# noamzilo/sed-crnn

Measured on AMD Instinct MI355X. Metric: mel-frames/sec training throughput (seq=256, mel=40), higher is better.
Workload: dtype f32; 1 GPU; BASELINE config 2: mono (B=128,256,40,1) per GPU, 3xConv3x3(128)+BN+ReLU+pool(1,2)+dropout0.5, BiGRU 2x128, Linear(256,1), BCEWithLogits, Adam lr 1e-3; full fit step (fwd+loss+bwd+allreduce+Adam); global_batch=128, seq_len=256, n_mels=40, parallelism=single

## Files before the change

### include/sedcrnn.h

```cpp
#ifndef SEDCRNN_H
#define SEDCRNN_H

#include <stddef.h>
#include <stdint.h>

#ifdef __cplusplus
extern "C" {
#endif

#define SED_MAX_CONV 4
#define SED_MAX_GRU 4
#define SED_MAX_DENSE 4

int sed_version(void);
const char* sed_last_error_string(void);

int sed_conv3x3_pack_weights(const float* w_oihw, float* wp_fwd, float* wp_dgrad,
                             int Cout, int Cin, void* stream);

int sed_conv3x3_stat_rows(int B, int Cin, int F, int T, int Cout, int x_is_nchw);

int sed_conv3x3_plan(int B, int Cin, int F, int T, int Cout, int x_is_nchw, int which, int* out);

int sed_conv3x3_fwd(const float* x, int x_is_nchw, const float* wp, const float* bias,
                    float* y, float* stat_partials,
                    int B, int Cin, int F, int T, int Cout, void* stream);

int sed_conv3x3_pack_weights_ex(const float* w_oihw, float* wp_fwd, float* wp_dgrad, int Cout, int Cin, int mode, void* stream);
int sed_conv3x3_fwd_ex(const float* x, int x_is_nchw, const float* wp, const float* bias, float* y, float* stat_partials,
                       int B, int Cin, int F, int T, int Cout, int mode, void* stream);

size_t sed_conv3x3_wgrad_workspace_bytes(int B, int Cin, int F, int T, int Cout);
int sed_conv3x3_wgrad(const float* x, int x_is_nchw, const float* dy, float* dw_oihw,
                      void* workspace, int B, int Cin, int F, int T, int Cout, void* stream);

#define SED_WGRAD_ZERO_ROW_CLEAN 0x100
#define SED_WGRAD_DIRECT 0x200
size_t sed_conv3x3_wgrad_zero_row_bytes(int B, int Cin, int F, int T, int Cout);
int sed_conv3x3_wgrad_ex(const float* x, int x_is_nchw, const float* dy, float* dw_oihw,
                         void* workspace, int B, int Cin, int F, int T, int Cout, int mode, void* stream);

int sed_conv3x3_bn_relu_pool_eval_supported(int B, int Cin, int F, int T, int Cout);
int sed_conv3x3_pack_weights_bn_folded(const float* w, const float* bias, const float* gamma, const float* beta,
                                       const float* running_mean, const float* running_var, float eps,
                                       float* wf, float* bias_folded, int Cout, int Cin, void* stream);
int sed_conv3x3_bn_relu_pool_eval(const float* x, const float* wp_folded, const float* bias_folded, float* pooled,
                                  int B, int Cin, int F, int T, int Cout, void* stream);
int sed_conv3x3_bf16_eval_supported(int B, int Cin, int F, int T, int Cout);
int sed_conv3x3_bf16_pack_weights_bn_folded(const float* w, const float* bias, const float* gamma, const float* beta,
                                            const float* running_mean, const float* running_var, float eps,
                                            void* wf_bf16, float* bias_folded, int Cout, int Cin, void* stream);
int sed_conv3x3_bf16_bn_relu_pool_eval(const void* x, int x_is_bf16, const void* wf_bf16, const float* bias_folded,
                                       void* pooled_bf16, int B, int Cin, int F, int T, int Cout, void* stream);
int sed_conv3x3_dgrad_bnred_rows(int B, int C, int F, int T, int Cin);
int sed_conv3x3_dgrad_bnred(const float* dy, const float* wp_dgrad, float* dx, float* partials, const float* pooled,
                            const float* gamma, const float* beta, const float* conv_out_below, const float* mean,
                            const float* rstd, float drop_p, int pool_f, int pool_t, int Fy, int Ty,
                            int B, int C, int F, int T, int Cin, void* stream);
int sed_conv3x3_wino_rows(int B, int Cin, int F, int T, int Cout);
int sed_conv3x3_wino_phase_ticks(unsigned long long* buf);
size_t sed_conv3x3_wino_packed_floats(int Cout, int Cin);
int sed_conv3x3_wino_pack_weights(const float* w_oihw, float* uf, float* ud, int Cout, int Cin, void* stream);
int sed_conv3x3_wino_fwd(const float* x, const float* uf, const float* bias, float* y, float* stat_partials,
                         int B, int Cin, int F, int T, int Cout, void* stream);
int sed_conv3x3_wino_dgrad_bnred(const float* dy, const float* ud, float* dx, float* partials, const float* pooled,
                                 const float* gamma, const float* beta, const float* conv_out_below, const float* mean,
                                 const float* rstd, float drop_p, int pool_f, int pool_t, int Fy, int Ty,
                                 int B, int C, int F, int T, int Cin, void* stream);
int sed_conv3x3_wino_pack_weights_bn_folded(const float* w_oihw, const float* bias, const float* gamma, const float* beta,
                                            const float* running_mean, const float* running_var, float eps,
                                            float* uf, float* bias_folded, int Cout, int Cin, void* stream);
int sed_conv3x3_wino_bn_relu_pool_eval(const float* x, const float* uf_folded, const float* bias_folded, float* pooled,
                                       int B, int Cin, int F, int T, int Cout, void* stream);
int sed_conv3x3_wino_rg_rows(int B, int C, int F, int T, int Cin, int Cin1);
int sed_conv3x3_wino_dgrad_bnred_rg(const float* dy, const float* ud, float* dx, float* partials, const float* pooled,
                                    const float* gamma, const float* beta, const float* mean, const float* rstd, float drop_p,
                                    const float* x1, int Cin1, const unsigned char* argmax_bits, float* rg_partials,
                                    int B, int C, int F, int T, int Cin, void* stream);
int sed_conv3x3_dgrad_bnred_rg_rows(int B, int C, int F, int T, int Cin, int Cin1);
int sed_conv3x3_dgrad_bnred_rg(const float* dy, const float* wp_dgrad, float* dx, float* partials, const float* pooled,
                               const float* gamma, const float* beta, const float* mean, const float* rstd, float drop_p,
                               const float* x1, int Cin1, const unsigned char* argmax_bits, float* rg_partials,
                               int B, int C, int F, int T, int Cin, void* stream);

int sed_bn_finalize_train(const float* stat_partials, int rows, int C, double count,
                          const float* gamma, const float* beta,
                          float* running_mean, float* running_var, float momentum, float eps,
                          float* mean, float* rstd, float* scale, float* shift, void* stream);
int sed_bn_stat_sums(const float* stat_partials, int rows, int C, float* sums, void* stream);
int sed_bn_finalize_from_sums(const float* sums, int C, double count, const float* gamma, const float* beta,
                              float* running_mean, float* running_var, float momentum, float eps,
                              float* mean, float* rstd, float* scale, float* shift, void* stream);
int sed_bn_finalize_eval(const float* gamma, const float* beta, const float* running_mean,
                         const float* running_var, float eps, int C,
                         float* scale, float* shift, void* stream);

int sed_bn_relu_pool_drop_fwd(const float* y, const float* scale, const float* shift, float* out,
                              int B, int T, int F, int C, int pool_f, int pool_t, int out_tcf,
                              float drop_p, uint64_t seed, const uint64_t* seed_dev, void* stream);

int sed_bn_relu_pool_route(const float* y, const float* scale, const float* shift, unsigned char* route,
                           int B, int T, int F, int C, int pool_f, int pool_t, void* stream);
int sed_bn_bwd_rows(int B, int T, int pool_t);
int sed_bn_relu_pool_drop_bwd_reduce(const float* y, const float* dout, const float* scale,
                                     const float* shift, const float* mean, const float* rstd,
                                     float* partials, int B, int T, int F, int C, int pool_f,
                                     int pool_t, int out_tcf, float drop_p, uint64_t seed, const uint64_t* seed_dev, void* stream);
int sed_bn_bwd_finalize(const float* partials, int rows, int C, float* sum_g, float* sum_gx,
                        float* dgamma, float* dbeta, void* stream);
int sed_bn_bwd_finalize_small_gamma(const float* partials, int rows, int C, float* sum_g, float* sum_gx,
                                    float* dgamma, float* dbeta, const float* dpooled, const float* pooled,
                                    const float* y, const float* gamma, const float* beta, const float* mean,
                                    const float* rstd, const float* scale, const float* shift,
                                    int B, int T, int F, int pool_f, int pool_t, float drop_p, void* stream);
int sed_bn_bwd_reduce_pooled_supported(int F, int C, int pool_f, int pool_t, int out_tcf);
int sed_bn_bwd_reduce_pooled(const float* pooled, const float* dout, const float* gamma, const float* beta,
                             const float* y, const float* mean, const float* rstd, const float* scale, const float* shift,
                             float* partials, int B, int T, int F, int C, int pool_f, int pool_t, int out_tcf, float drop_p, void* stream);
int sed_bn_relu_pool_drop_bwd_apply(const float* y, const float* dout, const float* scale,
                                    const float* shift, const float* mean, const float* rstd,
                                    const float* sum_g, const float* sum_gx, float* dy,
                                    float* dbias_partials, int B, int T, int F, int C, int pool_f,
                                    int pool_t, int out_tcf, float drop_p, uint64_t seed, const uint64_t* seed_dev, void* stream);
int sed_reduce_rows(const float* partials, int rows, int C, int row_stride, float* out, void* stream);

int sed_conv1_fused_supported(int Cin, int F, int T, int C, int pool_f, int pool_t);
int sed_conv1_fused_rows(int B, int T);
size_t sed_conv1_stats_workspace_bytes(int B, int Cin, int T);
size_t sed_conv1_moments_doubles(int Cin);
int sed_conv1_stats(const float* x, const float* wp, const float* bias, float* stat_partials, void* workspace,
                    int B, int Cin, int F, int T, int C, double* moments, void* stream);
int sed_conv1_bn_relu_pool_drop_fwd(const float* x, const float* wp, const float* bias, const float* scale,
                                    const float* shift, float* out, int B, int Cin, int F, int T, int C,
                                    int pool_f, int pool_t, float drop_p, uint64_t seed, const uint64_t* seed_dev,
                                    unsigned char* argmax_bits, void* stream);
int sed_conv1_route(const float* x, const float* wp, const float* bias, const float* scale, const float* shift,
                    unsigned char* route, int B, int Cin, int F, int T, int C, int pool_f, int pool_t, void* stream);
int sed_conv1_bwd_reduce(const float* x, const float* wp, const float* bias, const float* dout,
                         const float* scale, const float* shift, const float* mean, const float* rstd,
                         float* partials, int B, int Cin, int F, int T, int C, int pool_f, int pool_t,
                         float drop_p, uint64_t seed, const uint64_t* seed_dev, void* stream);
size_t sed_conv1_bwd_apply_workspace_bytes(int B, int Cin, int T, int C);
int sed_conv1_bwd_apply_wgrad(const float* x, const float* wp, const float* bias, const float* dout,
                              const float* scale, const float* shift, const float* mean, const float* rstd,
                              const float* sum_g, const float* sum_gx, float* dw_oihw, float* dbias,
                              void* workspace, int B, int Cin, int F, int T, int C, int pool_f, int pool_t,
                              float drop_p, uint64_t seed, const uint64_t* seed_dev,
                              const float* gamma, const float* beta, float* dgamma, void* stream);

int sed_conv1_rgrad_supported(int Cin, int F, int T, int C, int pool_f, int pool_t);
size_t sed_conv1_bwd_wgrad_workspace_bytes(int B, int Cin, int T, int C);
int sed_conv1_bwd_wgrad(const float* x, const float* dout, const float* pooled, const unsigned char* argmax_bits,
                        const double* moments, const float* wp, const float* bias, const float* mean, const float* rstd,
                        const float* scale, const float* sum_g, const float* sum_gx, float* dw_oihw, float* dbias,
                        void* workspace, int B, int Cin, int F, int T, int C, float drop_p,
                        const float* gamma, const float* beta, float* dgamma, void* stream);
int sed_conv1_bwd_wgrad_assemble(const float* partials, int rows, const double* moments, const float* wp, const float* bias,
                                 const float* mean, const float* rstd, const float* scale, const float* sum_g,
                                 const float* sum_gx, float* dw_oihw, float* dbias, int B, int Cin, int F, int T, int C,
                                 const float* gamma, const float* beta, float* dgamma, void* stream);

int sed_gemm_f32(const float* A, long a_si, long a_sk, const float* B, long b_sk, long b_sj,
                 float* C, long ldc, const float* bias, float beta, int M, int N, int K, void* stream);
size_t sed_gemm_f32_workspace_bytes(int M, int N, int K);
int sed_gemm_f32_ws(const float* A, long a_si, long a_sk, const float* B, long b_sk, long b_sj,
                    float* C, long ldc, const float* bias, int M, int N, int K, void* workspace, void* stream);

int sed_gemm_bf16_nt(const void* A, const void* B, const float* bias, float* C, long ldc, int M, int N, int K, void* stream);

int sed_gemm_f32_wgrad(const float* A, long a_si, long a_sk, const float* B, long b_sk, long b_sj,
                       float* C, long ldc, int M, int N, int K, void* workspace, void* stream);
int sed_gemm_f32_plan(int M, int N, int K, int policy, int* bm, int* bn, int* splits, int* k_len);

int sed_linear_fwd(const float* x, const float* W, const float* b, float* y,
                   int M, int K, int N, int relu, void* stream);
size_t sed_linear_bwd_workspace_bytes(int M, int K, int N);
int sed_linear_bwd(const float* x, const float* W, const float* y, float* dy, float* dx,
                   float* dW, float* db, void* workspace, int M, int K, int N, int relu, void* stream);

size_t sed_gru_seq_workspace_bytes(int H);
int sed_gru_seq_fwd(const float* gi, const float* const* whh, const float* const* bhh,
                    float* out, float* saved, void* workspace, int B, int T, int H, void* stream);
size_t sed_gru_seq_bwd_workspace_bytes(int B, int H);
int sed_gru_seq_bwd(const float* dout, const float* saved, const float* const* whh,
                    float* dgi, float* dgh, float* const* dbih, float* const* dbhh, void* workspace,
                    int B, int T, int H, void* stream);
int sed_gru_seq_variant(int B, int H, int* bt, int* hreg, int* hlds);

int sed_loss_fwd_bwd(const float* logits, const float* targets, int n, int kind, float alpha,
                     float gamma, int reduction_mean, float* loss, float* dlogits, float* probs,
                     void* stream);
int sed_sigmoid(const float* x, float* y, int n, void* stream);
int sed_scale(float* x, long n, float alpha, void* stream);

size_t sed_sqnorm_workspace_bytes(long n);
int sed_grad_norm_clip_coef(const float* g, long n, float max_norm, float* norm_out,
                            void* workspace, void* stream);
int sed_adam_step(float* p, const float* g, float* m, float* v, long n, float lr, float beta1,
                  float beta2, float eps, float weight_decay, int step, const float* grad_scale,
                  const uint64_t* step_state, void* stream);
int sed_step_advance(uint64_t* step_state, void* stream);

size_t sed_logmel_tables_bytes(const float* melfb_host, int n_fft, int n_mels);
int sed_logmel_build_tables(const float* window_host, const float* melfb_host, int n_fft, int n_mels,
                            void* tables_host, size_t tables_bytes);
int sed_logmel(const float* pcm, long n_samples, const void* tables, size_t tables_bytes,
               const float* mu, const float* inv_sigma, float* out,
               int n_fft, int hop, int n_mels, int pad_mode, void* stream);
size_t sed_logmel_batch_workspace_bytes(int R);
int sed_logmel_batch(const float* pcm, long pcm_len, const long* clips_host, int R, const void* tables, size_t tables_bytes,
                     const float* mu, const float* inv_sigma, float* out, long out_rows, int n_fft, int hop, int n_mels,
                     int pad_mode, void* workspace, size_t workspace_bytes, void* stream);
size_t sed_logmel_multi_workspace_bytes(int R, int channels);
int sed_logmel_multi(const float* pcm, long pcm_len, const long* clips_host, int R, int channels, const void* tables,
                     size_t tables_bytes, const float* mu, const float* inv_sigma, float* out, long out_rows, int n_fft, int hop,
                     int n_mels, int pad_mode, void* workspace, size_t workspace_bytes, void* stream);
size_t sed_logmel_gcc_workspace_bytes(int R, int channels);
int sed_logmel_gcc(const float* pcm, long pcm_len, const long* clips_host, int R, int channels, const void* tables,
                   size_t tables_bytes, const float* mu, const float* inv_sigma, float* out, long out_rows, int n_fft, int hop,
                   int n_mels, int n_lags, int pad_mode, void* workspace, size_t workspace_bytes, void* stream);
size_t sed_event_tdoa_workspace_bytes(int R, int channels, long E, long max_n_samples, int hop, int max_frames);
int sed_event_tdoa(const float* pcm, long pcm_len, const long* clips_host, int R, int channels, const void* tables,
                   size_t tables_bytes, const int* ev_rec, const int* ev_onset, const int* ev_offset, const int* ev_peak_frame,
                   long E, int time_factor, int hop, int pad_mode, int max_lag, int max_frames, float* lag_out, float* strength_out,
                   int* frames_out, float* acc_out, void* workspace, size_t workspace_bytes, void* stream);
size_t sed_stream_ring_write_workspace_bytes(int lanes);
int sed_stream_ring_write(float* ring, long ring_len, int lanes, long cap, const float* src, long src_len, const long* table_host,
                          void* workspace, size_t workspace_bytes, void* stream);
size_t sed_event_tdoa_ring_workspace_bytes(int R, int channels, long E, long cap, int hop, int max_frames);
int sed_event_tdoa_ring(const float* ring, long ring_len, long cap, const long* n_host, int R, int channels, const void* tables,
                        size_t tables_bytes, const int* ev_rec, const int* ev_onset, const int* ev_offset, const int* ev_peak_frame,
                        long E, int time_factor, int hop, int max_lag, int max_frames, int lat_frames, int history_frames,
                        float* lag_out, float* strength_out, int* frames_out, float* acc_out, void* workspace,
                        size_t workspace_bytes, void* stream);
size_t sed_event_doa_workspace_bytes(int R, int channels, long E, long max_n_samples, int hop, int max_frames);
int sed_event_doa(const float* pcm, long pcm_len, const long* clips_host, int R, int channels, const void* tables,
                  size_t tables_bytes, const int* ev_rec, const int* ev_onset, const int* ev_offset, const int* ev_peak_frame,
                  long E, int time_factor, int hop, int pad_mode, int max_lag, int max_frames, float* lag_out, float* strength_out,
                  int* frames_out, float* acc_out, const int* steer_lags, int D, int Q, const float* trig, int* dir_out,
                  float* power_out, float* srp_out, void* workspace, size_t workspace_bytes, void* stream);
size_t sed_event_doa_ring_workspace_bytes(int R, int channels, long E, long cap, int hop, int max_frames);
int sed_event_doa_ring(const float* ring, long ring_len, long cap, const long* n_host, int R, int channels, const void* tables,
                       size_t tables_bytes, const int* ev_rec, const int* ev_onset, const int* ev_offset, const int* ev_peak_frame,
                       long E, int time_factor, int hop, int max_lag, int max_frames, int lat_frames, int history_frames,
                       float* lag_out, float* strength_out, int* frames_out, float* acc_out, const int* steer_lags, int D, int Q,
                       const float* trig, int* dir_out, float* power_out, float* srp_out, void* workspace, size_t workspace_bytes,
                       void* stream);
size_t sed_event_doa_track_workspace_bytes(int R, int channels, long E, long max_n_samples, int hop, int max_frames, int D,
                                           int block_chunks, int smooth);
int sed_event_doa_track(const float* pcm, long pcm_len, const long* clips_host, int R, int channels, const void* tables,
                        size_t tables_bytes, const int* ev_rec, const int* ev_onset, const int* ev_offset, const int* ev_peak_frame,
                        long E, int time_factor, int hop, int pad_mode, int max_lag, int max_frames, float* lag_out,
// ... 50 lines not shown
                         const int* ev_loc_frames, long E, int time_factor, int hop, int max_frames, const double* tau, int D,
                         double loading, int noise_blocks, int noise_guard, const void* tables, size_t tables_bytes,
                         const int* audio_len, const long* audio_start, float* audio, long audio_total, int* noise_frames_out,
                         void* workspace, size_t workspace_bytes, void* stream);
size_t sed_event_mvdr_noise_ring_workspace_bytes(int R, int channels, int max_frames, int hop, int noise_blocks);
int sed_event_mvdr_noise_ring(const float* ring, long ring_len, long cap, const long* n_host, int R, int channels, const int* ev_rec,
                              const int* ev_onset, const int* ev_offset, const int* ev_peak_frame, const int* ev_dir,
                              const int* ev_loc_frames, long E, int time_factor, int hop, int max_frames, const double* tau, int D,
                              double loading, int noise_blocks, int noise_guard, const void* tables, size_t tables_bytes,
                              const int* audio_len, const long* audio_start, float* audio, long audio_total, int* noise_frames_out,
                              void* workspace, size_t workspace_bytes, void* stream);

size_t sed_event_quiet_frames_workspace_bytes(int R, int channels, long mask_frames, int noise_blocks);
int sed_event_quiet_frames(long pcm_len, const long* clips_host, int R, int channels, const int* ev_rec, const int* ev_cls,
                           const int* ev_onset, const int* ev_offset, const int* ev_peak_frame, const int* ev_dir,
                           const int* ev_loc_frames, long E, int time_factor, int hop, int max_frames, int D, int n_classes,
                           int noise_blocks, int noise_guard, int noise_search, int noise_min, int exclude_any, int* noise_frames_out,
                           int* noise_sel_out, void* workspace, size_t workspace_bytes, void* stream);
size_t sed_event_mvdr_quiet_workspace_bytes(int R, int channels, int max_frames, int hop, int noise_blocks, long mask_frames);
int sed_event_mvdr_quiet(const float* pcm, long pcm_len, const long* clips_host, int R, int channels, const int* ev_rec,
                         const int* ev_cls, const int* ev_onset, const int* ev_offset, const int* ev_peak_frame, const int* ev_dir,
                         const int* ev_loc_frames, long E, int time_factor, int hop, int max_frames, const double* tau, int D,
                         double loading, int noise_blocks, int noise_guard, int n_classes, int noise_search, int noise_min,
                         int exclude_any, const void* tables, size_t tables_bytes, const int* audio_len, const long* audio_start,
                         float* audio, long audio_total, int* noise_frames_out, int* noise_sel_out, void* workspace,
                         size_t workspace_bytes, void* stream);

size_t sed_event_mvdr_track_workspace_bytes(int R, int channels, int max_frames, int hop, int noise_blocks, int track_slots);
int sed_event_mvdr_track(const float* pcm, long pcm_len, const long* clips_host, int R, int channels, const int* ev_rec,
                         const int* ev_onset, const int* ev_offset, const int* ev_peak_frame, const int* ev_dir,
                         const int* ev_loc_frames, long E, int time_factor, int hop, int max_frames, const double* tau, int D,
                         double loading, int noise_blocks, int noise_guard, const void* tables, size_t tables_bytes,
                         const int* audio_len, const long* audio_start, float* audio, long audio_total, int* noise_frames_out,
                         int block_chunks, int track_slots, const int* trk_len, const int* trk_dir, void* workspace,
                         size_t workspace_bytes, void* stream);
size_t sed_event_mvdr_track_ring_workspace_bytes(int R, int channels, int max_frames, int hop, int noise_blocks, int track_slots);
int sed_event_mvdr_track_ring(const float* ring, long ring_len, long cap, const long* n_host, int R, int channels, const int* ev_rec,
                              const int* ev_onset, const int* ev_offset, const int* ev_peak_frame, const int* ev_dir,
                              const int* ev_loc_frames, long E, int time_factor, int hop, int max_frames, const double* tau, int D,
                              double loading, int noise_blocks, int noise_guard, const void* tables, size_t tables_bytes,
                              const int* audio_len, const long* audio_start, float* audio, long audio_total, int* noise_frames_out,
                              int block_chunks, int track_slots, const int* trk_len, const int* trk_dir, void* workspace,
                              size_t workspace_bytes, void* stream);
size_t sed_event_mvdr_quiet_track_workspace_bytes(int R, int channels, int max_frames, int hop, int noise_blocks, long mask_frames,
                                                  int track_slots);
int sed_event_mvdr_quiet_track(const float* pcm, long pcm_len, const long* clips_host, int R, int channels, const int* ev_rec,
                               const int* ev_cls, const int* ev_onset, const int* ev_offset, const int* ev_peak_frame,
                               const int* ev_dir, const int* ev_loc_frames, long E, int time_factor, int hop, int max_frames,
                               const double* tau, int D, double loading, int noise_blocks, int noise_guard, int n_classes,
                               int noise_search, int noise_min, int exclude_any, const void* tables, size_t tables_bytes,
                               const int* audio_len, const long* audio_start, float* audio, long audio_total, int* noise_frames_out,
                               int* noise_sel_out, int block_chunks, int track_slots, const int* trk_len, const int* trk_dir,
                               void* workspace, size_t workspace_bytes, void* stream);

size_t sed_pcen_workspace_bytes(long rows, int R, int W);
int sed_pcen(float* x, long rows, int stride, int col0, int W, const long* recs_host, int R, float* state, double smooth_b,
             float gain, float bias, float power, float eps, float scale, const float* mu, const float* inv_sigma,
             void* workspace, size_t workspace_bytes, void* stream);

size_t sed_resample_workspace_bytes(int R);
int sed_resample_check_table(const long* rows_host, int R, long x_frames, long hist_len, long out_len, int L, int M, int half);
int sed_resample(const void* x, long x_frames, int format, int channels, float* hist, long hist_len, const float* taps,
                 long taps_len, int L, int M, int half, const long* rows_host, int R, float* out, long out_len, void* workspace,
                 size_t workspace_bytes, void* stream);
size_t sed_resample_select_workspace_bytes(int R);
int sed_resample_select_check_table(const long* rows_host, int R, int channels, long x_frames, long hist_len, long out_len, int L,
                                    int M, int half);
int sed_resample_select(const void* x, long x_frames, int format, int channels, float* hist, long hist_len, const float* taps,
                        long taps_len, int L, int M, int half, const long* rows_host, int R, float* out, long out_len,
                        void* workspace, size_t workspace_bytes, void* stream);

int sed_window_batch(const float* mel, const float* lab, long N, int C, int F, int K, const int* starts,
                     const int* tmask, const int* fmask, int n_masks, int time_w, int freq_w,
                     float* x, float* y, int B, int L, int pool, void* stream);
int sed_pack_sequences(const float* feat, long N, int C, int F, int S, int time_last, float* out, void* stream);
size_t sed_col_mean_std_workspace_bytes(int F);
int sed_col_mean_std(const float* x, long N, int F, double* mean, double* stdv, void* workspace, void* stream);
int sed_col_standardize(const float* x, long N, int F, const double* mean, const double* stdv, float* out, void* stream);

#define SED_SEGMENT_COUNTS 17
int sed_segment_counts(const float* pred, const float* lab, long rows, int K, int block, float threshold,
                       unsigned long long* counts17, void* stream);

int sed_detect_stitch(const float* logits, long n_win, int win_out, int K, int hop_out, long last_start_out, long n_out,
                      int combine, int trim, float* probs, void* stream);
size_t sed_detect_workspace_bytes(long n_out, int K, int max_events);
int sed_detect_events(const float* probs, long n_out, int K, int median, float lo, float hi, int min_gap, int min_len,
                      int max_events, void* workspace, size_t workspace_bytes, int* cls, int* onset, int* offset,
                      float* peak, int* peak_frame, int* count, void* stream);
size_t sed_detect_batch_workspace_bytes(long n_total, int K, int R, int max_events);
int sed_detect_stitch_batch(const float* logits, long logits_len, const long* recs_host, int R, int K, int combine, int trim,
                            float* probs, long n_total, void* workspace, size_t workspace_bytes, void* stream);
int sed_detect_events_batch(const float* probs, const long* n_out_host, int R, int K, int median, float lo, float hi, int min_gap,
                            int min_len, int max_events, void* workspace, size_t workspace_bytes, int* rec, int* cls, int* onset,
                            int* offset, float* peak, int* peak_frame, int* event_off, void* stream);

typedef struct sed_tune_setting { int median; float lo, hi; int min_gap, min_len; } sed_tune_setting;
size_t sed_tune_workspace_bytes(long n_total, int K, int R, int n_tracks, int G);
int sed_tune_sweep(const float* probs, const long* n_out_host, int R, int K, const sed_tune_setting* settings_host, int G,
                   const int* ref_off, const int* ref_onset, const int* ref_offset, const int* ref_tol, int collar, int block,
                   void* workspace, size_t workspace_bytes, long* counts, void* stream);

size_t sed_psds_workspace_bytes(long n_total, int K, int R, int n_tracks, int G);
int sed_psds_sweep(const float* probs, const long* n_out_host, int R, int K, const sed_tune_setting* settings_host, int G,
                   const int* ref_off, const int* ref_onset, const int* ref_offset, int dtc_milli, int gtc_milli, int cttc_milli,
                   void* workspace, size_t workspace_bytes, long* counts, long* ct, void* stream);

size_t sed_stream_state_bytes(int S, int K, int win_out, int hop_out, int median, int max_new_windows);
int sed_stream_init(void* state, size_t state_bytes, int S, int K, int win_out, int hop_out, int median, int max_new_windows,
                    void* stream);
int sed_stream_reset(void* state, size_t state_bytes, int S, int K, int win_out, int hop_out, int median, int max_new_windows,
                     const int* streams_host, int n_streams, void* stream);
size_t sed_stream_step_workspace_bytes(int S, int K, int max_new_decided);
int sed_stream_step(void* state, size_t state_bytes, int S, int K, int win_out, int hop_out, int median, int max_new_windows,
                    int combine, int trim, float lo, float hi, int min_gap, int min_len, const float* logits, long logits_len,
                    const long* table_host, int max_new_decided, float* probs, long probs_rows, int max_events, int* ev_stream,
                    int* cls, int* onset, int* offset, float* peak, int* peak_frame, int* event_off, void* workspace,
                    size_t workspace_bytes, void* stream);
size_t sed_stream_append_workspace_bytes(int S);
int sed_stream_append(float* buf, long buf_len, long stride, const float* fresh, long fresh_len, float* work, long work_len,
                      const long* table_host, int S, void* workspace, size_t workspace_bytes, void* stream);

typedef sed_tune_setting sed_decoder_setting;
int sed_detect_events_classwise(const float* probs, long n_out, int K, const sed_decoder_setting* classes_host, int max_events,
                                void* workspace, size_t workspace_bytes, int* cls, int* onset, int* offset, float* peak,
                                int* peak_frame, int* count, void* stream);
int sed_detect_events_batch_classwise(const float* probs, const long* n_out_host, int R, int K,
                                      const sed_decoder_setting* classes_host, int max_events, void* workspace, size_t workspace_bytes,
                                      int* rec, int* cls, int* onset, int* offset, float* peak, int* peak_frame, int* event_off,
                                      void* stream);
int sed_stream_step_classwise(void* state, size_t state_bytes, int S, int K, int win_out, int hop_out, int median, int max_new_windows,
                              int combine, int trim, const sed_decoder_setting* classes_host, const float* logits, long logits_len,
                              const long* table_host, int max_new_decided, float* probs, long probs_rows, int max_events,
                              int* ev_stream, int* cls, int* onset, int* offset, float* peak, int* peak_frame, int* event_off,
                              void* workspace, size_t workspace_bytes, void* stream);

typedef struct sed_net_cfg {
    int B, Cin, F, T;
    int n_conv;
    int C[SED_MAX_CONV];
    int pool_f[SED_MAX_CONV], pool_t[SED_MAX_CONV];
    float drop_p[SED_MAX_CONV];
    int n_gru;
    int H[SED_MAX_GRU];
    int n_dense;
    int D[SED_MAX_DENSE];
    float bn_eps, bn_momentum;
    int conv_mode;
    int flags;
} sed_net_cfg;
#define SED_NET_AUX_FIRST 0x1
#define SED_NET_NO_GATE 0x2
#define SED_NET_DIRECT_CONV 0x4

typedef struct sed_net_params {
    float* conv_w[SED_MAX_CONV];
    float* conv_b[SED_MAX_CONV];
    float* bn_g[SED_MAX_CONV];
    float* bn_b[SED_MAX_CONV];
    float* bn_rm[SED_MAX_CONV];
    float* bn_rv[SED_MAX_CONV];
    float* gru_wih[SED_MAX_GRU][2];
    float* gru_whh[SED_MAX_GRU][2];
    float* gru_bih[SED_MAX_GRU][2];
    float* gru_bhh[SED_MAX_GRU][2];
    float* dense_w[SED_MAX_DENSE];
    float* dense_b[SED_MAX_DENSE];
} sed_net_params;

int sed_net_out_shape(const sed_net_cfg* cfg, int* Tp, int* Fp);
size_t sed_net_workspace_bytes(const sed_net_cfg* cfg, int training);
int sed_net_forward(const sed_net_cfg* cfg, const sed_net_params* p, const float* x, float* logits,
                    void* workspace, int training, uint64_t seed, const uint64_t* seed_dev, void* stream);
int sed_net_backward(const sed_net_cfg* cfg, const sed_net_params* p, const sed_net_params* g,
                     const float* x, const float* dlogits, void* workspace, uint64_t seed, const uint64_t* seed_dev,
                     int stage_begin, int stage_end, void* stream, void* aux_stream);
int sed_net_backward_ready_stage(const sed_net_cfg* cfg, int block);

int sed_net_sync_region(const sed_net_cfg* cfg, int backward, int block, size_t* offset_bytes, size_t* n_floats);
int sed_net_forward_phases(const sed_net_cfg* cfg, const sed_net_params* p, const float* x, float* logits,
                           void* workspace, int training, uint64_t seed, int phase_begin, int phase_end,
                           float count_scale, void* stream);
int sed_net_backward_phases(const sed_net_cfg* cfg, const sed_net_params* p, const sed_net_params* g,
                            const float* x, const float* dlogits, void* workspace, uint64_t seed,
                            int phase_begin, int phase_end, float count_scale, void* stream);

int sed_net_workspace_region(const sed_net_cfg* cfg, int training, const char* name, int index,
                             size_t* offset_bytes, size_t* n_floats);

int sed_net_inference_plan(const sed_net_cfg* cfg, int* conv_bf16, int* proj_bf16);

int sed_net_routing(const sed_net_cfg* cfg, const sed_net_params* p, const float* x, const void* workspace, int block,
                    unsigned char* route, void* stream);

enum sed_kernel_tag {
    SED_K_CONV_MFMA_FWD = 0,
    SED_K_CONV_SMALL_FWD,
    SED_K_CONV_MFMA_WGRAD,
    SED_K_CONV_SMALL_WGRAD,
    SED_K_BN_FWD,
    SED_K_BN_BWD_REDUCE,
    SED_K_BN_BWD_APPLY,
    SED_K_GEMM,
    SED_K_GRU_FWD,
    SED_K_GRU_BWD,
    SED_K_ADAM,
    SED_K_LOGMEL,
    SED_K_CONV_MFMA_DGRAD,
    SED_K_COUNT
};
int sed_prof_enable(unsigned tag_mask);
int sed_prof_read(int tag, double* total_ms, long* launches, double* total_units);
const char* sed_prof_tag_name(int tag);
int sed_prof_tag_count(void);

#ifdef __cplusplus
}
#endif
#endif
```

### sed_crnn_amd/_lib.py

```python
import ctypes as C
import os

HERE = os.path.dirname(os.path.abspath(__file__))
LIB_PATH = os.environ.get("SED_CRNN_LIB") or os.path.join(HERE, "libsedcrnn.so")

SED_MAX_CONV = 4
SED_MAX_GRU = 4
SED_MAX_DENSE = 4

_fp = C.c_void_p
_stream = C.c_void_p


class NetCfg(C.Structure):
    _fields_ = [
        ("B", C.c_int), ("Cin", C.c_int), ("F", C.c_int), ("T", C.c_int),
        ("n_conv", C.c_int),
        ("C", C.c_int * SED_MAX_CONV),
        ("pool_f", C.c_int * SED_MAX_CONV), ("pool_t", C.c_int * SED_MAX_CONV),
        ("drop_p", C.c_float * SED_MAX_CONV),
        ("n_gru", C.c_int), ("H", C.c_int * SED_MAX_GRU),
        ("n_dense", C.c_int), ("D", C.c_int * SED_MAX_DENSE),
        ("bn_eps", C.c_float), ("bn_momentum", C.c_float),
        ("conv_mode", C.c_int),
        ("flags", C.c_int),
    ]


class NetParams(C.Structure):
    _fields_ = [
        ("conv_w", _fp * SED_MAX_CONV), ("conv_b", _fp * SED_MAX_CONV),
        ("bn_g", _fp * SED_MAX_CONV), ("bn_b", _fp * SED_MAX_CONV),
        ("bn_rm", _fp * SED_MAX_CONV), ("bn_rv", _fp * SED_MAX_CONV),
        ("gru_wih", (_fp * 2) * SED_MAX_GRU), ("gru_whh", (_fp * 2) * SED_MAX_GRU),
        ("gru_bih", (_fp * 2) * SED_MAX_GRU), ("gru_bhh", (_fp * 2) * SED_MAX_GRU),
        ("dense_w", _fp * SED_MAX_DENSE), ("dense_b", _fp * SED_MAX_DENSE),
    ]


class TuneSetting(C.Structure):
    _fields_ = [("median", C.c_int), ("lo", C.c_float), ("hi", C.c_float), ("min_gap", C.c_int), ("min_len", C.c_int)]


_i, _l, _f, _d, _u64, _sz = C.c_int, C.c_long, C.c_float, C.c_double, C.c_uint64, C.c_size_t
_pp = C.POINTER(_fp)

SIGNATURES = {
    "sed_version": (_i, []),
    "sed_last_error_string": (C.c_char_p, []),
    "sed_conv3x3_pack_weights": (_i, [_fp, _fp, _fp, _i, _i, _stream]),
    "sed_conv3x3_stat_rows": (_i, [_i, _i, _i, _i, _i, _i]),
    "sed_conv3x3_plan": (_i, [_i, _i, _i, _i, _i, _i, _i, C.POINTER(_i)]),
    "sed_conv3x3_fwd": (_i, [_fp, _i, _fp, _fp, _fp, _fp, _i, _i, _i, _i, _i, _stream]),
    "sed_conv3x3_pack_weights_ex": (_i, [_fp, _fp, _fp, _i, _i, _i, _stream]),
    "sed_conv3x3_fwd_ex": (_i, [_fp, _i, _fp, _fp, _fp, _fp, _i, _i, _i, _i, _i, _i, _stream]),
    "sed_conv3x3_wgrad_workspace_bytes": (_sz, [_i, _i, _i, _i, _i]),
    "sed_conv3x3_wgrad_zero_row_bytes": (_sz, [_i, _i, _i, _i, _i]),
    "sed_conv3x3_wgrad": (_i, [_fp, _i, _fp, _fp, _fp, _i, _i, _i, _i, _i, _stream]),
    "sed_conv3x3_wgrad_ex": (_i, [_fp, _i, _fp, _fp, _fp, _i, _i, _i, _i, _i, _i, _stream]),
    "sed_conv3x3_bn_relu_pool_eval_supported": (_i, [_i, _i, _i, _i, _i]),
    "sed_conv3x3_pack_weights_bn_folded": (_i, [_fp, _fp, _fp, _fp, _fp, _fp, _f, _fp, _fp, _i, _i, _stream]),
    "sed_conv3x3_bn_relu_pool_eval": (_i, [_fp, _fp, _fp, _fp, _i, _i, _i, _i, _i, _stream]),
    "sed_conv3x3_bf16_eval_supported": (_i, [_i, _i, _i, _i, _i]),
    "sed_conv3x3_bf16_pack_weights_bn_folded": (_i, [_fp, _fp, _fp, _fp, _fp, _fp, _f, _fp, _fp, _i, _i, _stream]),
    "sed_conv3x3_bf16_bn_relu_pool_eval": (_i, [_fp, _i, _fp, _fp, _fp, _i, _i, _i, _i, _i, _stream]),
    "sed_conv3x3_dgrad_bnred_rows": (_i, [_i, _i, _i, _i, _i]),
    "sed_conv3x3_dgrad_bnred": (_i, [_fp, _fp, _fp, _fp, _fp, _fp, _fp, _fp, _fp, _fp, _f, _i, _i, _i, _i, _i, _i, _i, _i, _i, _stream]),
    "sed_conv3x3_wino_rows": (_i, [_i, _i, _i, _i, _i]),
    "sed_conv3x3_wino_phase_ticks": (_i, [_fp]),
    "sed_conv3x3_wino_packed_floats": (_sz, [_i, _i]),
    "sed_conv3x3_wino_pack_weights": (_i, [_fp, _fp, _fp, _i, _i, _stream]),
    "sed_conv3x3_wino_fwd": (_i, [_fp, _fp, _fp, _fp, _fp, _i, _i, _i, _i, _i, _stream]),
    "sed_conv3x3_wino_dgrad_bnred": (_i, [_fp, _fp, _fp, _fp, _fp, _fp, _fp, _fp, _fp, _fp, _f, _i, _i, _i, _i, _i, _i, _i, _i, _i, _stream]),
    "sed_conv3x3_wino_pack_weights_bn_folded": (_i, [_fp, _fp, _fp, _fp, _fp, _fp, _f, _fp, _fp, _i, _i, _stream]),
    "sed_conv3x3_wino_bn_relu_pool_eval": (_i, [_fp, _fp, _fp, _fp, _i, _i, _i, _i, _i, _stream]),
    "sed_conv3x3_wino_rg_rows": (_i, [_i, _i, _i, _i, _i, _i]),
    "sed_conv3x3_wino_dgrad_bnred_rg": (_i, [_fp, _fp, _fp, _fp, _fp, _fp, _fp, _fp, _fp, _f, _fp, _i, _fp, _fp, _i, _i, _i, _i, _i, _stream]),
    "sed_conv3x3_dgrad_bnred_rg_rows": (_i, [_i, _i, _i, _i, _i, _i]),
    "sed_conv3x3_dgrad_bnred_rg": (_i, [_fp, _fp, _fp, _fp, _fp, _fp, _fp, _fp, _fp, _f, _fp, _i, _fp, _fp, _i, _i, _i, _i, _i, _stream]),
    "sed_conv1_fused_supported": (_i, [_i, _i, _i, _i, _i, _i]),
    "sed_conv1_fused_rows": (_i, [_i, _i]),
    "sed_conv1_stats_workspace_bytes": (_sz, [_i, _i, _i]),
    "sed_conv1_moments_doubles": (_sz, [_i]),
    "sed_conv1_stats": (_i, [_fp, _fp, _fp, _fp, _fp, _i, _i, _i, _i, _i, _fp, _stream]),
    "sed_conv1_bn_relu_pool_drop_fwd": (_i, [_fp, _fp, _fp, _fp, _fp, _fp, _i, _i, _i, _i, _i, _i, _i, _f, _u64, _fp, _fp, _stream]),
    "sed_conv1_rgrad_supported": (_i, [_i, _i, _i, _i, _i, _i]),
    "sed_conv1_bwd_wgrad_workspace_bytes": (_sz, [_i, _i, _i, _i]),
    "sed_conv1_bwd_wgrad": (_i, [_fp, _fp, _fp, _fp, _fp, _fp, _fp, _fp, _fp, _fp, _fp, _fp, _fp, _fp, _fp, _i, _i, _i, _i, _i, _f, _fp, _fp, _fp, _stream]),
    "sed_conv1_bwd_wgrad_assemble": (_i, [_fp, _i, _fp, _fp, _fp, _fp, _fp, _fp, _fp, _fp, _fp, _fp, _i, _i, _i, _i, _i, _fp, _fp, _fp, _stream]),
    "sed_conv1_route": (_i, [_fp, _fp, _fp, _fp, _fp, _fp, _i, _i, _i, _i, _i, _i, _i, _stream]),
    "sed_conv1_bwd_reduce": (_i, [_fp, _fp, _fp, _fp, _fp, _fp, _fp, _fp, _fp, _i, _i, _i, _i, _i, _i, _i, _f, _u64, _fp, _stream]),
    "sed_conv1_bwd_apply_workspace_bytes": (_sz, [_i, _i, _i, _i]),
    "sed_conv1_bwd_apply_wgrad": (_i, [_fp, _fp, _fp, _fp, _fp, _fp, _fp, _fp, _fp, _fp, _fp, _fp, _fp, _i, _i, _i, _i, _i, _i, _i, _f, _u64, _fp, _fp, _fp, _fp, _stream]),
    "sed_bn_finalize_train": (_i, [_fp, _i, _i, _d, _fp, _fp, _fp, _fp, _f, _f, _fp, _fp, _fp, _fp, _stream]),
    "sed_bn_stat_sums": (_i, [_fp, _i, _i, _fp, _stream]),
    "sed_bn_finalize_from_sums": (_i, [_fp, _i, _d, _fp, _fp, _fp, _fp, _f, _f, _fp, _fp, _fp, _fp, _stream]),
    "sed_bn_finalize_eval": (_i, [_fp, _fp, _fp, _fp, _f, _i, _fp, _fp, _stream]),
    "sed_bn_relu_pool_drop_fwd": (_i, [_fp, _fp, _fp, _fp, _i, _i, _i, _i, _i, _i, _i, _f, _u64, _fp, _stream]),
    "sed_bn_relu_pool_route": (_i, [_fp, _fp, _fp, _fp, _i, _i, _i, _i, _i, _i, _stream]),
    "sed_bn_bwd_rows": (_i, [_i, _i, _i]),
    "sed_bn_relu_pool_drop_bwd_reduce": (_i, [_fp, _fp, _fp, _fp, _fp, _fp, _fp, _i, _i, _i, _i, _i, _i, _i, _f, _u64, _fp, _stream]),
    "sed_bn_bwd_finalize": (_i, [_fp, _i, _i, _fp, _fp, _fp, _fp, _stream]),
    "sed_bn_bwd_finalize_small_gamma": (_i, [_fp, _i, _i, _fp, _fp, _fp, _fp, _fp, _fp, _fp, _fp, _fp, _fp, _fp, _fp, _fp, _i, _i, _i, _i, _i, _f, _stream]),
    "sed_bn_bwd_reduce_pooled_supported": (_i, [_i, _i, _i, _i, _i]),
    "sed_bn_bwd_reduce_pooled": (_i, [_fp, _fp, _fp, _fp, _fp, _fp, _fp, _fp, _fp, _fp, _i, _i, _i, _i, _i, _i, _i, _f, _stream]),
    "sed_bn_relu_pool_drop_bwd_apply": (_i, [_fp, _fp, _fp, _fp, _fp, _fp, _fp, _fp, _fp, _fp, _i, _i, _i, _i, _i, _i, _i, _f, _u64, _fp, _stream]),
    "sed_reduce_rows": (_i, [_fp, _i, _i, _i, _fp, _stream]),
    "sed_gemm_f32": (_i, [_fp, _l, _l, _fp, _l, _l, _fp, _l, _fp, _f, _i, _i, _i, _stream]),
    "sed_gemm_f32_workspace_bytes": (_sz, [_i, _i, _i]),
    "sed_gemm_f32_ws": (_i, [_fp, _l, _l, _fp, _l, _l, _fp, _l, _fp, _i, _i, _i, _fp, _stream]),
    "sed_gemm_bf16_nt": (_i, [_fp, _fp, _fp, _fp, _l, _i, _i, _i, _stream]),
    "sed_gemm_f32_wgrad": (_i, [_fp, _l, _l, _fp, _l, _l, _fp, _l, _i, _i, _i, _fp, _stream]),
    "sed_gemm_f32_plan": (_i, [_i, _i, _i, _i, C.POINTER(_i), C.POINTER(_i), C.POINTER(_i), C.POINTER(_i)]),
    "sed_linear_fwd": (_i, [_fp, _fp, _fp, _fp, _i, _i, _i, _i, _stream]),
    "sed_linear_bwd_workspace_bytes": (_sz, [_i, _i, _i]),
    "sed_linear_bwd": (_i, [_fp, _fp, _fp, _fp, _fp, _fp, _fp, _fp, _i, _i, _i, _i, _stream]),
    "sed_gru_seq_workspace_bytes": (_sz, [_i]),
    "sed_gru_seq_fwd": (_i, [_fp, _pp, _pp, _fp, _fp, _fp, _i, _i, _i, _stream]),
    "sed_gru_seq_bwd_workspace_bytes": (_sz, [_i, _i]),
    "sed_gru_seq_bwd": (_i, [_fp, _fp, _pp, _fp, _fp, _pp, _pp, _fp, _i, _i, _i, _stream]),
    "sed_gru_seq_variant": (_i, [_i, _i, C.POINTER(_i), C.POINTER(_i), C.POINTER(_i)]),
    "sed_loss_fwd_bwd": (_i, [_fp, _fp, _i, _i, _f, _f, _i, _fp, _fp, _fp, _stream]),
    "sed_sigmoid": (_i, [_fp, _fp, _i, _stream]),
    "sed_scale": (_i, [_fp, _l, _f, _stream]),
    "sed_sqnorm_workspace_bytes": (_sz, [_l]),
    "sed_grad_norm_clip_coef": (_i, [_fp, _l, _f, _fp, _fp, _stream]),
    "sed_adam_step": (_i, [_fp, _fp, _fp, _fp, _l, _f, _f, _f, _f, _f, _i, _fp, _fp, _stream]),
    "sed_step_advance": (_i, [_fp, _stream]),
    "sed_logmel_tables_bytes": (_sz, [_fp, _i, _i]),
    "sed_logmel_build_tables": (_i, [_fp, _fp, _i, _i, _fp, _sz]),
    "sed_logmel": (_i, [_fp, _l, _fp, _sz, _fp, _fp, _fp, _i, _i, _i, _i, _stream]),
    "sed_logmel_batch_workspace_bytes": (_sz, [_i]),
    "sed_logmel_batch": (_i, [_fp, _l, _fp, _i, _fp, _sz, _fp, _fp, _fp, _l, _i, _i, _i, _i, _fp, _sz, _stream]),
    "sed_logmel_multi_workspace_bytes": (_sz, [_i, _i]),
    "sed_logmel_multi": (_i, [_fp, _l, _fp, _i, _i, _fp, _sz, _fp, _fp, _fp, _l, _i, _i, _i, _i, _fp, _sz, _stream]),
    "sed_logmel_gcc_workspace_bytes": (_sz, [_i, _i]),
    "sed_logmel_gcc": (_i, [_fp, _l, _fp, _i, _i, _fp, _sz, _fp, _fp, _fp, _l, _i, _i, _i, _i, _i, _fp, _sz, _stream]),
    "sed_event_tdoa_workspace_bytes": (_sz, [_i, _i, _l, _l, _i, _i]),
    "sed_event_tdoa": (_i, [_fp, _l, _fp, _i, _i, _fp, _sz, _fp, _fp, _fp, _fp, _l, _i, _i, _i, _i, _i, _fp, _fp, _fp, _fp, _fp, _sz,
                            _stream]),
    "sed_stream_ring_write_workspace_bytes": (_sz, [_i]),
    "sed_stream_ring_write": (_i, [_fp, _l, _i, _l, _fp, _l, _fp, _fp, _sz, _stream]),
    "sed_event_tdoa_ring_workspace_bytes": (_sz, [_i, _i, _l, _l, _i, _i]),
    "sed_event_tdoa_ring": (_i, [_fp, _l, _l, _fp, _i, _i, _fp, _sz, _fp, _fp, _fp, _fp, _l, _i, _i, _i, _i, _i, _i, _fp, _fp, _fp, _fp,
                                 _fp, _sz, _stream]),
    "sed_event_doa_workspace_bytes": (_sz, [_i, _i, _l, _l, _i, _i]),
    "sed_event_doa": (_i, [_fp, _l, _fp, _i, _i, _fp, _sz, _fp, _fp, _fp, _fp, _l, _i, _i, _i, _i, _i, _fp, _fp, _fp, _fp, _fp, _i, _i,
                           _fp, _fp, _fp, _fp, _fp, _sz, _stream]),
    "sed_event_doa_ring_workspace_bytes": (_sz, [_i, _i, _l, _l, _i, _i]),
    "sed_event_doa_ring": (_i, [_fp, _l, _l, _fp, _i, _i, _fp, _sz, _fp, _fp, _fp, _fp, _l, _i, _i, _i, _i, _i, _i, _fp, _fp, _fp, _fp,
                                _fp, _i, _i, _fp, _fp, _fp, _fp, _fp, _sz, _stream]),
    "sed_event_doa_track_workspace_bytes": (_sz, [_i, _i, _l, _l, _i, _i, _i, _i, _i]),
    "sed_event_doa_track": (_i, [_fp, _l, _fp, _i, _i, _fp, _sz, _fp, _fp, _fp, _fp, _l, _i, _i, _i, _i, _i, _fp, _fp, _fp, _fp, _fp, _i,
                                 _i, _fp, _fp, _fp, _fp, _i, _fp, _fp, _fp, _fp, _fp, _fp, _fp, _fp, _sz, _stream]),
    "sed_event_doa_track_ring_workspace_bytes": (_sz, [_i, _i, _l, _l, _i, _i, _i, _i, _i]),
    "sed_event_doa_track_ring": (_i, [_fp, _l, _l, _fp, _i, _i, _fp, _sz, _fp, _fp, _fp, _fp, _l, _i, _i, _i, _i, _i, _i, _fp, _fp, _fp,
                                      _fp, _fp, _i, _i, _fp, _fp, _fp, _fp, _i, _fp, _fp, _fp, _fp, _fp, _fp, _fp, _fp, _sz, _stream]),
    "sed_event_beam_workspace_bytes": (_sz, [_i, _i]),
    "sed_event_beam_ring_workspace_bytes": (_sz, [_i]),
    "sed_event_beam_spans": (_i, [_l, _fp, _i, _i, _fp, _fp, _fp, _fp, _fp, _fp, _l, _i, _i, _i, _i, _fp, _fp, _fp, _fp, _sz, _stream]),
    "sed_event_beam_spans_ring": (_i, [_fp, _i, _i, _fp, _fp, _fp, _fp, _fp, _fp, _l, _i, _i, _i, _i, _fp, _fp, _fp, _fp, _sz, _stream]),
    "sed_event_beamform": (_i, [_fp, _l, _fp, _i, _i, _fp, _fp, _fp, _fp, _fp, _fp, _l, _i, _i, _i, _fp, _i, _i, _i, _fp, _fp, _fp, _fp,
                                _l, _fp, _sz, _stream]),
    "sed_event_beamform_ring": (_i, [_fp, _l, _l, _fp, _i, _i, _fp, _fp, _fp, _fp, _fp, _fp, _l, _i, _i, _i, _fp, _i, _i, _i, _fp, _fp,
                                     _fp, _fp, _l, _fp, _sz, _stream]),
    "sed_event_mvdr_workspace_bytes": (_sz, [_i, _i, _i, _i]),
    "sed_event_mvdr": (_i, [_fp, _l, _fp, _i, _i, _fp, _fp, _fp, _fp, _fp, _fp, _l, _i, _i, _i, _fp, _i, _d, _fp, _sz, _fp, _fp, _fp, _l,
                            _fp, _sz, _stream]),
    "sed_event_mvdr_ring_workspace_bytes": (_sz, [_i, _i, _i, _i]),
    "sed_event_mvdr_ring": (_i, [_fp, _l, _l, _fp, _i, _i, _fp, _fp, _fp, _fp, _fp, _fp, _l, _i, _i, _i, _fp, _i, _d, _fp, _sz, _fp, _fp,
                                 _fp, _l, _fp, _sz, _stream]),
    "sed_event_mvdr_noise_workspace_bytes": (_sz, [_i, _i, _i, _i, _i]),
    "sed_event_mvdr_noise": (_i, [_fp, _l, _fp, _i, _i, _fp, _fp, _fp, _fp, _fp, _fp, _l, _i, _i, _i, _fp, _i, _d, _i, _i, _fp, _sz, _fp,
                                  _fp, _fp, _l, _fp, _fp, _sz, _stream]),
    "sed_event_mvdr_noise_ring_workspace_bytes": (_sz, [_i, _i, _i, _i, _i]),
    "sed_event_mvdr_noise_ring": (_i, [_fp, _l, _l, _fp, _i, _i, _fp, _fp, _fp, _fp, _fp, _fp, _l, _i, _i, _i, _fp, _i, _d, _i, _i, _fp,
                                       _sz, _fp, _fp, _fp, _l, _fp, _fp, _sz, _stream]),
    "sed_event_quiet_frames_workspace_bytes": (_sz, [_i, _i, _l, _i]),
    "sed_event_quiet_frames": (_i, [_l, _fp, _i, _i, _fp, _fp, _fp, _fp, _fp, _fp, _fp, _l, _i, _i, _i, _i, _i, _i, _i, _i, _i, _i, _fp, _fp,
                                    _fp, _sz, _stream]),
    "sed_event_mvdr_quiet_workspace_bytes": (_sz, [_i, _i, _i, _i, _i, _l]),
    "sed_event_mvdr_quiet": (_i, [_fp, _l, _fp, _i, _i, _fp, _fp, _fp, _fp, _fp, _fp, _fp, _l, _i, _i, _i, _fp, _i, _d, _i, _i, _i, _i, _i,
                                  _i, _fp, _sz, _fp, _fp, _fp, _l, _fp, _fp, _fp, _sz, _stream]),
    "sed_event_mvdr_track_workspace_bytes": (_sz, [_i, _i, _i, _i, _i, _i]),
    "sed_event_mvdr_track": (_i, [_fp, _l, _fp, _i, _i, _fp, _fp, _fp, _fp, _fp, _fp, _l, _i, _i, _i, _fp, _i, _d, _i, _i, _fp, _sz, _fp,
                                  _fp, _fp, _l, _fp, _i, _i, _fp, _fp, _fp, _sz, _stream]),
    "sed_event_mvdr_track_ring_workspace_bytes": (_sz, [_i, _i, _i, _i, _i, _i]),
    "sed_event_mvdr_track_ring": (_i, [_fp, _l, _l, _fp, _i, _i, _fp, _fp, _fp, _fp, _fp, _fp, _l, _i, _i, _i, _fp, _i, _d, _i, _i, _fp,
                                       _sz, _fp, _fp, _fp, _l, _fp, _i, _i, _fp, _fp, _fp, _sz, _stream]),
    "sed_event_mvdr_quiet_track_workspace_bytes": (_sz, [_i, _i, _i, _i, _i, _l, _i]),
    "sed_event_mvdr_quiet_track": (_i, [_fp, _l, _fp, _i, _i, _fp, _fp, _fp, _fp, _fp, _fp, _fp, _l, _i, _i, _i, _fp, _i, _d, _i, _i, _i, _i,
                                        _i, _i, _fp, _sz, _fp, _fp, _fp, _l, _fp, _fp, _i, _i, _fp, _fp, _fp, _sz, _stream]),
    "sed_pcen_workspace_bytes": (_sz, [_l, _i, _i]),
    "sed_pcen": (_i, [_fp, _l, _i, _i, _i, _fp, _i, _fp, _d, _f, _f, _f, _f, _f, _fp, _fp, _fp, _sz, _stream]),
    "sed_resample_workspace_bytes": (_sz, [_i]),
    "sed_resample_check_table": (_i, [_fp, _i, _l, _l, _l, _i, _i, _i]),
    "sed_resample": (_i, [_fp, _l, _i, _i, _fp, _l, _fp, _l, _i, _i, _i, _fp, _i, _fp, _l, _fp, _sz, _stream]),
    "sed_resample_select_workspace_bytes": (_sz, [_i]),
    "sed_resample_select_check_table": (_i, [_fp, _i, _i, _l, _l, _l, _i, _i, _i]),
    "sed_resample_select": (_i, [_fp, _l, _i, _i, _fp, _l, _fp, _l, _i, _i, _i, _fp, _i, _fp, _l, _fp, _sz, _stream]),
    "sed_window_batch": (_i, [_fp, _fp, _l, _i, _i, _i, _fp, _fp, _fp, _i, _i, _i, _fp, _fp, _i, _i, _i, _stream]),
    "sed_pack_sequences": (_i, [_fp, _l, _i, _i, _i, _i, _fp, _stream]),
    "sed_col_mean_std_workspace_bytes": (_sz, [_i]),
    "sed_col_mean_std": (_i, [_fp, _l, _i, _fp, _fp, _fp, _stream]),
    "sed_col_standardize": (_i, [_fp, _l, _i, _fp, _fp, _fp, _stream]),
    "sed_segment_counts": (_i, [_fp, _fp, _l, _i, _i, _f, _fp, _stream]),
    "sed_detect_stitch": (_i, [_fp, _l, _i, _i, _i, _l, _l, _i, _i, _fp, _stream]),
    "sed_detect_workspace_bytes": (_sz, [_l, _i, _i]),
    "sed_detect_events": (_i, [_fp, _l, _i, _i, _f, _f, _i, _i, _i, _fp, _sz, _fp, _fp, _fp, _fp, _fp, _fp, _stream]),
    "sed_detect_batch_workspace_bytes": (_sz, [_l, _i, _i, _i]),
    "sed_detect_stitch_batch": (_i, [_fp, _l, _fp, _i, _i, _i, _i, _fp, _l, _fp, _sz, _stream]),
    "sed_detect_events_batch": (_i, [_fp, _fp, _i, _i, _i, _f, _f, _i, _i, _i, _fp, _sz, _fp, _fp, _fp, _fp, _fp, _fp, _fp, _stream]),
    "sed_tune_workspace_bytes": (_sz, [_l, _i, _i, _i, _i]),
    "sed_tune_sweep": (_i, [_fp, _fp, _i, _i, _fp, _i, _fp, _fp, _fp, _fp, _i, _i, _fp, _sz, _fp, _stream]),
    "sed_psds_workspace_bytes": (_sz, [_l, _i, _i, _i, _i]),
    "sed_psds_sweep": (_i, [_fp, _fp, _i, _i, _fp, _i, _fp, _fp, _fp, _i, _i, _i, _fp, _sz, _fp, _fp, _stream]),
    "sed_stream_state_bytes": (_sz, [_i, _i, _i, _i, _i, _i]),
    "sed_stream_init": (_i, [_fp, _sz, _i, _i, _i, _i, _i, _i, _stream]),
    "sed_stream_reset": (_i, [_fp, _sz, _i, _i, _i, _i, _i, _i, _fp, _i, _stream]),
    "sed_stream_step_workspace_bytes": (_sz, [_i, _i, _i]),
    "sed_stream_step": (_i, [_fp, _sz, _i, _i, _i, _i, _i, _i, _i, _i, _f, _f, _i, _i, _fp, _l, _fp, _i, _fp, _l, _i, _fp, _fp, _fp,
                             _fp, _fp, _fp, _fp, _fp, _sz, _stream]),
    "sed_stream_append_workspace_bytes": (_sz, [_i]),
    "sed_stream_append": (_i, [_fp, _l, _l, _fp, _l, _fp, _l, _fp, _i, _fp, _sz, _stream]),
    "sed_detect_events_classwise": (_i, [_fp, _l, _i, _fp, _i, _fp, _sz, _fp, _fp, _fp, _fp, _fp, _fp, _stream]),
    "sed_detect_events_batch_classwise": (_i, [_fp, _fp, _i, _i, _fp, _i, _fp, _sz, _fp, _fp, _fp, _fp, _fp, _fp, _fp, _stream]),
    "sed_stream_step_classwise": (_i, [_fp, _sz, _i, _i, _i, _i, _i, _i, _i, _i, _fp, _fp, _l, _fp, _i, _fp, _l, _i, _fp, _fp, _fp,
                                       _fp, _fp, _fp, _fp, _fp, _sz, _stream]),
    "sed_prof_enable": (_i, [C.c_uint]),
    "sed_prof_read": (_i, [_i, C.POINTER(_d), C.POINTER(_l), C.POINTER(_d)]),
    "sed_prof_tag_name": (C.c_char_p, [_i]),
    "sed_prof_tag_count": (_i, []),
    "sed_net_out_shape": (_i, [C.POINTER(NetCfg), C.POINTER(_i), C.POINTER(_i)]),
    "sed_net_workspace_bytes": (_sz, [C.POINTER(NetCfg), _i]),
    "sed_net_forward": (_i, [C.POINTER(NetCfg), C.POINTER(NetParams), _fp, _fp, _fp, _i, _u64, _fp, _stream]),
    "sed_net_sync_region": (_i, [C.POINTER(NetCfg), _i, _i, C.POINTER(_sz), C.POINTER(_sz)]),
    "sed_net_workspace_region": (_i, [C.POINTER(NetCfg), _i, C.c_char_p, _i, C.POINTER(_sz), C.POINTER(_sz)]),
    "sed_net_routing": (_i, [C.POINTER(NetCfg), C.POINTER(NetParams), _fp, _fp, _i, _fp, _stream]),
    "sed_net_inference_plan": (_i, [C.POINTER(NetCfg), C.POINTER(C.c_int), C.POINTER(C.c_int)]),
    "sed_net_forward_phases": (_i, [C.POINTER(NetCfg), C.POINTER(NetParams), _fp, _fp, _fp, _i, _u64, _i, _i, _f, _stream]),
    "sed_net_backward_phases": (_i, [C.POINTER(NetCfg), C.POINTER(NetParams), C.POINTER(NetParams), _fp, _fp, _fp, _u64, _i, _i, _f, _stream]),
    "sed_net_backward": (_i, [C.POINTER(NetCfg), C.POINTER(NetParams), C.POINTER(NetParams), _fp, _fp, _fp, _u64, _fp, _i, _i, _stream, _stream]),
    "sed_net_backward_ready_stage": (_i, [C.POINTER(NetCfg), _i]),
}

_lib = None


class SedHipError(RuntimeError):
    pass

# ... 33 lines not shown
```

### sed_crnn_amd/csrc/bnpool.hip

```cpp
#include "common.h"

#define BN_MAX_BLOCKS 1024

__device__ __forceinline__ void bn_two_channel_sums(const float* __restrict__ part, int rows, int C, int c, bool live,
                                                    double (*sred)[2][2], double* A_out, double* Q_out) {
    const int sl = threadIdx.x >> 1, lane = threadIdx.x & 63, wv = threadIdx.x >> 6;
    double a = 0.0, q = 0.0;
    if (live) {
#pragma unroll 8
        for (int r = sl; r < rows; r += 512) {
            const float* p0 = part + (size_t)r * 2 * C + c;
            a += (double)p0[0];
            q += (double)p0[C];
        }
    }
#pragma unroll
    for (int o = 2; o < 64; o <<= 1) { a += __shfl_xor(a, o, 64); q += __shfl_xor(q, o, 64); }
    if (lane < 2) { sred[wv][lane][0] = a; sred[wv][lane][1] = q; }
    __syncthreads();
    double A = 0.0, Q = 0.0;
    if (threadIdx.x < 2) {
        for (int w = 0; w < 16; ++w) { A += sred[w][threadIdx.x][0]; Q += sred[w][threadIdx.x][1]; }
    }
    *A_out = A; *Q_out = Q;
// ... 88 lines not shown
    int c = blockIdx.x * blockDim.x + threadIdx.x;
    if (c >= C) return;
    float sc = g[c] / sqrtf(rv[c] + eps);
    scale[c] = sc;
    shift[c] = b[c] - rm[c] * sc;
}

extern "C" int sed_bn_finalize_eval(const float* gamma, const float* beta, const float* rm, const float* rv,
                                    float eps, int C, float* scale, float* shift, void* stream) {
    SED_REQUIRE(gamma && beta && rm && rv && scale && shift && C > 0, "bn_finalize_eval: bad arguments");
    bn_finalize_eval_k<<<cdiv(C, 256), 256, 0, as_stream(stream)>>>(gamma, beta, rm, rv, eps, C, scale, shift);
    SED_LAUNCH_CHECK("bn_finalize_eval");
    return 0;
}

__global__ __launch_bounds__(256) void reduce_rows_k(const float* __restrict__ part, int rows, int C,
                                                     int row_stride, float* __restrict__ out) {
    __shared__ double s1[32][9];
    const int cl = threadIdx.x & 7, sl = threadIdx.x >> 3;
    const int c = blockIdx.x * 8 + cl;
    double a = 0.0;
    if (c < C) {
        double a1 = 0.0, a2 = 0.0, a3 = 0.0;
        int r = sl;
        for (; r + 96 < rows; r += 128) {
            const float* p0 = part + (size_t)r * row_stride + c;
            a += (double)p0[0];
            a1 += (double)p0[(size_t)32 * row_stride];
            a2 += (double)p0[(size_t)64 * row_stride];
            a3 += (double)p0[(size_t)96 * row_stride];
        }
        for (; r < rows; r += 32) a += (double)part[(size_t)r * row_stride + c];
        a += a1 + a2 + a3;
    }
    s1[sl][cl] = a;
    __syncthreads();
    if (sl == 0 && c < C) {
        double A = 0.0;
        for (int s = 0; s < 32; ++s) A += s1[s][cl];
        out[c] = (float)A;
    }
}

extern "C" int sed_reduce_rows(const float* part, int rows, int C, int row_stride, float* out, void* stream) {
    SED_REQUIRE(part && out && rows > 0 && C > 0 && row_stride >= C, "reduce_rows: bad arguments");
    reduce_rows_k<<<cdiv(C, 8), 256, 0, as_stream(stream)>>>(part, rows, C, row_stride, out);
    SED_LAUNCH_CHECK("reduce_rows");
    return 0;
}

__global__ __launch_bounds__(256) void bn_relu_pool_drop_fwd_k(
    const float* __restrict__ y, const float* __restrict__ scale, const float* __restrict__ shift,
    float* __restrict__ out, int B, int T, int F, int C, int pf, int pt, float drop_p, uint64_t seed,
    const uint64_t* __restrict__ seed_dev) {
    if (seed_dev) seed += seed_dev[0] * 0x9E3779B97F4A7C15ull;
    const int Tp = T / pt, Fp = F / pf, C4 = C >> 2;
    const size_t n = (size_t)B * Tp * Fp * C4;
    const float inv_keep = drop_p > 0.f ? 1.f / (1.f - drop_p) : 1.f;
    for (size_t i = (size_t)blockIdx.x * 256 + threadIdx.x; i < n; i += (size_t)gridDim.x * 256) {
        int c4 = (int)(i % C4);
        size_t pos = i / C4;
        int fp = (int)(pos % Fp);
        size_t bt = pos / Fp;
        int tp = (int)(bt % Tp);
        size_t b = bt / Tp;
        f32x4 sc = *(const f32x4*)(scale + c4 * 4), sh = *(const f32x4*)(shift + c4 * 4);
        f32x4 m = {0, 0, 0, 0};
        for (int dt = 0; dt < pt; ++dt)
            for (int df = 0; df < pf; ++df) {
                f32x4 v = *(const f32x4*)(y + (((b * T + tp * pt + dt) * F + fp * pf + df) * (size_t)C) + c4 * 4);
                v = v * sc + sh;
#pragma unroll
                for (int k = 0; k < 4; ++k) m[k] = fmaxf(m[k], v[k]);
            }
        if (drop_p > 0.f) {
#pragma unroll
            for (int k = 0; k < 4; ++k) m[k] *= sed_drop_mult(seed, i * 4 + k, drop_p, inv_keep);
        }
        *(f32x4*)(out + i * 4) = m;
    }
}

__global__ __launch_bounds__(256) void bn_relu_pool_drop_fwd_tcf_k(
    const float* __restrict__ y, const float* __restrict__ scale, const float* __restrict__ shift,
    float* __restrict__ out, int B, int T, int F, int C, int pf, int pt, float drop_p, uint64_t seed,
    const uint64_t* __restrict__ seed_dev) {
    if (seed_dev) seed += seed_dev[0] * 0x9E3779B97F4A7C15ull;
    extern __shared__ __attribute__((aligned(16))) float tile[];
    const int Tp = T / pt, Fp = F / pf, C4 = C >> 2, LD = C + 1;
    const float inv_keep = drop_p > 0.f ? 1.f / (1.f - drop_p) : 1.f;
    for (int bt = blockIdx.x; bt < B * Tp; bt += gridDim.x) {
        int tp = bt % Tp;
        size_t b = bt / Tp;
        __syncthreads();
        for (int i = threadIdx.x; i < Fp * C4; i += 256) {
            int c4 = i % C4, fp = i / C4;
            f32x4 sc = *(const f32x4*)(scale + c4 * 4), sh = *(const f32x4*)(shift + c4 * 4);
            f32x4 m = {0, 0, 0, 0};
            for (int dt = 0; dt < pt; ++dt)
                for (int df = 0; df < pf; ++df) {
                    f32x4 v = *(const f32x4*)(y + (((b * T + tp * pt + dt) * F + fp * pf + df) * (size_t)C) + c4 * 4);
                    v = v * sc + sh;
#pragma unroll
                    for (int k = 0; k < 4; ++k) m[k] = fmaxf(m[k], v[k]);
                }
            if (drop_p > 0.f) {
                size_t oi = (((size_t)bt * Fp + fp) * C4 + c4) * 4;
#pragma unroll
                for (int k = 0; k < 4; ++k) m[k] *= sed_drop_mult(seed, oi + k, drop_p, inv_keep);
            }
#pragma unroll
            for (int k = 0; k < 4; ++k) tile[fp * LD + c4 * 4 + k] = m[k];
        }
        __syncthreads();
        float* o = out + (size_t)bt * C * Fp;
        for (int i = threadIdx.x; i < C * Fp; i += 256) {
            int c = i / Fp, fp = i - c * Fp;
            o[i] = tile[fp * LD + c];
        }
    }
}

static int check_pool(const char* who, int B, int T, int F, int C, int pf, int pt) {
    SED_REQUIRE(B > 0 && T > 0 && F > 0 && C > 0 && pf > 0 && pt > 0, "%s: bad shape", who);
    SED_REQUIRE(C % 4 == 0, "%s: C must be a multiple of 4 (got %d)", who, C);
    SED_REQUIRE(T / pt >= 1 && F / pf >= 1, "%s: T=%d / F=%d smaller than the pool (%d,%d)", who, T, F, pt, pf);
    return 0;
}

extern "C" int sed_bn_relu_pool_drop_fwd(const float* y, const float* scale, const float* shift, float* out, int B,
                                         int T, int F, int C, int pf, int pt, int out_tcf, float drop_p,
                                         uint64_t seed, const uint64_t* seed_dev, void* stream) {
    SED_REQUIRE(y && scale && shift && out, "bn_relu_pool_drop_fwd: null pointer");
    SED_TRY(check_pool("bn_relu_pool_drop_fwd", B, T, F, C, pf, pt));
    SED_REQUIRE(drop_p >= 0.f && drop_p < 1.f, "bn_relu_pool_drop_fwd: drop_p=%f out of [0,1)", drop_p);
    hipStream_t s = as_stream(stream);
    const int Tp = T / pt, Fp = F / pf;
    SedProfScope prof(SED_K_BN_FWD, s, 4.0 * B * C * ((double)T * F + (double)Tp * Fp));
    if (!out_tcf) {
        size_t n = (size_t)B * Tp * Fp * (C / 4);
        int grid = (int)((n + 255) / 256 < 8192 ? (n + 255) / 256 : 8192);
        bn_relu_pool_drop_fwd_k<<<grid, 256, 0, s>>>(y, scale, shift, out, B, T, F, C, pf, pt, drop_p, seed, seed_dev);
    } else {
        size_t lds = (size_t)Fp * (C + 1) * sizeof(float);
        SED_REQUIRE(lds <= 150 * 1024, "bn_relu_pool_drop_fwd: F'*C tile too large for LDS");
        if (lds > 48 * 1024) (void)hipFuncSetAttribute((const void*)bn_relu_pool_drop_fwd_tcf_k, hipFuncAttributeMaxDynamicSharedMemorySize, (int)lds);
        int grid = B * Tp < 4096 ? B * Tp : 4096;
        bn_relu_pool_drop_fwd_tcf_k<<<grid, 256, lds, s>>>(y, scale, shift, out, B, T, F, C, pf, pt, drop_p, seed, seed_dev);
    }
    SED_LAUNCH_CHECK("bn_relu_pool_drop_fwd");
    return 0;
}

__global__ __launch_bounds__(256) void bn_relu_pool_route_k(
    const float* __restrict__ y, const float* __restrict__ scale, const float* __restrict__ shift,
    unsigned char* __restrict__ route, int B, int T, int F, int C, int pf, int pt) {
    const int Tp = T / pt, Fp = F / pf, C4 = C >> 2;
    const size_t n = (size_t)B * Tp * Fp * C4;
    for (size_t i = (size_t)blockIdx.x * 256 + threadIdx.x; i < n; i += (size_t)gridDim.x * 256) {
        int c4 = (int)(i % C4);
        size_t pos = i / C4;
        int fp = (int)(pos % Fp);
        size_t bt = pos / Fp;
        int tp = (int)(bt % Tp);
        size_t b = bt / Tp;
        f32x4 sc = *(const f32x4*)(scale + c4 * 4), sh = *(const f32x4*)(shift + c4 * 4);
        f32x4 best = {-INFINITY, -INFINITY, -INFINITY, -INFINITY};
        int bidx[4] = {0, 0, 0, 0};
        int widx = 0;
        for (int df = 0; df < pf; ++df)
            for (int dt = 0; dt < pt; ++dt, ++widx) {
                f32x4 v = *(const f32x4*)(y + (((b * T + tp * pt + dt) * F + fp * pf + df) * (size_t)C) + c4 * 4);
                f32x4 z = v * sc + sh;
#pragma unroll
                for (int k = 0; k < 4; ++k)
                    if (z[k] > best[k]) { best[k] = z[k]; bidx[k] = widx; }
            }
        uchar4 code;
        code.x = best[0] > 0.f ? (unsigned char)(1 + bidx[0]) : 0;
        code.y = best[1] > 0.f ? (unsigned char)(1 + bidx[1]) : 0;
        code.z = best[2] > 0.f ? (unsigned char)(1 + bidx[2]) : 0;
        code.w = best[3] > 0.f ? (unsigned char)(1 + bidx[3]) : 0;
        *(uchar4*)(route + i * 4) = code;
    }
}

extern "C" int sed_bn_relu_pool_route(const float* y, const float* scale, const float* shift, unsigned char* route,
                                      int B, int T, int F, int C, int pf, int pt, void* stream) {
    SED_REQUIRE(y && scale && shift && route, "bn_relu_pool_route: null pointer");
    SED_TRY(check_pool("bn_relu_pool_route", B, T, F, C, pf, pt));
    SED_REQUIRE(pf * pt <= 254, "bn_relu_pool_route: a %dx%d window does not fit the one-byte code", pf, pt);
    size_t n = (size_t)B * (T / pt) * (F / pf) * (C / 4);
    int grid = (int)((n + 255) / 256 < 8192 ? (n + 255) / 256 : 8192);
    bn_relu_pool_route_k<<<grid, 256, 0, as_stream(stream)>>>(y, scale, shift, route, B, T, F, C, pf, pt);
    SED_LAUNCH_CHECK("bn_relu_pool_route");
    return 0;
}

extern "C" int sed_bn_bwd_rows(int B, int T, int pool_t) {
    long r = (long)B * (T / (pool_t > 0 ? pool_t : 1));
    return (int)(r < BN_MAX_BLOCKS ? r : BN_MAX_BLOCKS);
}

template <int MODE, bool P12>
__global__ __launch_bounds__(256) void bn_relu_pool_drop_bwd_k(
    const float* __restrict__ y, const float* __restrict__ dout, const float* __restrict__ scale,
    const float* __restrict__ shift, const float* __restrict__ mean, const float* __restrict__ rstd,
    const float* __restrict__ sum_g, const float* __restrict__ sum_gx, float* __restrict__ dy,
    float* __restrict__ partials, int B, int T, int F, int C, int pf, int pt, int out_tcf, float drop_p,
    uint64_t seed, const uint64_t* __restrict__ seed_dev) {
    if (seed_dev) seed += seed_dev[0] * 0x9E3779B97F4A7C15ull;
    extern __shared__ __attribute__((aligned(16))) float smem[];
    const int Tp = T / pt, Fp = F / pf, C4 = C >> 2, LD = C + 1;
    float* tile = smem;
    const int tid = threadIdx.x;
    const int nslots = 256 / C4 > 0 ? 256 / C4 : 1;
    const int c4 = tid % C4, slot = tid / C4;
    const bool active = slot < nslots;
    const float inv_keep = drop_p > 0.f ? 1.f / (1.f - drop_p) : 1.f;
    const float invN = 1.f / ((float)B * (float)T * (float)F);

    f32x4 sc = {0, 0, 0, 0}, sh = sc, mu = sc, rs = sc, sg = sc, sgx = sc;
    if (active) {
        sc = *(const f32x4*)(scale + c4 * 4);
        sh = *(const f32x4*)(shift + c4 * 4);
        mu = *(const f32x4*)(mean + c4 * 4);
        rs = *(const f32x4*)(rstd + c4 * 4);
        if (MODE == 1) {
            sg = *(const f32x4*)(sum_g + c4 * 4) * invN;
            sgx = *(const f32x4*)(sum_gx + c4 * 4) * invN;
        }
    }
    f32x4 a1 = {0, 0, 0, 0}, a2 = {0, 0, 0, 0};

    for (int bt = blockIdx.x; bt < B * Tp; bt += gridDim.x) {
        int tp = bt % Tp;
        size_t b = bt / Tp;
        if (out_tcf) {
            __syncthreads();
            const float* d = dout + (size_t)bt * C * Fp;
            for (int i = tid; i < C * Fp; i += 256) {
                int c = i / Fp, fp = i - c * Fp;
                tile[fp * LD + c] = d[i];
            }
            __syncthreads();
        }
        if (!active) continue;
        for (int fp = slot; fp < Fp; fp += nslots) {
            f32x4 g;
            if (out_tcf) {
#pragma unroll
                for (int k = 0; k < 4; ++k) g[k] = tile[fp * LD + c4 * 4 + k];
            } else {
                g = *(const f32x4*)(dout + (((size_t)bt * Fp + fp) * C4 + c4) * 4);
            }
            if (drop_p > 0.f) {
                size_t oi = (((size_t)bt * Fp + fp) * C4 + c4) * 4;
#pragma unroll
                for (int k = 0; k < 4; ++k) g[k] *= sed_drop_mult(seed, oi + k, drop_p, inv_keep);
            }
            f32x4 best = {-INFINITY, -INFINITY, -INFINITY, -INFINITY};
            f32x4 bx = {0, 0, 0, 0};
            int bidx[4] = {0, 0, 0, 0};
            int widx = 0;
            f32x4 vw[2];
            if (P12) {
                const float* yp = y + (((b * T + tp * 2) * F + fp) * (size_t)C) + c4 * 4;
                vw[0] = *(const f32x4*)yp;
                vw[1] = *(const f32x4*)(yp + (size_t)F * C);
            }
#pragma unroll
            for (int df = 0; df < (P12 ? 1 : pf); ++df)
#pragma unroll
                for (int dt = 0; dt < (P12 ? 2 : pt); ++dt, ++widx) {
                    f32x4 v = P12 ? vw[dt] : *(const f32x4*)(y + (((b * T + tp * pt + dt) * F + fp * pf + df) * (size_t)C) + c4 * 4);
                    f32x4 z = v * sc + sh;
#pragma unroll
                    for (int k = 0; k < 4; ++k)
                        if (z[k] > best[k]) { best[k] = z[k]; bx[k] = (v[k] - mu[k]) * rs[k]; bidx[k] = widx; }
                }
#pragma unroll
            for (int k = 0; k < 4; ++k)
                if (!(best[k] > 0.f)) g[k] = 0.f;
            if (MODE == 0) {
                a1 += g;
                a2 += g * bx;
            } else {
                widx = 0;
#pragma unroll
                for (int df = 0; df < (P12 ? 1 : pf); ++df)
#pragma unroll
                    for (int dt = 0; dt < (P12 ? 2 : pt); ++dt, ++widx) {
                        size_t off = (((b * T + tp * pt + dt) * F + fp * pf + df) * (size_t)C) + c4 * 4;
                        f32x4 v = P12 ? vw[dt] : *(const f32x4*)(y + off);
                        f32x4 o;
#pragma unroll
                        for (int k = 0; k < 4; ++k) {
                            float xh = (v[k] - mu[k]) * rs[k];
                            float gk = (bidx[k] == widx) ? g[k] : 0.f;
                            o[k] = sc[k] * (gk - sg[k] - xh * sgx[k]);
                        }
                        *(f32x4*)(dy + off) = o;
                        a1 += o;
                    }
            }
        }
// ... 307 lines not shown
```

### sed_crnn_amd/csrc/conv_shared.h

```cpp
#pragma once
#include "common.h"

struct ConvBnRed {
    const float* pooled;
    const float* gamma;
    const float* beta;
    const float* ybelow;
    const float* mean;
    const float* rstd;
    float keep, inv_keep;
    int pf, pt, Fy, Ty;
    const float* x1;
    const unsigned char* bits;
    float* rgp;
    float invXT;
};

#ifdef __HIPCC__
__host__ __device__ inline size_t wino_frag_index(int comp, int k, int n, int K, int N) {
    const int cc = k >> 5, g = (k & 31) >> 3, h = (k & 7) >> 2, j = k & 3, coh = n >> 6, nt = (n >> 5) & 1, r = n & 31;
    (void)N;
    return (((((((size_t)coh * 16 + comp) * (K >> 5) + cc) * 4 + g) * 2 + nt) * 64) + r + 32 * h) * 4 + j;
}
__host__ __device__ inline size_t bf16_eval_frag_index(int tap, int co, int ci, int Cout, int Cin) {
    return (((((size_t)tap * (Cin >> 4) + (ci >> 4)) * (Cout >> 5) + (co >> 5)) * 64) + (co & 31) + 32 * ((ci & 15) >> 3)) * 8 + (ci & 7);
}
#define WN_ZTAIL 256
__device__ __forceinline__ void wino_pack_one(const float* __restrict__ w, float* __restrict__ uf, float* __restrict__ ud, int Cout, int Cin, int i,
                                              const float* __restrict__ gamma = nullptr, const float* __restrict__ rv = nullptr, float eps = 0.f) {
    if (i < WN_ZTAIL) {
        if (uf) uf[(size_t)16 * Cout * Cin + i] = 0.f;
        if (ud) ud[(size_t)16 * Cout * Cin + i] = 0.f;
    }
    if (i >= Cout * Cin) return;
    const int ci = i % Cin, co = i / Cin;
    float g[3][3];
#pragma unroll
    for (int kh = 0; kh < 3; ++kh)
#pragma unroll
        for (int kw = 0; kw < 3; ++kw) g[kw][kh] = w[(size_t)i * 9 + kh * 3 + kw];
    if (gamma) {
        const float sc = gamma[co] / sqrtf(rv[co] + eps);
#pragma unroll
        for (int k = 0; k < 9; ++k) g[k / 3][k % 3] *= sc;
    }
#pragma unroll
    for (int pass = 0; pass < 2; ++pass) {
        float* dst = pass ? ud : uf;
        if (!dst) continue;
        float t[4][3];
#pragma unroll
        for (int c = 0; c < 3; ++c) {
            const float g0 = pass ? g[2][2 - c] : g[0][c], g1 = pass ? g[1][2 - c] : g[1][c], g2 = pass ? g[0][2 - c] : g[2][c];
            t[0][c] = g0;
            t[1][c] = 0.5f * (g0 + g1 + g2);
            t[2][c] = 0.5f * (g0 - g1 + g2);
            t[3][c] = g2;
        }
#pragma unroll
        for (int xi = 0; xi < 4; ++xi) {
            const float u0 = t[xi][0], u1 = 0.5f * (t[xi][0] + t[xi][1] + t[xi][2]), u2 = 0.5f * (t[xi][0] - t[xi][1] + t[xi][2]), u3 = t[xi][2];
            const float uu[4] = {u0, u1, u2, u3};
#pragma unroll
            for (int nu = 0; nu < 4; ++nu)
                dst[pass ? wino_frag_index(xi * 4 + nu, co, ci, Cout, Cin) : wino_frag_index(xi * 4 + nu, ci, co, Cin, Cout)] = uu[nu];
        }
    }
}
#endif

int sed_internal_wino_rows(int B, int Cin, int F, int T, int Cout);
int sed_internal_wino_launch(const float* x, const float* uq, const float* bias, float* y, float* stat, const ConvBnRed* br,
                             int rgc, int B, int Cin, int F, int T, int Cout, hipStream_t s);
```

### sed_crnn_amd/csrc/net.hip

```cpp
#include <string.h>
#include "common.h"

namespace {

struct ConvL { int Cin, C, T, F, Tp, Fp, pf, pt, rows, bn_rows, nchw, fused; float drop;
               int red_rows;
               int rg_rows;
               int rgrad;
               int wino, wino_d;
               int ev;
               int bf; };

struct GruL { int in, H; };

struct Layout {
    int n_conv, n_gru, n_dense, M, Tp, Fp, feat;
    int proj_bf;
    ConvL cv[SED_MAX_CONV];
    GruL gr[SED_MAX_GRU];
    int dK[SED_MAX_DENSE], dN[SED_MAX_DENSE];
    size_t wp_f[SED_MAX_CONV], wp_d[SED_MAX_CONV], conv_out[SED_MAX_CONV], stat[SED_MAX_CONV];
    size_t mean[SED_MAX_CONV], rstd[SED_MAX_CONV], scale[SED_MAX_CONV], shift[SED_MAX_CONV];
    size_t pooled[SED_MAX_CONV], bn_sums[SED_MAX_CONV], c1_stat_ws, c1_bits, c1_mom;
    size_t bias_f[SED_MAX_CONV];
    size_t wih_perm;
    size_t gi[SED_MAX_GRU], gout[SED_MAX_GRU], saved[SED_MAX_GRU];
    size_t gru_ws[SED_MAX_GRU];
    size_t act[SED_MAX_DENSE];
    size_t wgrad_zrow;
    size_t wg_arrive;
    size_t bn_part, sum_g, sum_gx, dbias_part, dconv[SED_MAX_CONV], gradA, wgrad_ws, wgrad_ws_aux, c1_ws, dgi[SED_MAX_GRU], dgh[SED_MAX_GRU], dgout[SED_MAX_GRU];
    size_t gru_bws[SED_MAX_GRU];
    size_t dact[SED_MAX_DENSE], lin_ws, gemm_ws, gemm_ws_aux;
    size_t total;
};

struct Carver {
    size_t off = 0;
    size_t take(size_t n) { size_t o = off; off += (n + 63) & ~(size_t)63; return o; }
};

int build_layout(const sed_net_cfg* c, int training, Layout* L) {
    SED_REQUIRE(c, "net: null config");
    SED_REQUIRE(c->B > 0 && c->Cin > 0 && c->F > 0 && c->T > 0, "net: bad input shape B=%d Cin=%d F=%d T=%d", c->B, c->Cin, c->F, c->T);
    SED_REQUIRE(c->n_conv >= 1 && c->n_conv <= SED_MAX_CONV, "net: n_conv=%d out of range", c->n_conv);
    SED_REQUIRE(c->n_gru >= 1 && c->n_gru <= SED_MAX_GRU, "net: n_gru=%d out of range", c->n_gru);
    SED_REQUIRE(c->n_dense >= 1 && c->n_dense <= SED_MAX_DENSE, "net: n_dense=%d out of range", c->n_dense);
    SED_REQUIRE(c->conv_mode >= 0 && c->conv_mode <= 2, "net: conv_mode=%d (0 = exact fp32, 1 = bf16x3 experiment, 2 = bf16 inference)", c->conv_mode);
    SED_REQUIRE(c->conv_mode != 2 || !training, "net: conv_mode 2 (bf16 inference) is an eval-only plan; training runs with conv_mode 0 or 1");
    SED_REQUIRE((c->flags & ~(SED_NET_AUX_FIRST | SED_NET_NO_GATE | SED_NET_DIRECT_CONV)) == 0, "net: unknown flags 0x%x", c->flags);
    memset(L, 0, sizeof(*L));
    L->n_conv = c->n_conv; L->n_gru = c->n_gru; L->n_dense = c->n_dense;
    const int fm = c->conv_mode == 2 ? 0 : c->conv_mode;
    int bfl[SED_MAX_CONV] = {0};
    if (c->conv_mode == 2) {
        int Ci = c->Cin, Ti = c->T, Fi = c->F;
        int ok[SED_MAX_CONV] = {0};
        for (int l = 0; l < c->n_conv; ++l) {
            const int pf = c->pool_f[l], pt = c->pool_t[l];
            ok[l] = l > 0 && pf == 1 && pt == 2 && c->C[l] > 0 && Ti >= 2 && sed_conv3x3_bf16_eval_supported(c->B, Ci, Fi, Ti, c->C[l]);
            if (l == c->n_conv - 1 && (size_t)c->C[l] * Fi * sizeof(float) > 64 * 1024) ok[l] = 0;
            Ci = c->C[l]; Ti = pt > 0 ? Ti / pt : Ti; Fi = pf > 0 ? Fi / pf : Fi;
        }
        for (int l = c->n_conv - 1; l >= 0 && ok[l]; --l) bfl[l] = 1;
    }
    Carver cv;
    int Cin = c->Cin, T = c->T, F = c->F;
    size_t max_pool = 0, max_wgrad = 0, c1_ws = 64, c1_stat_ws = 64;
    int max_bn_rows = 0, maxC = 0;
    for (int l = 0; l < c->n_conv; ++l) {
        ConvL& q = L->cv[l];
        q.Cin = Cin; q.C = c->C[l]; q.T = T; q.F = F; q.pf = c->pool_f[l]; q.pt = c->pool_t[l];
        q.drop = c->drop_p[l]; q.nchw = (l == 0);
        SED_REQUIRE(q.C > 0 && q.C % 4 == 0, "net: conv channels C[%d]=%d must be a positive multiple of 4", l, q.C);
        SED_REQUIRE(q.pf >= 1 && q.pt >= 1 && T / q.pt >= 1 && F / q.pf >= 1,
                    "net: block %d: T=%d/F=%d smaller than the pool (%d,%d)", l, T, F, q.pt, q.pf);
        SED_REQUIRE(q.drop >= 0.f && q.drop < 1.f, "net: drop_p[%d]=%f out of [0,1)", l, q.drop);
        q.Tp = T / q.pt; q.Fp = F / q.pf;
        q.fused = (l == 0 && c->n_conv > 1 && sed_conv1_fused_supported(q.Cin, q.F, q.T, q.C, q.pf, q.pt)) ? 1 : 0;
        q.bf = bfl[l];
        if (l == 0 && !q.fused && c->n_conv > 1 && q.Cin <= 4 && fm == 0 &&
            sed_conv1_rgrad_supported(q.Cin, q.F, q.T, q.C, q.pf, q.pt) &&
            sed_conv3x3_dgrad_bnred_rows(c->B, c->C[1], q.F / q.pf, q.T / q.pt, q.C) > 0)
            q.fused = 1;
        const bool wino_ok = l > 0 && fm == 0 && !q.bf && !(c->flags & SED_NET_DIRECT_CONV);
        q.wino = (wino_ok && sed_conv3x3_wino_rows(c->B, q.Cin, q.F, q.T, q.C) > 0) ? 1 : 0;
        q.wino_d = (wino_ok && training && sed_conv3x3_wino_rows(c->B, q.C, q.F, q.T, q.Cin) > 0) ? 1 : 0;
        if (q.fused) {
            q.rows = 1;
            q.bn_rows = sed_conv1_fused_rows(c->B, q.T);
        } else {
            q.rows = q.wino ? sed_conv3x3_wino_rows(c->B, q.Cin, q.F, q.T, q.C) : sed_conv3x3_stat_rows(c->B, q.Cin, q.F, q.T, q.C, q.nchw);
            SED_REQUIRE(q.rows > 0, "net: conv block %d (Cin=%d C=%d F=%d) is not supported by any conv kernel", l, q.Cin, q.C, q.F);
            q.bn_rows = sed_bn_bwd_rows(c->B, q.T, q.pt);
        }
        q.ev = (!training && l > 0 && fm == 0 && !q.bf && q.pf == 1 && q.pt == 2 &&
                (q.wino || sed_conv3x3_bn_relu_pool_eval_supported(c->B, q.Cin, q.F, q.T, q.C))) ? 1 : 0;
        size_t nout = (q.fused || q.ev || q.bf) ? 64 : (size_t)c->B * q.T * q.F * q.C, npool = (size_t)c->B * q.Tp * q.Fp * q.C;
        L->wp_f[l] = cv.take(q.wino ? sed_conv3x3_wino_packed_floats(q.C, q.Cin) : q.bf ? (size_t)9 * q.C * q.Cin / 2 : (size_t)9 * q.C * q.Cin);
        L->wp_d[l] = cv.take(q.wino_d ? sed_conv3x3_wino_packed_floats(q.C, q.Cin) : (size_t)9 * q.C * q.Cin);
        L->conv_out[l] = cv.take(nout);
        L->stat[l] = cv.take((size_t)q.rows * 2 * q.C);
        L->mean[l] = cv.take(q.C); L->rstd[l] = cv.take(q.C); L->scale[l] = cv.take(q.C); L->shift[l] = cv.take(q.C);
        L->pooled[l] = cv.take(q.bf ? (npool + 1) / 2 : npool);
        L->bn_sums[l] = cv.take((size_t)2 * q.C);
        L->bias_f[l] = cv.take(q.C);
        if (npool > max_pool) max_pool = npool;
        if (q.fused) {
            q.rgrad = training && sed_conv1_rgrad_supported(q.Cin, q.F, q.T, q.C, q.pf, q.pt) ? 1 : 0;
            c1_ws = sed_conv1_bwd_apply_workspace_bytes(c->B, q.Cin, q.T, q.C) / sizeof(float);
            const size_t w2 = sed_conv1_bwd_wgrad_workspace_bytes(c->B, q.Cin, q.T, q.C) / sizeof(float);
            if (w2 > c1_ws) c1_ws = w2;
            const size_t sws = sed_conv1_stats_workspace_bytes(c->B, q.Cin, q.T) / sizeof(float);
            if (sws > c1_stat_ws) c1_stat_ws = sws;
        } else {
            size_t wg = sed_conv3x3_wgrad_workspace_bytes(c->B, q.Cin, q.F, q.T, q.C) / sizeof(float);
            if (l > 0) {
                const size_t zr = fm == 0 ? sed_conv3x3_wgrad_zero_row_bytes(c->B, q.Cin, q.F, q.T, q.C) / sizeof(float) : 0;
                if (l == 1) L->wgrad_zrow = zr;
                else if (zr != L->wgrad_zrow) L->wgrad_zrow = 0;
            }
            if (l == 0 && c->n_conv > 1) c1_ws = wg + 64;
            else if (wg > max_wgrad) max_wgrad = wg;
        }
        if (q.bn_rows > max_bn_rows) max_bn_rows = q.bn_rows;
        if (q.C > maxC) maxC = q.C;
        Cin = q.C; T = q.Tp; F = q.Fp;
    }
    for (int l = 1; l < c->n_conv; ++l) {
        const ConvL& q = L->cv[l];
        const int rr = (fm != 0) ? 0 : q.wino_d ? sed_conv3x3_wino_rows(c->B, q.C, q.F, q.T, q.Cin)
                                                           : sed_conv3x3_dgrad_bnred_rows(c->B, q.C, q.F, q.T, q.Cin);
        L->cv[l - 1].red_rows = rr;
        if (rr > max_bn_rows) max_bn_rows = rr;
        if (l == 1 && rr > 0 && L->cv[0].fused && L->cv[0].rgrad && L->cv[0].Cin <= 2) {
            const int gr = q.wino_d ? sed_conv3x3_wino_rg_rows(c->B, q.C, q.F, q.T, q.Cin, L->cv[0].Cin)
                                    : sed_conv3x3_dgrad_bnred_rg_rows(c->B, q.C, q.F, q.T, q.Cin, L->cv[0].Cin);
            L->cv[0].rg_rows = gr;
            const size_t need = (size_t)gr * q.Cin * (1 + 9 * L->cv[0].Cin);
            if (need > c1_ws) c1_ws = need;
        }
    }
    L->c1_stat_ws = cv.take(c1_stat_ws);
    L->c1_bits = L->cv[0].rgrad ? cv.take(((size_t)c->B * L->cv[0].Tp * L->cv[0].Fp * (L->cv[0].C / 4) + 3) / 4) : 0;
    L->c1_mom = L->cv[0].rgrad ? cv.take(2 * sed_conv1_moments_doubles(L->cv[0].Cin)) : 0;
    L->Tp = T; L->Fp = F; L->feat = Cin * F; L->M = c->B * T;
    const size_t M = (size_t)L->M;
    if (L->cv[c->n_conv - 1].ev && (size_t)L->feat * sizeof(float) > 64 * 1024) {
        ConvL& q = L->cv[c->n_conv - 1];
        q.ev = 0;
        L->conv_out[c->n_conv - 1] = cv.take((size_t)c->B * q.T * q.F * q.C);
    }
    L->proj_bf = L->cv[c->n_conv - 1].bf;
    L->wih_perm = ((L->cv[c->n_conv - 1].ev || L->proj_bf) && c->H[0] > 0) ? cv.take((size_t)6 * c->H[0] * L->feat / (L->proj_bf ? 2 : 1)) : 0;
    int in = L->feat, max2H = 0;
    for (int i = 0; i < c->n_gru; ++i) {
        int H = c->H[i];
        SED_REQUIRE(H > 0 && H % 4 == 0 && 3 * H <= 1024, "net: GRU hidden H[%d]=%d must be a multiple of 4 and <= 341", i, H);
        L->gr[i].in = in; L->gr[i].H = H;
        L->gi[i] = cv.take(M * 6 * H);
        L->gout[i] = cv.take(M * 2 * H);
        L->saved[i] = training ? cv.take(M * 10 * H) : 0;
        in = 2 * H;
        if (in > max2H) max2H = in;
    }
    for (int i = 0; i < c->n_gru; ++i) L->gru_ws[i] = cv.take((size_t)6 * c->H[i] * c->H[i]);
    size_t max_lin_ws = 0;
    for (int j = 0; j < c->n_dense; ++j) {
        SED_REQUIRE(c->D[j] > 0, "net: dense size D[%d]=%d", j, c->D[j]);
        L->dK[j] = in; L->dN[j] = c->D[j];
        L->act[j] = (j < c->n_dense - 1) ? cv.take(M * c->D[j]) : 0;
        size_t w = sed_linear_bwd_workspace_bytes(L->M, in, c->D[j]) / sizeof(float);
        if (w > max_lin_ws) max_lin_ws = w;
        in = c->D[j];
    }
    if (training) {
        L->bn_part = cv.take((size_t)max_bn_rows * 2 * maxC);
        L->sum_g = cv.take((size_t)2 * maxC); L->sum_gx = 0;
        L->dbias_part = cv.take((size_t)max_bn_rows * maxC);
        for (int l = 0; l < c->n_conv; ++l)
            L->dconv[l] = L->cv[l].fused ? 0 : cv.take((size_t)c->B * L->cv[l].T * L->cv[l].F * L->cv[l].C);
        size_t ga = max_pool > M * (size_t)L->feat ? max_pool : M * (size_t)L->feat;
        L->gradA = cv.take(ga);
        L->wg_arrive = cv.take(64);
        L->wgrad_ws = cv.take(max_wgrad + 64);
        L->wgrad_ws_aux = cv.take(max_wgrad + 64);
        L->c1_ws = cv.take(c1_ws);
        for (int i = 0; i < c->n_gru; ++i) {
            L->dgi[i] = cv.take(M * 6 * c->H[i]);
            L->dgh[i] = cv.take(M * 6 * c->H[i]);
        }
        for (int i = 0; i < c->n_gru; ++i) L->gru_bws[i] = cv.take(sed_gru_seq_bwd_workspace_bytes(c->B, c->H[i]) / sizeof(float));
        for (int i = 0; i < c->n_gru; ++i) L->dgout[i] = cv.take(M * 2 * c->H[i]);
        for (int j = 0; j < c->n_dense - 1; ++j) L->dact[j] = cv.take(M * c->D[j]);
        L->lin_ws = cv.take(max_lin_ws);
    }
    {
        size_t gw = 0;
        for (int i = 0; i < c->n_gru; ++i) {
            size_t f = sed_gemm_f32_workspace_bytes(L->M, 6 * c->H[i], L->gr[i].in) / sizeof(float);
            if (f > gw) gw = f;
            if (training) {
                size_t a = sed_gemm_f32_workspace_bytes(3 * c->H[i], c->H[i], L->M) / sizeof(float);
                size_t b = sed_gemm_f32_workspace_bytes(6 * c->H[i], L->gr[i].in, L->M) / sizeof(float);
                if (a > gw) gw = a;
                if (b > gw) gw = b;
            }
        }
        L->gemm_ws = cv.take(gw + 64);
        L->gemm_ws_aux = training ? cv.take(gw + 64) : 0;
    }
    L->total = cv.off;
    return 0;
}

inline uint64_t layer_seed(uint64_t seed, int l) { return seed + 0x9E3779B97F4A7C15ull * (uint64_t)(l + 1); }

}

extern "C" int sed_net_out_shape(const sed_net_cfg* cfg, int* Tp, int* Fp) {
    Layout L;
    SED_TRY(build_layout(cfg, 0, &L));
    if (Tp) *Tp = L.Tp;
    if (Fp) *Fp = L.Fp;
    return 0;
}

extern "C" size_t sed_net_workspace_bytes(const sed_net_cfg* cfg, int training) {
    Layout L;
    if (build_layout(cfg, training, &L) != 0) return 0;
    return L.total * sizeof(float);
}

static int forward_impl(const sed_net_cfg* c, const sed_net_params* p, const float* x, float* logits, void* workspace,
                        int training, uint64_t seed, const uint64_t* seed_dev, int pb, int pe, float count_scale, void* stream) {
    SED_REQUIRE(p && x && logits && workspace, "net_forward: null pointer");
    Layout L;
    SED_TRY(build_layout(c, training, &L));
    SED_REQUIRE(pb >= 0 && pe <= 2 * L.n_conv + 1 && pb < pe, "net_forward: bad phase range [%d,%d)", pb, pe);
    float* ws = (float*)workspace;
    const int B = c->B;
    SED_REQUIRE(c->conv_mode != 2 || (pb == 0 && pe == 2 * L.n_conv + 1), "net_forward: the bf16 inference plan (conv_mode 2) runs whole, not in phases");
    const bool eval_plan = !training && (c->conv_mode == 0 || c->conv_mode == 2) && pb == 0 && pe == 2 * L.n_conv + 1;
    if (!eval_plan)
        for (int l = 0; l < L.n_conv; ++l)
            SED_REQUIRE(!(L.cv[l].ev || L.cv[l].bf),
                        "net_forward: phases [%d,%d) of an inference layout whose conv block %d keeps no conv output (pooled in the conv epilogue); "
                        "run inference whole: sed_net_forward, or phases [0,%d)", pb, pe, l, 2 * L.n_conv + 1);
    const ConvL& qtop = L.cv[L.n_conv - 1];
    const bool wih_permuted = eval_plan && (qtop.ev || L.proj_bf) && L.wih_perm != 0;
    if (eval_plan) {
        const float* w[SED_MAX_CONV]; const float* bs[SED_MAX_CONV]; const float* gm[SED_MAX_CONV]; const float* bt[SED_MAX_CONV];
        const float* rm[SED_MAX_CONV]; const float* rv[SED_MAX_CONV];
        float* wf[SED_MAX_CONV]; float* sc[SED_MAX_CONV]; float* sh[SED_MAX_CONV]; float* bf[SED_MAX_CONV];
        int fold[SED_MAX_CONV], co[SED_MAX_CONV], ci[SED_MAX_CONV], wn[SED_MAX_CONV];
        void* wb[SED_MAX_CONV];
        for (int l = 0; l < L.n_conv; ++l) {
            SED_REQUIRE(p->conv_w[l] && p->conv_b[l] && p->bn_g[l] && p->bn_b[l] && p->bn_rm[l] && p->bn_rv[l],
                        "net_forward: missing parameters of conv block %d", l);
            w[l] = p->conv_w[l]; bs[l] = p->conv_b[l]; gm[l] = p->bn_g[l]; bt[l] = p->bn_b[l]; rm[l] = p->bn_rm[l]; rv[l] = p->bn_rv[l];
            wf[l] = ws + L.wp_f[l]; sc[l] = ws + L.scale[l]; sh[l] = ws + L.shift[l]; bf[l] = ws + L.bias_f[l];
            fold[l] = L.cv[l].ev || L.cv[l].bf; co[l] = L.cv[l].C; ci[l] = L.cv[l].Cin; wn[l] = L.cv[l].ev && L.cv[l].wino;
            wb[l] = L.cv[l].bf ? (void*)wf[l] : nullptr;
            if (L.cv[l].bf) wf[l] = nullptr;
        }
        if (wih_permuted) SED_REQUIRE(p->gru_wih[0][0] && p->gru_wih[0][1], "net_forward: missing parameters of GRU layer 0");
        SED_TRY(sed_internal_conv_pack_eval(L.n_conv, w, bs, gm, bt, rm, rv, c->bn_eps, wf, sc, sh, bf, fold, wn, co, ci,
                                            wih_permuted ? p->gru_wih[0][0] : nullptr, wih_permuted ? p->gru_wih[0][1] : nullptr,
                                            ws + L.wih_perm, 3 * L.gr[0].H, qtop.C, qtop.Fp, wb, L.proj_bf, stream));
        for (int l = 0; l < L.n_conv; ++l) {
            const ConvL& q = L.cv[l];
            const float* in = (l == 0) ? x : ws + L.pooled[l - 1];
            const int last = (l == L.n_conv - 1);
            if (q.bf) {
                SED_TRY(sed_conv3x3_bf16_bn_relu_pool_eval(in, l > 0 && L.cv[l - 1].bf, ws + L.wp_f[l], ws + L.bias_f[l], ws + L.pooled[l],
                                                           B, q.Cin, q.F, q.T, q.C, stream));
            } else if (q.fused) {
                SED_TRY(sed_conv1_bn_relu_pool_drop_fwd(in, ws + L.wp_f[l], p->conv_b[l], ws + L.scale[l], ws + L.shift[l], ws + L.pooled[l],
                                                        B, q.Cin, q.F, q.T, q.C, q.pf, q.pt, 0.f, 0, nullptr, nullptr, stream));
            } else if (q.ev && q.wino) {
                SED_TRY(sed_conv3x3_wino_bn_relu_pool_eval(in, ws + L.wp_f[l], ws + L.bias_f[l], ws + L.pooled[l], B, q.Cin, q.F, q.T, q.C, stream));
            } else if (q.ev) {
                SED_TRY(sed_conv3x3_bn_relu_pool_eval(in, ws + L.wp_f[l], ws + L.bias_f[l], ws + L.pooled[l], B, q.Cin, q.F, q.T, q.C, stream));
            } else {
                SED_TRY(sed_conv3x3_fwd_ex(in, q.nchw, ws + L.wp_f[l], p->conv_b[l], ws + L.conv_out[l], nullptr, B, q.Cin, q.F, q.T, q.C, 0, stream));
                SED_TRY(sed_bn_relu_pool_drop_fwd(ws + L.conv_out[l], ws + L.scale[l], ws + L.shift[l], ws + L.pooled[l], B,
                                                  q.T, q.F, q.C, q.pf, q.pt, last, 0.f, 0, nullptr, stream));
            }
        }
    }
    const bool packed_up_front = !eval_plan && pb == 0 && c->conv_mode == 0 && L.n_conv > 1;
    const bool gru_packed_up_front = packed_up_front && pe > 2 * L.n_conv;
    if (packed_up_front) {
        const float* w[SED_MAX_CONV]; float* wf[SED_MAX_CONV]; float* wd[SED_MAX_CONV]; int co[SED_MAX_CONV], ci[SED_MAX_CONV];
        int wnf[SED_MAX_CONV], wnd[SED_MAX_CONV];
        for (int l = 0; l < L.n_conv; ++l) {
            SED_REQUIRE(p->conv_w[l], "net_forward: missing parameters of conv block %d", l);
            w[l] = p->conv_w[l]; wf[l] = ws + L.wp_f[l]; wd[l] = (training && l > 0) ? ws + L.wp_d[l] : nullptr;
            co[l] = L.cv[l].C; ci[l] = L.cv[l].Cin; wnf[l] = L.cv[l].wino; wnd[l] = L.cv[l].wino_d;
        }
        const float* whh[2 * SED_MAX_GRU]; float* whh_t[SED_MAX_GRU]; int gh[SED_MAX_GRU];
        for (int i = 0; i < L.n_gru && gru_packed_up_front; ++i) {
            SED_REQUIRE(p->gru_whh[i][0] && p->gru_whh[i][1], "net_forward: missing parameters of GRU layer %d", i);
            whh[2 * i] = p->gru_whh[i][0]; whh[2 * i + 1] = p->gru_whh[i][1]; whh_t[i] = ws + L.gru_ws[i]; gh[i] = L.gr[i].H;
        }
        SED_TRY(sed_internal_conv_pack_multi_gru(L.n_conv, w, wf, wd, co, ci, wnf, wnd, gru_packed_up_front ? L.n_gru : 0, whh, whh_t, gh, stream));
    }
    for (int l = 0; l < L.n_conv && !eval_plan; ++l) {
        const ConvL& q = L.cv[l];
        const float* in = (l == 0) ? x : ws + L.pooled[l - 1];
        const bool do_a = pb <= 2 * l && 2 * l < pe, do_b = pb <= 2 * l + 1 && 2 * l + 1 < pe;
        if (!do_a && !do_b) continue;
        const bool one_shot = do_a && do_b && count_scale == 1.f;
        const bool stats_with_bn = training && one_shot && q.fused && q.Cin <= 2;
        SED_REQUIRE(p->conv_w[l] && p->conv_b[l] && p->bn_g[l] && p->bn_b[l] && p->bn_rm[l] && p->bn_rv[l],
                    "net_forward: missing parameters of conv block %d", l);
        if (do_a) {
            if (!packed_up_front) {
                float* const wdp = (training && l > 0) ? ws + L.wp_d[l] : nullptr;
                if (q.wino || (q.wino_d && wdp))
                    SED_TRY(sed_conv3x3_wino_pack_weights(p->conv_w[l], q.wino ? ws + L.wp_f[l] : nullptr, q.wino_d ? wdp : nullptr, q.C, q.Cin, stream));
                if (!q.wino || (wdp && !q.wino_d))
                    SED_TRY(sed_conv3x3_pack_weights_ex(p->conv_w[l], q.wino ? nullptr : ws + L.wp_f[l], q.wino_d ? nullptr : wdp,
                                                        q.C, q.Cin, (l > 0) ? c->conv_mode : 0, stream));
            }
            if (q.fused) {
                if (training && stats_with_bn)
                    SED_TRY(sed_internal_conv1_stats_bn(in, ws + L.wp_f[l], p->conv_b[l], ws + L.stat[l], ws + L.c1_stat_ws, B, q.Cin, q.F, q.T, q.C,
                                                        q.rgrad ? (double*)(ws + L.c1_mom) : nullptr, p->bn_g[l], p->bn_b[l], p->bn_rm[l], p->bn_rv[l],
                                                        c->bn_momentum, c->bn_eps, ws + L.mean[l], ws + L.rstd[l], ws + L.scale[l], ws + L.shift[l], stream));
                else if (training)
                    SED_TRY(sed_conv1_stats(in, ws + L.wp_f[l], p->conv_b[l], ws + L.stat[l], ws + L.c1_stat_ws, B, q.Cin, q.F, q.T, q.C,
                                            q.rgrad ? (double*)(ws + L.c1_mom) : nullptr, stream));
            } else if (q.wino) {
                SED_TRY(sed_conv3x3_wino_fwd(in, ws + L.wp_f[l], p->conv_b[l], ws + L.conv_out[l], training ? ws + L.stat[l] : nullptr,
                                             B, q.Cin, q.F, q.T, q.C, stream));
            } else {
                SED_TRY(sed_conv3x3_fwd_ex(in, q.nchw, ws + L.wp_f[l], p->conv_b[l], ws + L.conv_out[l],
                                           training ? ws + L.stat[l] : nullptr, B, q.Cin, q.F, q.T, q.C, (l > 0) ? c->conv_mode : 0, stream));
            }
            if (training && !one_shot) SED_TRY(sed_bn_stat_sums(ws + L.stat[l], q.rows, q.C, ws + L.bn_sums[l], stream));
        }
        if (!do_b) continue;
        const double count = (double)B * q.T * q.F;
        if (stats_with_bn) {
        } else if (training && one_shot)
            SED_TRY(sed_bn_finalize_train(ws + L.stat[l], q.rows, q.C, count, p->bn_g[l], p->bn_b[l],
                                          p->bn_rm[l], p->bn_rv[l], c->bn_momentum, c->bn_eps, ws + L.mean[l],
                                          ws + L.rstd[l], ws + L.scale[l], ws + L.shift[l], stream));
        else if (training)
            SED_TRY(sed_bn_finalize_from_sums(ws + L.bn_sums[l], q.C, count * (double)count_scale, p->bn_g[l], p->bn_b[l],
                                              p->bn_rm[l], p->bn_rv[l], c->bn_momentum, c->bn_eps, ws + L.mean[l],
                                              ws + L.rstd[l], ws + L.scale[l], ws + L.shift[l], stream));
        else
            SED_TRY(sed_bn_finalize_eval(p->bn_g[l], p->bn_b[l], p->bn_rm[l], p->bn_rv[l], c->bn_eps, q.C,
                                         ws + L.scale[l], ws + L.shift[l], stream));
        const int last = (l == L.n_conv - 1);
        if (q.fused)
            SED_TRY(sed_conv1_bn_relu_pool_drop_fwd(in, ws + L.wp_f[l], p->conv_b[l], ws + L.scale[l], ws + L.shift[l],
                                                    ws + L.pooled[l], B, q.Cin, q.F, q.T, q.C, q.pf, q.pt,
                                                    training ? q.drop : 0.f, layer_seed(seed, l), seed_dev,
                                                    (training && q.rgrad) ? (unsigned char*)(ws + L.c1_bits) : nullptr, stream));
        else
            SED_TRY(sed_bn_relu_pool_drop_fwd(ws + L.conv_out[l], ws + L.scale[l], ws + L.shift[l], ws + L.pooled[l], B,
                                              q.T, q.F, q.C, q.pf, q.pt, last, training ? q.drop : 0.f,
                                              layer_seed(seed, l), seed_dev, stream));
    }
    if (pe <= 2 * L.n_conv) return 0;
    const int M = L.M;
    const float* gin = ws + L.pooled[L.n_conv - 1];
    for (int i = 0; i < L.n_gru; ++i) {
        const int H = L.gr[i].H, K = L.gr[i].in;
        for (int d = 0; d < 2; ++d)
            SED_REQUIRE(p->gru_wih[i][d] && p->gru_whh[i][d] && p->gru_bih[i][d] && p->gru_bhh[i][d],
                        "net_forward: missing parameters of GRU layer %d dir %d", i, d);
        const float* wih[2] = {p->gru_wih[i][0], p->gru_wih[i][1]};
        if (i == 0 && wih_permuted) { wih[0] = ws + L.wih_perm; wih[1] = wih[0] + (size_t)3 * H * K; }
        const bool fused = wih[1] == wih[0] + (size_t)3 * H * K && p->gru_bih[i][1] == p->gru_bih[i][0] + 3 * H;
        if (i == 0 && eval_plan && L.proj_bf) {
            const void* wb16 = (const void*)(ws + L.wih_perm);
            if (p->gru_bih[i][1] == p->gru_bih[i][0] + 3 * H) {
                SED_TRY(sed_gemm_bf16_nt(gin, wb16, p->gru_bih[i][0], ws + L.gi[i], 6 * H, M, 6 * H, K, stream));
            } else {
                for (int d = 0; d < 2; ++d)
                    SED_TRY(sed_gemm_bf16_nt(gin, (const void*)((const uint16_t*)wb16 + (size_t)d * 3 * H * K), p->gru_bih[i][d],
                                             ws + L.gi[i] + d * 3 * H, 6 * H, M, 3 * H, K, stream));
            }
        } else if (fused) {
            SED_TRY(sed_gemm_f32_ws(gin, K, 1, wih[0], 1, K, ws + L.gi[i], 6 * H, p->gru_bih[i][0], M, 6 * H, K, ws + L.gemm_ws, stream));
        } else {
            for (int d = 0; d < 2; ++d)
                SED_TRY(sed_gemm_f32(gin, K, 1, wih[d], 1, K, ws + L.gi[i] + d * 3 * H, 6 * H,
                                     p->gru_bih[i][d], 0.f, M, 3 * H, K, stream));
        }
        const float* whh[2] = {p->gru_whh[i][0], p->gru_whh[i][1]};
        const float* bhh[2] = {p->gru_bhh[i][0], p->gru_bhh[i][1]};
        if (gru_packed_up_front)
            SED_TRY(sed_internal_gru_seq_fwd_packed(ws + L.gi[i], ws + L.gru_ws[i], bhh, ws + L.gout[i], training ? ws + L.saved[i] : nullptr,
                                                    B, L.Tp, H, stream));
        else
            SED_TRY(sed_gru_seq_fwd(ws + L.gi[i], whh, bhh, ws + L.gout[i], training ? ws + L.saved[i] : nullptr,
                                    ws + L.gru_ws[i], B, L.Tp, H, stream));
        gin = ws + L.gout[i];
    }
    const float* din = gin;
    for (int j = 0; j < L.n_dense; ++j) {
        SED_REQUIRE(p->dense_w[j] && p->dense_b[j], "net_forward: missing parameters of dense layer %d", j);
        const int last = (j == L.n_dense - 1);
        float* y = last ? logits : ws + L.act[j];
        SED_TRY(sed_linear_fwd(din, p->dense_w[j], p->dense_b[j], y, M, L.dK[j], L.dN[j], !last, stream));
        din = y;
    }
    return 0;
}

extern "C" int sed_net_forward(const sed_net_cfg* c, const sed_net_params* p, const float* x, float* logits,
                               void* workspace, int training, uint64_t seed, const uint64_t* seed_dev, void* stream) {
    return forward_impl(c, p, x, logits, workspace, training, seed, seed_dev, 0, 2 * (c ? c->n_conv : 0) + 1, 1.f, stream);
}

extern "C" int sed_net_forward_phases(const sed_net_cfg* c, const sed_net_params* p, const float* x, float* logits,
                                      void* workspace, int training, uint64_t seed, int phase_begin, int phase_end,
                                      float count_scale, void* stream) {
    SED_REQUIRE(count_scale >= 1.f, "net_forward_phases: count_scale must be >= 1");
    SED_REQUIRE(!c || c->conv_mode != 2, "net_forward_phases: conv_mode 2 (bf16 inference) has no phases; run it with sed_net_forward, training = 0");
    return forward_impl(c, p, x, logits, workspace, training, seed, nullptr, phase_begin, phase_end, count_scale, stream);
}

extern "C" int sed_net_sync_region(const sed_net_cfg* c, int backward, int block, size_t* offset_bytes, size_t* n_floats) {
    Layout L;
    SED_TRY(build_layout(c, 1, &L));
    SED_REQUIRE(block >= 0 && block < L.n_conv && offset_bytes && n_floats, "net_sync_region: bad arguments");
    *offset_bytes = (backward ? L.sum_g : L.bn_sums[block]) * sizeof(float);
    *n_floats = (size_t)2 * L.cv[block].C;
    return 0;
}

extern "C" int sed_net_workspace_region(const sed_net_cfg* c, int training, const char* name, int index,
                                        size_t* offset_bytes, size_t* n_floats) {
    Layout L;
    SED_TRY(build_layout(c, training, &L));
    SED_REQUIRE(name && offset_bytes && n_floats, "net_workspace_region: null pointer");
    const bool conv_idx = index >= 0 && index < L.n_conv, gru_idx = index >= 0 && index < L.n_gru;
    size_t off = 0, n = 0;
    bool ok = false;
    auto is = [&](const char* q) { return strcmp(name, q) == 0; };
    if (conv_idx) {
        const ConvL& q = L.cv[index];
        const size_t nout = (size_t)c->B * q.T * q.F * q.C, npool = (size_t)c->B * q.Tp * q.Fp * q.C;
        if (is("conv_out") && !q.fused && !q.ev && !q.bf) { off = L.conv_out[index]; n = nout; ok = true; }
        else if (is("pooled")) { off = L.pooled[index]; n = npool; ok = true; }
        else if (is("mean")) { off = L.mean[index]; n = q.C; ok = true; }
        else if (is("rstd")) { off = L.rstd[index]; n = q.C; ok = true; }
        else if (is("scale")) { off = L.scale[index]; n = q.C; ok = true; }
        else if (is("shift")) { off = L.shift[index]; n = q.C; ok = true; }
        else if (is("dconv") && training && !q.fused) { off = L.dconv[index]; n = nout; ok = true; }
    }
    if (!ok && gru_idx) {
        const size_t M = (size_t)L.M, H = L.gr[index].H;
        if (is("gi")) { off = L.gi[index]; n = M * 6 * H; ok = true; }
        else if (is("gru_out")) { off = L.gout[index]; n = M * 2 * H; ok = true; }
        else if (is("dgru_out") && training) { off = L.dgout[index]; n = M * 2 * H; ok = true; }
        else if (is("gru_whh_t")) { off = L.gru_ws[index]; n = 6 * H * H; ok = true; }
        else if (is("gru_bias_part") && training) { off = L.gru_bws[index]; n = sed_gru_seq_bwd_workspace_bytes(c->B, (int)H) / sizeof(float); ok = true; }
    }
    if (!ok && training && index == 0) {
        if (is("grad_act")) {
            off = L.gradA;
            size_t mp = 0;
            for (int l = 0; l < L.n_conv; ++l) {
                const size_t np = (size_t)c->B * L.cv[l].Tp * L.cv[l].Fp * L.cv[l].C;
                if (np > mp) mp = np;
            }
            n = mp > (size_t)L.M * L.feat ? mp : (size_t)L.M * L.feat;
            ok = true;
        } else if (is("bn_sums_bwd")) { off = L.sum_g; n = 2 * (size_t)L.cv[0].C; ok = true; }
    }
    if (!ok && training && (index == 0 || index == 1) && is("wgrad_zero_row") && L.wgrad_zrow > 0) {
        off = index ? L.wgrad_ws_aux : L.wgrad_ws; n = L.wgrad_zrow; ok = true;
    }
    SED_REQUIRE(ok, "net_workspace_region: no region '%s'[%d] in this plan (training=%d)", name, index, training);
    *offset_bytes = off * sizeof(float);
    *n_floats = n;
    return 0;
}

extern "C" int sed_net_inference_plan(const sed_net_cfg* c, int* conv_bf16, int* proj_bf16) {
    Layout L;
    SED_TRY(build_layout(c, 0, &L));
    SED_REQUIRE(conv_bf16 && proj_bf16, "net_inference_plan: null pointer");
    for (int l = 0; l < L.n_conv; ++l) conv_bf16[l] = L.cv[l].bf;
    *proj_bf16 = L.proj_bf;
    return 0;
}

extern "C" int sed_net_routing(const sed_net_cfg* c, const sed_net_params* p, const float* x, const void* workspace, int block,
                               unsigned char* route, void* stream) {
    SED_REQUIRE(p && x && workspace && route, "net_routing: null pointer");
    Layout L;
    SED_TRY(build_layout(c, 1, &L));
    SED_REQUIRE(block >= 0 && block < L.n_conv, "net_routing: block %d out of range", block);
    const float* ws = (const float*)workspace;
    const ConvL& q = L.cv[block];
    if (q.fused) {
        SED_REQUIRE(p->conv_b[block], "net_routing: missing parameters of conv block %d", block);
        return sed_conv1_route(x, ws + L.wp_f[block], p->conv_b[block], ws + L.scale[block], ws + L.shift[block], route,
                               c->B, q.Cin, q.F, q.T, q.C, q.pf, q.pt, stream);
    }
    return sed_bn_relu_pool_route(ws + L.conv_out[block], ws + L.scale[block], ws + L.shift[block], route,
                                  c->B, q.T, q.F, q.C, q.pf, q.pt, stream);
}

static int bn_backward(const Layout& L, const sed_net_cfg* c, const sed_net_params* p, const sed_net_params* g,
                       const float* x, float* ws, uint64_t seed, const uint64_t* seed_dev, int l, int part, float count_scale, void* st) {
    const ConvL& q = L.cv[l];
    const int B = c->B, last = (l == L.n_conv - 1);
    const uint64_t sd = layer_seed(seed, l);
    SED_REQUIRE(g->conv_w[l] && g->conv_b[l] && g->bn_g[l] && g->bn_b[l], "net_backward: missing gradient buffers of conv block %d", l);
    float* sum_g = ws + L.sum_g;
    float* sum_gx = sum_g + q.C;
    if ((part & 1) && q.red_rows > 0 && !q.fused) {
        SED_TRY(sed_bn_bwd_finalize_small_gamma(ws + L.bn_part, q.red_rows, q.C, sum_g, sum_gx, g->bn_g[l], g->bn_b[l], ws + L.gradA,
                                                ws + L.pooled[l], ws + L.conv_out[l], p->bn_g[l], p->bn_b[l], ws + L.mean[l], ws + L.rstd[l],
                                                ws + L.scale[l], ws + L.shift[l], B, q.T, q.F, q.pf, q.pt, q.drop, st));
    } else if ((part & 1) && q.red_rows > 0) {
        SED_TRY(sed_bn_bwd_finalize(ws + L.bn_part, q.red_rows, q.C, sum_g, sum_gx, g->bn_g[l], g->bn_b[l], st));
    } else if (part & 1) {
        if (q.fused)
            SED_TRY(sed_conv1_bwd_reduce(x, ws + L.wp_f[l], p->conv_b[l], ws + L.gradA, ws + L.scale[l], ws + L.shift[l],
                                         ws + L.mean[l], ws + L.rstd[l], ws + L.bn_part, B, q.Cin, q.F, q.T, q.C, q.pf, q.pt,
                                         q.drop, sd, seed_dev, st));
        else if (sed_bn_bwd_reduce_pooled_supported(q.F, q.C, q.pf, q.pt, last))
            SED_TRY(sed_bn_bwd_reduce_pooled(ws + L.pooled[l], ws + L.gradA, p->bn_g[l], p->bn_b[l], ws + L.conv_out[l],
                                             ws + L.mean[l], ws + L.rstd[l], ws + L.scale[l], ws + L.shift[l], ws + L.bn_part, B, q.T, q.F, q.C, q.pf, q.pt, last, q.drop, st));
        else
            SED_TRY(sed_bn_relu_pool_drop_bwd_reduce(ws + L.conv_out[l], ws + L.gradA, ws + L.scale[l], ws + L.shift[l],
                                                     ws + L.mean[l], ws + L.rstd[l], ws + L.bn_part, B, q.T, q.F, q.C, q.pf,
                                                     q.pt, last, q.drop, sd, seed_dev, st));
        SED_TRY(sed_bn_bwd_finalize(ws + L.bn_part, q.bn_rows, q.C, sum_g, sum_gx, g->bn_g[l], g->bn_b[l], st));
    }
    if (part & 2) {
        if (count_scale != 1.f) SED_TRY(sed_scale(sum_g, 2 * q.C, 1.f / count_scale, st));
        if (q.fused && q.rgrad && q.rg_rows > 0) {
            SED_TRY(sed_conv1_bwd_wgrad_assemble(ws + L.c1_ws, q.rg_rows, (const double*)(ws + L.c1_mom), ws + L.wp_f[l], p->conv_b[l],
                                                 ws + L.mean[l], ws + L.rstd[l], ws + L.scale[l], sum_g, count_scale == 1.f ? nullptr : sum_gx, g->conv_w[l], g->conv_b[l],
                                                 B, q.Cin, q.F, q.T, q.C, p->bn_g[l], p->bn_b[l], g->bn_g[l], st));
        } else if (q.fused && q.rgrad) {
            SED_TRY(sed_conv1_bwd_wgrad(x, ws + L.gradA, ws + L.pooled[l], (const unsigned char*)(ws + L.c1_bits), (const double*)(ws + L.c1_mom),
                                        ws + L.wp_f[l], p->conv_b[l], ws + L.mean[l], ws + L.rstd[l], ws + L.scale[l], sum_g,
                                        (count_scale == 1.f && q.red_rows > 0) ? nullptr : sum_gx,
                                        g->conv_w[l], g->conv_b[l], ws + L.c1_ws, B, q.Cin, q.F, q.T, q.C, q.drop,
                                        q.red_rows > 0 ? p->bn_g[l] : nullptr, q.red_rows > 0 ? p->bn_b[l] : nullptr,
                                        q.red_rows > 0 ? g->bn_g[l] : nullptr, st));
        } else if (q.fused) {
            SED_TRY(sed_conv1_bwd_apply_wgrad(x, ws + L.wp_f[l], p->conv_b[l], ws + L.gradA, ws + L.scale[l], ws + L.shift[l],
                                              ws + L.mean[l], ws + L.rstd[l], sum_g, sum_gx, g->conv_w[l], g->conv_b[l],
                                              ws + L.c1_ws, B, q.Cin, q.F, q.T, q.C, q.pf, q.pt, q.drop, sd, seed_dev,
                                              q.red_rows > 0 ? p->bn_g[l] : nullptr, q.red_rows > 0 ? p->bn_b[l] : nullptr,
                                              q.red_rows > 0 ? g->bn_g[l] : nullptr, st));
        } else {
            SED_TRY(sed_bn_relu_pool_drop_bwd_apply(ws + L.conv_out[l], ws + L.gradA, ws + L.scale[l], ws + L.shift[l],
                                                    ws + L.mean[l], ws + L.rstd[l], sum_g, sum_gx, ws + L.dconv[l],
                                                    ws + L.dbias_part, B, q.T, q.F, q.C, q.pf, q.pt, last, q.drop, sd, seed_dev, st));
            SED_TRY(sed_reduce_rows(ws + L.dbias_part, q.bn_rows, q.C, q.C, g->conv_b[l], st));
        }
    }
    return 0;
}

static int dgrad(const Layout& L, const sed_net_cfg* c, const sed_net_params* p, const float* x, float* ws, int l, void* st) {
    const ConvL& q = L.cv[l];
    const ConvL& u = L.cv[l - 1];
    if (u.rg_rows > 0 && q.wino_d)
        return sed_conv3x3_wino_dgrad_bnred_rg(ws + L.dconv[l], ws + L.wp_d[l], (u.fused && u.rgrad && u.rg_rows > 0) ? nullptr : ws + L.gradA, ws + L.bn_part, ws + L.pooled[l - 1],
                                               p->bn_g[l - 1], p->bn_b[l - 1], ws + L.mean[l - 1], ws + L.rstd[l - 1], u.drop,
                                               x, u.Cin, (const unsigned char*)(ws + L.c1_bits), ws + L.c1_ws, c->B, q.C, q.F, q.T, q.Cin, st);
    if (u.rg_rows > 0)
        return sed_conv3x3_dgrad_bnred_rg(ws + L.dconv[l], ws + L.wp_d[l], ws + L.gradA, ws + L.bn_part, ws + L.pooled[l - 1],
                                          p->bn_g[l - 1], p->bn_b[l - 1], ws + L.mean[l - 1], ws + L.rstd[l - 1], u.drop,
                                          x, u.Cin, (const unsigned char*)(ws + L.c1_bits), ws + L.c1_ws, c->B, q.C, q.F, q.T, q.Cin, st);
    if (q.wino_d)
        return sed_conv3x3_wino_dgrad_bnred(ws + L.dconv[l], ws + L.wp_d[l], ws + L.gradA, ws + L.bn_part, ws + L.pooled[l - 1],
                                            p->bn_g[l - 1], p->bn_b[l - 1], u.fused ? nullptr : ws + L.conv_out[l - 1],
                                            ws + L.mean[l - 1], ws + L.rstd[l - 1], u.drop, u.pf, u.pt, u.F, u.T, c->B, q.C, q.F, q.T, q.Cin, st);
    if (u.red_rows > 0)
        return sed_conv3x3_dgrad_bnred(ws + L.dconv[l], ws + L.wp_d[l], ws + L.gradA, ws + L.bn_part, ws + L.pooled[l - 1],
                                       p->bn_g[l - 1], p->bn_b[l - 1],
                                       u.fused ? nullptr : ws + L.conv_out[l - 1],
                                       ws + L.mean[l - 1], ws + L.rstd[l - 1],
                                       u.drop, u.pf, u.pt, u.F, u.T, c->B, q.C, q.F, q.T, q.Cin, st);
    return sed_conv3x3_fwd_ex(ws + L.dconv[l], 0, ws + L.wp_d[l], nullptr, ws + L.gradA, nullptr, c->B, q.C, q.F, q.T, q.Cin, c->conv_mode, st);
}

extern "C" int sed_net_backward(const sed_net_cfg* c, const sed_net_params* p, const sed_net_params* g,
                                const float* x, const float* dlogits, void* workspace, uint64_t seed,
                                const uint64_t* seed_dev, int stage_begin, int stage_end, void* stream, void* aux_stream) {
    SED_REQUIRE(p && g && x && dlogits && workspace, "net_backward: null pointer");
    constexpr int kMaxDev = 16;
    static thread_local hipEvent_t ev_all[kMaxDev][2][SED_MAX_CONV] = {};
    static thread_local hipEvent_t ev_gru_all[kMaxDev][SED_MAX_GRU + 6] = {};
    hipStream_t s_main = as_stream(stream), s_aux = as_stream(aux_stream);
    hipEvent_t* ev_dg = nullptr;
    hipEvent_t* ev_bn = nullptr;
    hipEvent_t* ev_gru = nullptr;
    if (s_aux && s_aux != s_main) {
        int dev = 0;
        if (hipGetDevice(&dev) != hipSuccess || dev < 0 || dev >= kMaxDev) {
            sed_set_error("net_backward: device index %d outside [0,%d)", dev, kMaxDev);
            return SED_EINVAL;
// ... 257 lines not shown
```

### sed_crnn_amd/csrc/wino.hip

```cpp
#include "common.h"
#include "conv_shared.h"
#include <type_traits>

#define WN_CIN 128
#define WN_NHMAX 14

typedef __attribute__((address_space(1))) const void* sed_gptr_t;
typedef __attribute__((address_space(3))) void* sed_lptr_t;

struct WinoGeo {
    int Fw;
    int ncg, Tw, ntile, nblk, TR, F2, H2, HR, nb8, ncoh, NH;
    float invFw, invF2;
    size_t lds;
    unsigned long long* dbg;
};

__global__ void conv_pack_wino_k(const float* __restrict__ w, float* __restrict__ uf, float* __restrict__ ud, int Cout, int Cin,
                                 const float* __restrict__ bias, const float* __restrict__ gamma, const float* __restrict__ beta,
                                 const float* __restrict__ rm, const float* __restrict__ rv, float eps, float* __restrict__ bias_out) {
    const int i = blockIdx.x * blockDim.x + threadIdx.x;
    if (gamma && i < Cout) {
        const float sc = gamma[i] / sqrtf(rv[i] + eps);
        bias_out[i] = (bias ? bias[i] : 0.f) * sc + (beta[i] - rm[i] * sc);
// ... 166 lines not shown
            const bool in = f >= 0 && f < F && t >= 0 && t < br.Ty;
#pragma unroll
            for (int ci = 0; ci < RGC; ++ci)
                xs[ci * (F + 2) * XT + i] = in ? br.x1[(((size_t)b * RGC + ci) * F + f) * br.Ty + t] : 0.f;
        }
    }

    f32x16 acc[4][2][2];
#pragma unroll
    for (int nu = 0; nu < 4; ++nu)
#pragma unroll
        for (int mt = 0; mt < 2; ++mt)
#pragma unroll
            for (int nt = 0; nt < 2; ++nt)
#pragma unroll
                for (int j = 0; j < 16; ++j) acc[nu][mt][nt][j] = 0.f;

    const f32x4* wl = (const f32x4*)uq + (size_t)(coh * 16 + wave * 4) * (NCHUNK * 4 * 2 * 64);
    f32x4 bq[4][2];
    const unsigned lane16 = (unsigned)lane * 16u;
    auto load_b = [&](int nu, int st) {
#pragma unroll
        for (int nt = 0; nt < 2; ++nt)
            bq[nu][nt] = *(const f32x4*)((const char*)(wl + ((nu * NSTEP + st) * 2 + nt) * 64) + lane16);
    };
    static_assert(NH <= 16, "the patch DMA of a slice rides in every fourth slot of its first step");
    f32x2 vp[2][2][4][2];
    f32x4 raw[2][2][4];
    f32x2 up[2][4][2];
    const f32x2 sg2 = {sg, sg};
    auto slot_read = [&](const float* buf, int g, int i) {
        const int mt = i >> 3, s2 = (i >> 2) & 1, c = i & 3;
        raw[mt][s2][c] = *(const f32x4*)(buf + aoff[mt][s2][c] + g * 64);
    };
    auto slot_xform = [&](int k, f32x2 (&v)[2][4][2]) {
        const int mt = k >> 4, q = k & 15, hf = q & 1;
        if (q < 8) {
            const int c = q >> 1;
            const f32x2 da = hf ? __builtin_shufflevector(raw[mt][0][c], raw[mt][0][c], 2, 3) : __builtin_shufflevector(raw[mt][0][c], raw[mt][0][c], 0, 1);
            const f32x2 db = hf ? __builtin_shufflevector(raw[mt][1][c], raw[mt][1][c], 2, 3) : __builtin_shufflevector(raw[mt][1][c], raw[mt][1][c], 0, 1);
            up[mt][c][hf] = wn_pk_fma(sg2, db, da);
        } else {
            const int nu = (q - 8) >> 1;
            if (nu == 0) v[mt][0][hf] = wn_pk_sub(up[mt][0][hf], up[mt][2][hf]);
            else if (nu == 1) v[mt][1][hf] = wn_pk_add(up[mt][1][hf], up[mt][2][hf]);
            else if (nu == 2) v[mt][2][hf] = wn_pk_sub(up[mt][2][hf], up[mt][1][hf]);
            else v[mt][3][hf] = wn_pk_sub(up[mt][1][hf], up[mt][3][hf]);
        }
    };
    constexpr int PF = RGC == 2 ? 2 : 4;
    int rq = 0, c4 = 0, cb = 0;
    const char* qb = nullptr;
    const unsigned char* bitq = nullptr;
    unsigned rstride = 0, cstride = 0;
    unsigned rov[4] = {0, 0, 0, 0};
    f32x4 pqv[PF][BNR ? 4 : 1];
    unsigned btv[PF][RG ? 4 : 1];
    f32x4 q_beta = {0, 0, 0, 0}, gm = {0, 0, 0, 0};
#define WN_EPI_LANE() do { rq = lane >> 3; c4 = (lane & 7) * 4; cb = co0 + nt * 32 + c4; } while (0)
#define WN_EPI_STRIDES() do { rstride = (unsigned)(F * Cout) * 4u; cstride = (unsigned)Cout * 4u; } while (0)
#define WN_EPI_ROWS() do { _Pragma("unroll") for (int k = 0; k < 4; ++k) rov[k] = rowtab[mt * 32 + rq + 8 * k]; } while (0)
    auto epi_setup = [&]() {
        const int mt = wave >> 1, nt = wave & 1;
        WN_EPI_LANE();
        qb = (const char*)(br.pooled + (size_t)b * T * F * Cout + cb);
        bitq = RG ? br.bits + (size_t)b * T * F * (Cout >> 2) + (cb >> 2) : nullptr;
        WN_EPI_STRIDES();
        WN_EPI_ROWS();
    };
    auto prefetch_one = [&](int k, int n, f32x4* pqd, unsigned* btd) {
        if (!BNR) return;
        const unsigned off = rov[k] != 0xFFFFFFFFu ? rov[k] + (n & 1) * rstride + (n >> 1) * cstride : 0u;
        pqd[n] = *(const f32x4*)(qb + off);
        if (RG) btd[n] = bitq[off >> 4];
    };

#pragma unroll
    for (int nu = 0; nu < 4; ++nu) load_b(nu, 0);
    __syncthreads();
#pragma unroll
    for (int i = 0; i < 16; ++i) slot_read(smem, 0, i);
#pragma unroll
    for (int k = 0; k < 32; ++k) slot_xform(k, vp[0]);
    if (geo.dbg) tk1 = __builtin_amdgcn_s_memrealtime();
#pragma unroll
    for (int st = 0; st < (BNR ? NSTEP - 1 : NSTEP); ++st) {
        const int cc = st >> 2, g = st & 3, par = st & 1;
        const bool more = cc + 1 < NCHUNK, nxt = st + 1 < NSTEP;
        const float* nbuf = smem + (((st + 1) >> 2) & 1) * HBUF;
        __builtin_amdgcn_sched_barrier(0);
#pragma unroll
        for (int i = 0; i < 64; ++i) {
            const int nu = i >> 4, j = (i >> 2) & 3, mt = (i >> 1) & 1, nt = i & 1;
            acc[nu][mt][nt] = __builtin_amdgcn_mfma_f32_32x32x2f32(vp[par][mt][nu][j >> 1][j & 1], bq[nu][nt][j], acc[nu][mt][nt], 0, 0, 0);
            if (nxt && !(ABL & 4)) {
                if (i < 16) slot_read(nbuf, (st + 1) & 3, i);
                else if (i < 48 && !(ABL & 1)) slot_xform(i - 16, vp[par ^ 1]);
            }
            if (nxt && (i & 15) == 15 && !(ABL & 2)) load_b(nu, st + 1);
            if (g == 0 && more && !(ABL & 8) && (i & 3) == 1 && (i >> 2) < NH) issue_one(cc + 1, smem + ((cc + 1) & 1) * HBUF, i >> 2);
            __builtin_amdgcn_sched_barrier(0);
        }
        if (nxt && (ABL & 5)) {
#pragma unroll
            for (int a = 0; a < 2; ++a)
#pragma unroll
                for (int c = 0; c < 4; ++c) { vp[par ^ 1][a][c][0] = vp[par][a][c][0]; vp[par ^ 1][a][c][1] = vp[par][a][c][1]; }
        }
        if (g == 2 && more) __syncthreads();
    }
    if (BNR) {
        constexpr int par = (NSTEP - 1) & 1;
        epi_setup();
        __builtin_amdgcn_sched_barrier(0);
#pragma unroll
        for (int i = 0; i < 64; ++i) {
            const int nu = i >> 4, j = (i >> 2) & 3, mt = (i >> 1) & 1, nt = i & 1;
            acc[nu][mt][nt] = __builtin_amdgcn_mfma_f32_32x32x2f32(vp[par][mt][nu][j >> 1][j & 1], bq[nu][nt][j], acc[nu][mt][nt], 0, 0, 0);
            if (i < 4 * (PF == 4 ? 4 : 2)) prefetch_one(i >> 2, i & 3, pqv[i >> 2], btv[i >> 2]);
            else if (i == 16) q_beta = *(const f32x4*)(br.beta + cb);
            else if (i == 17) gm = *(const f32x4*)(br.gamma + cb);
            __builtin_amdgcn_sched_barrier(0);
        }
    }
    __syncthreads();
    if (geo.dbg) tk2 = __builtin_amdgcn_s_memrealtime();

#pragma unroll
    for (int mt = 0; mt < 2; ++mt)
#pragma unroll
        for (int nt = 0; nt < 2; ++nt) {
            if (BNR) {
#pragma unroll
                for (int nu = 0; nu < 4; ++nu) asm volatile("" : "+a"(acc[nu][mt][nt]));
            }
            const f32x16 z0 = acc[0][mt][nt] + acc[1][mt][nt] + acc[2][mt][nt];
            const f32x16 z1 = acc[1][mt][nt] - acc[2][mt][nt] - acc[3][mt][nt];
            float* zb0 = smem + ((((wave * 2 + 0) * 2 + mt) * 2 + nt) << 10);
            float* zb1 = smem + ((((wave * 2 + 1) * 2 + mt) * 2 + nt) << 10);
#pragma unroll
            for (int j = 0; j < 16; ++j) {
                const int row = (j & 3) + 8 * (j >> 2) + 4 * h;
                zb0[row * 32 + r] = z0[j];
                zb1[row * 32 + r] = z1[j];
            }
            if (BNR) __builtin_amdgcn_sched_barrier(0);
        }
    __builtin_amdgcn_sched_barrier(0);
    const int mt = wave >> 1, nt = wave & 1;
    if (!BNR) WN_EPI_LANE();
    f32x4 bv = {0, 0, 0, 0};
    if (bias) bv = *(const f32x4*)(bias + cb);
    char* const yb = (char*)(y + (size_t)b * (EV ? T >> 1 : T) * F * Cout + cb);
    f32x4 q_kr = {0, 0, 0, 0}, q_nb = {0, 0, 0, 0}, a1 = {0, 0, 0, 0}, a2 = {0, 0, 0, 0};
    if (BNR) {
#pragma unroll
        for (int e = 0; e < 4; ++e) {
            const bool zero = gm[e] == 0.f || (br.ybelow != nullptr && fabsf(gm[e]) * 64.f < fabsf(q_beta[e]));
            const float rg = zero ? 0.f : 1.0f / gm[e];
            q_kr[e] = br.keep * rg;
            q_nb[e] = -q_beta[e] * rg;
        }
    }
    if (!BNR) WN_EPI_STRIDES();
    f32x4 R[RG ? 9 * RGC : 1];
#pragma unroll
    for (int k = 0; k < (RG ? 9 * RGC : 1); ++k) R[k] = (f32x4){0, 0, 0, 0};
    if (!BNR) WN_EPI_ROWS();
    unsigned xov[4];
#pragma unroll
    for (int k = 0; k < 4; ++k) xov[k] = RG ? xofftab[mt * 32 + rq + 8 * k] : 0u;
    auto prefetch = [&](int k, f32x4* pqd, unsigned* btd) {
#pragma unroll
        for (int n = 0; n < 4; ++n) prefetch_one(k, n, pqd, btd);
    };
    const bool wr_y = !RG || y != nullptr;

    __syncthreads();
    unsigned long long tkx = 0;
    if (BNR && geo.dbg) tkx = __builtin_amdgcn_s_memrealtime();
#pragma unroll
    for (int k = 0; k < 4; ++k) {
        const int m = rq + 8 * k;
        const unsigned ro = rov[k];
        if (PF == 2 && k >= 1 && k + 1 < 4) prefetch(k + 1, pqv[(k + 1) & 1], btv[(k + 1) & 1]);
        if (ro == 0xFFFFFFFFu) continue;
        const unsigned xo = xov[k];
#pragma unroll
        for (int jj = 0; jj < 2; ++jj) {
            f32x4 z[4];
#pragma unroll
            for (int xi = 0; xi < 4; ++xi) z[xi] = *(const f32x4*)(smem + ((((xi * 2 + jj) * 2 + mt) * 2 + nt) << 10) + m * 32 + c4);
            const f32x4 o[2] = {z[0] + z[1] + z[2] + bv, z[1] - z[2] - z[3] + bv};
            if (EV) {
                f32x4 pl;
#pragma unroll
                for (int e = 0; e < 4; ++e) pl[e] = fmaxf(fmaxf(o[0][e], o[1][e]), 0.f);
                *(f32x4*)(yb + ro + jj * cstride) = pl;
                continue;
            }
#pragma unroll
            for (int i = 0; i < 2; ++i) {
                const unsigned off = ro + i * rstride + jj * cstride;
                const f32x4 v = o[i];
                if (wr_y) *(f32x4*)(yb + off) = v;
                if (BNR) {
                    const f32x4 pq = pqv[k & (PF - 1)][jj * 2 + i];
                    f32x4 g0;
#pragma unroll
                    for (int e = 0; e < 4; ++e) g0[e] = pq[e] > 0.f ? v[e] : 0.f;
                    a1 += g0;
                    a2 += g0 * (pq * q_kr + q_nb);
                    if (RG) {
                        const unsigned bt = btv[k & (PF - 1)][jj * 2 + i];
                        f32x4 g1;
#pragma unroll
                        for (int e = 0; e < 4; ++e) g1[e] = ((bt >> e) & 1u) ? g0[e] : 0.f;
                        const f32x4 gA = g0 - g1;
#pragma unroll
                        for (int ci = 0; ci < RGC; ++ci) {
                            const float* xb = xs + ci * (F + 2) * XT + xo + jj * XT + 2 * i;
#pragma unroll
                            for (int kh = 0; kh < 3; ++kh) {
                                const f32x2 x01 = *(const f32x2*)(xb + kh * XT), x23 = *(const f32x2*)(xb + kh * XT + 2);
                                R[(kh * 3 + 0) * RGC + ci] += gA * x01[0] + g1 * x01[1];
                                R[(kh * 3 + 1) * RGC + ci] += gA * x01[1] + g1 * x23[0];
                                R[(kh * 3 + 2) * RGC + ci] += gA * x23[0] + g1 * x23[1];
                            }
                        }
                    }
                } else {
                    a1 += v;
                    a2 += v * v;
                }
            }
        }
    }
    if (stat && !EV) {
        float* red = smem + 32768;
        if (BNR) { a1 *= br.inv_keep; a2 *= br.inv_keep; }
#pragma unroll
        for (int e = 0; e < 4; ++e) {
#pragma unroll
            for (int o = 8; o < 64; o <<= 1) { a1[e] += __shfl_xor(a1[e], o, 64); a2[e] += __shfl_xor(a2[e], o, 64); }
        }
        if (lane < 8) {
            *(f32x4*)(red + (wave * 2 + 0) * 32 + c4) = a1;
            *(f32x4*)(red + (wave * 2 + 1) * 32 + c4) = a2;
        }
        float* red2 = xs + RGC * (F + 2) * XT;
        if (RG) {
#pragma unroll
            for (int k = 0; k < 9 * RGC; ++k) {
                R[k] *= br.inv_keep;
#pragma unroll
                for (int e = 0; e < 4; ++e) {
#pragma unroll
                    for (int o = 8; o < 64; o <<= 1) R[k][e] += __shfl_xor(R[k][e], o, 64);
                }
                if (lane < 8) *(f32x4*)(red2 + (wave * 9 * RGC + k) * 32 + c4) = R[k];
            }
        }
        __syncthreads();
        const size_t row = (size_t)b * geo.nblk * geo.ncg + blka;
        if (tid < 128) {
            const int which = tid >> 6, c = tid & 63, cn = c >> 5, cr = c & 31;
            const float a = red[((0 * 2 + cn) * 2 + which) * 32 + cr] + red[((1 * 2 + cn) * 2 + which) * 32 + cr];
            stat[row * 2 * Cout + which * Cout + co0 + c] = a;
        }
        if (RG && tid < 64) {
            const int cn = tid >> 5, cr = tid & 31;
            float* o = br.rgp + (row * Cout + co0 + tid) * (1 + 9 * RGC);
            o[0] = red[((0 * 2 + cn) * 2 + 0) * 32 + cr] + red[((1 * 2 + cn) * 2 + 0) * 32 + cr];
#pragma unroll
            for (int k = 0; k < 9 * RGC; ++k)
                o[1 + k] = red2[((0 * 2 + cn) * 9 * RGC + k) * 32 + cr] + red2[((1 * 2 + cn) * 9 * RGC + k) * 32 + cr];
        }
    }
    if (geo.dbg && tid == 0) {
        const unsigned long long tk3 = __builtin_amdgcn_s_memrealtime();
        atomicAdd(geo.dbg + 0, tk1 - tk0);
        atomicAdd(geo.dbg + 1, tk2 - tk1);
        atomicAdd(geo.dbg + 2, tk3 - tk2);
        atomicAdd(geo.dbg + 3, 1ull);
        if (BNR) atomicAdd(geo.dbg + 4, tkx - tk2);
    }
}

#undef WN_EPI_LANE
#undef WN_EPI_STRIDES
#undef WN_EPI_ROWS

template <typename K>
static int wino_set_lds(K kernel, size_t bytes) {
    hipError_t e = hipFuncSetAttribute((const void*)kernel, hipFuncAttributeMaxDynamicSharedMemorySize, (int)bytes);
    if (e != hipSuccess) { sed_set_error("hipFuncSetAttribute(%zu B LDS): %s", bytes, hipGetErrorString(e)); return (int)e; }
    return 0;
}

static unsigned long long* g_wino_dbg = nullptr;
#ifdef WN_ABLATION
static int g_wino_abl = 0;
extern "C" int sed_conv3x3_wino_ablate(int mask) { g_wino_abl = mask; return 0; }
#endif
extern "C" int sed_conv3x3_wino_phase_ticks(unsigned long long* buf) { g_wino_dbg = buf; return 0; }

int sed_internal_wino_launch(const float* x, const float* uq, const float* bias, float* y, float* stat, const ConvBnRed* br,
                             int rgc, int B, int Cin, int F, int T, int Cout, hipStream_t s) {
    WinoGeo g;
    SED_REQUIRE(wino_geo(B, Cin, F, T, Cout, &g), "conv3x3_wino: shape B=%d Cin=%d F=%d T=%d Cout=%d is not supported (sed_conv3x3_wino_rows)", B, Cin, F, T, Cout);
    SED_REQUIRE(rgc >= -1 && rgc <= 2 && (rgc <= 0 || (br && br->x1 && br->bits && br->rgp)) && (rgc >= 0 || (!br && !stat)), "conv3x3_wino: bad epilogue arguments");
    g.dbg = g_wino_dbg;
    if (rgc > 0) {
        g.lds += ((size_t)64 + (size_t)rgc * (F + 2) * (4 * g.TR + 2) + (size_t)4 * 9 * rgc * 32) * sizeof(float);
        SED_REQUIRE(g.lds <= 160 * 1024, "conv3x3_wino: the first block's input patch does not fit the LDS (F=%d)", F);
    }
    const dim3 grid(g.nblk * g.ncg * g.ncoh, B);
    const ConvBnRed none{};
#define WN_LAUNCH(NHv, BNRv, RGv, EVv)                                                                                          \
    do {                                                                                                                           \
        SED_TRY(wino_set_lds((conv3x3_wino_k<NHv, BNRv, RGv, EVv>), g.lds));                                                       \
        conv3x3_wino_k<NHv, BNRv, RGv, EVv><<<grid, 256, g.lds, s>>>(x, uq, bias, y, stat, B, F, T, Cout, g, br ? *br : none);     \
    } while (0)
#ifdef WN_ABLATION
    if (g_wino_abl && rgc == 0 && !br) {
        switch (g_wino_abl) {
            case 1: { SED_TRY(wino_set_lds((conv3x3_wino_k<WN_NHMAX, false, 0, false, 1>), g.lds)); conv3x3_wino_k<WN_NHMAX, false, 0, false, 1><<<grid, 256, g.lds, s>>>(x, uq, bias, y, stat, B, F, T, Cout, g, none); break; }
            case 2: { SED_TRY(wino_set_lds((conv3x3_wino_k<WN_NHMAX, false, 0, false, 2>), g.lds)); conv3x3_wino_k<WN_NHMAX, false, 0, false, 2><<<grid, 256, g.lds, s>>>(x, uq, bias, y, stat, B, F, T, Cout, g, none); break; }
            case 4: { SED_TRY(wino_set_lds((conv3x3_wino_k<WN_NHMAX, false, 0, false, 5>), g.lds)); conv3x3_wino_k<WN_NHMAX, false, 0, false, 5><<<grid, 256, g.lds, s>>>(x, uq, bias, y, stat, B, F, T, Cout, g, none); break; }
            case 8: { SED_TRY(wino_set_lds((conv3x3_wino_k<WN_NHMAX, false, 0, false, 8>), g.lds)); conv3x3_wino_k<WN_NHMAX, false, 0, false, 8><<<grid, 256, g.lds, s>>>(x, uq, bias, y, stat, B, F, T, Cout, g, none); break; }
            default: { SED_TRY(wino_set_lds((conv3x3_wino_k<WN_NHMAX, false, 0, false, 15>), g.lds)); conv3x3_wino_k<WN_NHMAX, false, 0, false, 15><<<grid, 256, g.lds, s>>>(x, uq, bias, y, stat, B, F, T, Cout, g, none); break; }
        }
        SED_LAUNCH_CHECK("conv3x3_wino (ablation)");
        return 0;
    }
#endif
    if (rgc == 1) WN_LAUNCH(WN_NHMAX, true, 1, false);
    else if (rgc == 2) WN_LAUNCH(WN_NHMAX, true, 2, false);
    else if (rgc == -1) WN_LAUNCH(WN_NHMAX, false, 0, true);
    else if (br) WN_LAUNCH(WN_NHMAX, true, 0, false);
    else WN_LAUNCH(WN_NHMAX, false, 0, false);
#undef WN_LAUNCH
    SED_LAUNCH_CHECK("conv3x3_wino");
    return 0;
}

extern "C" int sed_conv3x3_wino_rows(int B, int Cin, int F, int T, int Cout) { return sed_internal_wino_rows(B, Cin, F, T, Cout); }

extern "C" int sed_conv3x3_wino_fwd(const float* x, const float* uq, const float* bias, float* y, float* stat,
                                    int B, int Cin, int F, int T, int Cout, void* stream) {
    SED_REQUIRE(x && uq && y, "conv3x3_wino_fwd: null pointer");
    hipStream_t s = as_stream(stream);
    SedProfScope prof(SED_K_CONV_MFMA_FWD, s, 2.0 * 9.0 * Cin * Cout * (double)B * T * F);
    return sed_internal_wino_launch(x, uq, bias, y, stat, nullptr, 0, B, Cin, F, T, Cout, s);
}

extern "C" int sed_conv3x3_wino_dgrad_bnred(const float* dy, const float* ud, float* dx, float* partials, const float* pooled,
                                            const float* gamma, const float* beta, const float* conv_out_below, const float* mean,
                                            const float* rstd, float drop_p, int pool_f, int pool_t, int Fy, int Ty,
                                            int B, int C, int F, int T, int Cin, void* stream) {
    SED_REQUIRE(dy && ud && dx && partials && pooled && gamma && beta && mean && rstd, "conv3x3_wino_dgrad_bnred: null pointer");
    SED_REQUIRE(drop_p >= 0.f && drop_p < 1.f && pool_f >= 1 && pool_t >= 1, "conv3x3_wino_dgrad_bnred: bad drop_p / pool");
    SED_REQUIRE(Ty / pool_t == T && Fy / pool_f == F, "conv3x3_wino_dgrad_bnred: conv output %dx%d does not pool (%d,%d) to %dx%d", Ty, Fy, pool_f, pool_t, T, F);
    hipStream_t s = as_stream(stream);
    SedProfScope prof(SED_K_CONV_MFMA_DGRAD, s, 2.0 * 9.0 * C * Cin * (double)B * T * F);
    const ConvBnRed br{pooled, gamma, beta, conv_out_below, mean, rstd, 1.f - drop_p, 1.f / (1.f - drop_p), pool_f, pool_t, Fy, Ty,
                       nullptr, nullptr, nullptr, 0.f};
    return sed_internal_wino_launch(dy, ud, nullptr, dx, partials, &br, 0, B, C, F, T, Cin, s);
}

extern "C" int sed_conv3x3_wino_rg_rows(int B, int C, int F, int T, int Cin, int Cin1) {
    WinoGeo g;
    if (Cin1 < 1 || Cin1 > 2 || !wino_geo(B, C, F, T, Cin, &g)) return 0;
    const size_t lds = g.lds + ((size_t)64 + (size_t)Cin1 * (F + 2) * (4 * g.TR + 2) + (size_t)4 * 9 * Cin1 * 32) * sizeof(float);
    return lds <= 160 * 1024 ? B * g.nblk * g.ncg : 0;
}
extern "C" int sed_conv3x3_wino_dgrad_bnred_rg(const float* dy, const float* ud, float* dx, float* partials, const float* pooled,
                                               const float* gamma, const float* beta, const float* mean, const float* rstd, float drop_p,
                                               const float* x1, int Cin1, const unsigned char* argmax_bits, float* rg_partials,
                                               int B, int C, int F, int T, int Cin, void* stream) {
    SED_REQUIRE(dy && ud && partials && pooled && gamma && beta && mean && rstd && x1 && argmax_bits && rg_partials, "conv3x3_wino_dgrad_bnred_rg: null pointer");
    SED_REQUIRE(drop_p >= 0.f && drop_p < 1.f && (Cin1 == 1 || Cin1 == 2), "conv3x3_wino_dgrad_bnred_rg: bad drop_p / input channels");
    hipStream_t s = as_stream(stream);
    SedProfScope prof(SED_K_CONV_MFMA_DGRAD, s, 2.0 * 9.0 * C * Cin * (double)B * T * F);
    const ConvBnRed br{pooled, gamma, beta, nullptr, mean, rstd, 1.f - drop_p, 1.f / (1.f - drop_p), 1, 2, F, 2 * T,
                       x1, argmax_bits, rg_partials, 0.f};
    return sed_internal_wino_launch(dy, ud, nullptr, dx, partials, &br, Cin1, B, C, F, T, Cin, s);
}

extern "C" int sed_conv3x3_wino_bn_relu_pool_eval(const float* x, const float* uf_folded, const float* bias_folded, float* pooled,
                                                  int B, int Cin, int F, int T, int Cout, void* stream) {
    SED_REQUIRE(x && uf_folded && bias_folded && pooled, "conv3x3_wino_bn_relu_pool_eval: null pointer");
    hipStream_t s = as_stream(stream);
    SedProfScope prof(SED_K_CONV_MFMA_FWD, s, 2.0 * 9.0 * Cin * Cout * (double)B * T * F);
    return sed_internal_wino_launch(x, uf_folded, bias_folded, pooled, nullptr, nullptr, -1, B, Cin, F, T, Cout, s);
}
```

### sed_crnn_amd/model.py

```python
import ctypes as C
import math
import weakref

import torch
import torch.nn as nn

from . import _lib
from ._lib import NetCfg, NetParams, check, lib

_MASK64 = (1 << 64) - 1
_ARENA_OWNERS = weakref.WeakValueDictionary()


def arena_owner(param):
    try:
        m = _ARENA_OWNERS.get(param.untyped_storage().data_ptr())
    except Exception:
        return None
    if m is not None and any(q is param for q in m._arena_params):
        return m
    return None


class ConvParams(nn.Module):
# ... 171 lines not shown
        place(order)
        stage_ends.append(off)
        for l in range(nconv - 1, -1, -1):
            ps = [r["conv_w"][l], r["conv_b"][l], r["bn_g"][l], r["bn_b"][l]]
            order += ps
            place(ps)
            stage_ends.append(off)
        dev = order[0].device
        flat = torch.zeros(off, device=dev, dtype=torch.float32)
        flat_g = torch.zeros(off, device=dev, dtype=torch.float32)
        views = []
        with torch.no_grad():
            for p, o in zip(order, offs):
                n = p.numel()
                flat[o:o + n].copy_(p.detach().reshape(-1))
                p.data = flat[o:o + n].view(p.shape)
                views.append(flat_g[o:o + n].view(p.shape))
                p.grad = None
        assert len(order) == len(list(self.parameters())), "every parameter must have a role"
        self._arena, self._arena_grad = flat, flat_g
        _ARENA_OWNERS[flat.untyped_storage().data_ptr()] = self
        self._arena_params, self._grad_views, self._arena_offsets = order, views, offs
        self._stage_ends = stage_ends
        self._structs = None
        self._ws = {}
        self._ws_pinned = set()
        self._arena_dirty = False
        self._last = None
        if self._bound_grads:
            self.bind_flat_grads()

    def _apply(self, fn, *a, **k):
        super()._apply(fn, *a, **k)
        if hasattr(self, "_arena_params"):
            self._flatten()
        return self

    def __getstate__(self):
        st = self.__dict__.copy()
        for k in ("_structs", "_ws", "_aux_stream", "_last", "_arena", "_arena_grad", "_arena_params", "_grad_views",
                  "_arena_offsets", "_stage_ends"):
            st.pop(k, None)
        return st

    def __setstate__(self, st):
        self.__dict__.update(st)
        self._structs, self._ws, self._aux_stream, self._arena = None, {}, None, None
        with torch.no_grad():
            for p_ in self.parameters():
                p_.data = p_.data.clone()
        self._flatten()

    def flat_parameters(self):
        return self._arena

    def flat_grads(self):
        return self._arena_grad

    def bucket_slices(self):
        b = [0] + self._stage_ends
        n = len(self.conv_channels)
        cfg = self._cfg(1, self.time_factor)
        ready = [lib().sed_net_backward_ready_stage(C.byref(cfg), n - s) for s in range(1, n + 1)]
        out = [(b[0], b[1])]
        for st in range(1, n + 1):
            mine = [s for s in range(1, n + 1) if ready[s - 1] == st]
            out.append((b[mine[0]], b[mine[-1] + 1]) if mine else (b[st], b[st]))
        return out

    def bind_flat_grads(self):
        self._bound_grads = True
        for p, g in zip(self._arena_params, self._grad_views):
            p.grad = g if p.requires_grad else None

    def zero_grad(self, set_to_none=True):
        self._arena_dirty = False
        return super().zero_grad(set_to_none)

    def _alias_mask(self, aliased):
        if all(aliased):
            return None
        m = torch.zeros_like(self._arena_grad)
        for p, o, al in zip(self._arena_params, self._arena_offsets, aliased):
            if al:
                m[o:o + p.numel()] = 1.0
        return m

    def _cfg(self, B, T, training=True):
        c = NetCfg()
        c.B, c.Cin, c.F, c.T = B, self.in_channels, self.n_mels, T
        c.n_conv = len(self.conv_channels)
        for l, ch in enumerate(self.conv_channels):
            c.C[l] = ch
            c.pool_f[l], c.pool_t[l] = self.pools[l]
            c.drop_p[l] = float(self.drops[l])
        c.n_gru = len(self.gru_hidden)
        for i, h in enumerate(self.gru_hidden):
            c.H[i] = h
        c.n_dense = len(self.dense)
        for j, d in enumerate(self.dense):
            c.D[j] = d
        c.bn_eps, c.bn_momentum = self.bn_eps, self.bn_momentum
        c.conv_mode = int(getattr(self, "conv_mode", 0))
        if not training and getattr(self, "inference_precision", "f32") == "bf16":
            c.conv_mode = 2
        c.flags = int(getattr(self, "plan_flags", 0))
        return c

    def set_conv_precision(self, name="f32"):
        self.conv_mode = {"f32": 0, "bf16x3": 1}[name]
        return self

    def set_inference_precision(self, name="f32"):
        if name not in ("f32", "bf16"):
            raise ValueError(f"inference precision must be 'f32' or 'bf16', got {name!r}")
        self.inference_precision = name
        return self

    def inference_plan(self, B=1, T=None):
        T = int(T) if T is not None else 32 * self.time_factor
        cfg = self._cfg(int(B), T, training=False)
        cb, pj = (C.c_int * _lib.SED_MAX_CONV)(), C.c_int(0)
        check(lib().sed_net_inference_plan(C.byref(cfg), cb, C.byref(pj)), "sed_net_inference_plan")
        name = {0: "f32", 1: "bf16"}
        return {"conv": [name[cb[l]] for l in range(len(self.conv_channels))], "proj": name[pj.value]}

    def _param_structs(self):
        if self._structs is None:
            r = self._roles()
            gmap = {id(p): g for p, g in zip(self._arena_params, self._grad_views)}
            P, G = NetParams(), NetParams()

            def put(field, idx, t, grad=True):
                tgt_p, tgt_g = getattr(P, field), getattr(G, field)
                if isinstance(idx, tuple):
                    tgt_p[idx[0]][idx[1]] = t.data_ptr()
                    tgt_g[idx[0]][idx[1]] = gmap[id(t)].data_ptr() if grad else None
                else:
                    tgt_p[idx] = t.data_ptr()
                    tgt_g[idx] = gmap[id(t)].data_ptr() if grad else None
            for l in range(len(self.conv_channels)):
                put("conv_w", l, r["conv_w"][l]); put("conv_b", l, r["conv_b"][l])
                put("bn_g", l, r["bn_g"][l]); put("bn_b", l, r["bn_b"][l])
                put("bn_rm", l, r["bn_rm"][l], grad=False); put("bn_rv", l, r["bn_rv"][l], grad=False)
            for i in range(len(self.gru_hidden)):
                for d in range(2):
                    put("gru_wih", (i, d), r["gru_wih"][i][d]); put("gru_whh", (i, d), r["gru_whh"][i][d])
                    put("gru_bih", (i, d), r["gru_bih"][i][d]); put("gru_bhh", (i, d), r["gru_bhh"][i][d])
            for j in range(len(self.dense)):
                put("dense_w", j, r["dense_w"][j]); put("dense_b", j, r["dense_b"][j])
            self._structs = (P, G)
        return self._structs

    def _workspace(self, cfg, training):
        key = (cfg.B, cfg.T, bool(training))
        if cfg.conv_mode == 2:
            key = key + ("bf16",)
        ws = self._ws.get(key)
        if ws is None:
            nbytes = lib().sed_net_workspace_bytes(C.byref(cfg), int(training))
            if nbytes == 0:
                check(-1, "sed_net_workspace_bytes")
            ws = torch.empty(nbytes // 4 + 64, device=self._arena.device, dtype=torch.float32)
            while len(self._ws) - len(self._ws_pinned) >= 4:
                victim = next((k for k in self._ws if k not in self._ws_pinned), None)
                if victim is None:
                    break
                if self._last is not None and self._last[1] is self._ws[victim]:
                    self._last = None
                del self._ws[victim]
            self._ws[key] = ws
        return ws

    def pin_workspace(self, B, T, training=True):
        self._ws_pinned.add((int(B), int(T), bool(training)))

    def _check_input(self, x):
        if not (isinstance(x, torch.Tensor) and x.is_cuda):
            raise _lib.SedHipError("sed_crnn_amd runs on an MI355X only: input must be a CUDA(HIP) tensor "
                                   "(there is no CPU fallback; the CPU reference lives in oracle/ for tests)")
        if self._arena is None or not self._arena.is_cuda:
            raise _lib.SedHipError("sed_crnn_amd: move the module to the GPU first (model.to('cuda'))")
        if x.dim() != 4 or x.shape[1] != self.in_channels or x.shape[2] != self.n_mels:
            raise ValueError(f"expected input [B,{self.in_channels},{self.n_mels},T], got {tuple(x.shape)}")
        if x.shape[3] < self.time_factor:
            raise ValueError(f"T={x.shape[3]} is shorter than one output frame ({self.time_factor} input frames)")
        if not (x.dtype.is_floating_point or x.dtype in (torch.uint8, torch.int8, torch.int16, torch.int32, torch.int64)):
            raise ValueError(f"unsupported input dtype {x.dtype}")

    @staticmethod
    def _rank_salt():
        import torch.distributed as dist
        if dist.is_available() and dist.is_initialized():
            return dist.get_rank() * 0xA24BAED4963EE407
        return 0

    def _graph_seed(self):
        return (torch.initial_seed() * 0x9E3779B97F4A7C15 + 0x51ED270B + self._rank_salt()) & _MASK64

    def _next_seed(self):
        self._seed_counter += 1
        return (torch.initial_seed() * 0x9E3779B97F4A7C15 + self._seed_counter * 0xD1B54A32D192ED03 + self._rank_salt()) & _MASK64

    def enable_sync_bn(self, process_group=None, enabled=True):
        self._sync_bn, self._sync_group = bool(enabled), process_group
        return self

    def _sync_world(self):
        import torch.distributed as dist
        if self._sync_bn and dist.is_available() and dist.is_initialized():
            return dist.get_world_size(self._sync_group)
        return 1

    def _allreduce_region(self, cfg, ws, backward, block):
        import torch.distributed as dist
        off, n = C.c_size_t(), C.c_size_t()
        check(lib().sed_net_sync_region(C.byref(cfg), int(backward), block, C.byref(off), C.byref(n)), "sed_net_sync_region")
        dist.all_reduce(ws[off.value // 4: off.value // 4 + n.value], op=dist.ReduceOp.SUM, group=self._sync_group)

    def workspace_view(self, name, index=0):
        if self._last is None:
            raise RuntimeError("sed_crnn_amd: no training forward to look into")
        cfg, ws, _ = self._last
        off, n = C.c_size_t(), C.c_size_t()
        check(lib().sed_net_workspace_region(C.byref(cfg), 1, name.encode(), int(index), C.byref(off), C.byref(n)),
              "sed_net_workspace_region")
        return ws[off.value // 4: off.value // 4 + n.value]

    def eval_workspace_view(self, name, index=0):
        if getattr(self, "_last_eval", None) is None:
            raise RuntimeError("sed_crnn_amd: no eval forward to look into")
        cfg, ws = self._last_eval
        off, n = C.c_size_t(), C.c_size_t()
        check(lib().sed_net_workspace_region(C.byref(cfg), 0, name.encode(), int(index), C.byref(off), C.byref(n)),
              "sed_net_workspace_region")
        bf16 = False
        if name == "pooled" and cfg.conv_mode == 2:
            cb, pj = (C.c_int * _lib.SED_MAX_CONV)(), C.c_int(0)
            check(lib().sed_net_inference_plan(C.byref(cfg), cb, C.byref(pj)), "sed_net_inference_plan")
            bf16 = bool(cb[int(index)])
        o = off.value // 4
        if bf16:
            return ws[o: o + (n.value + 1) // 2].view(torch.bfloat16)[:n.value]
        return ws[o: o + n.value]

    def routing(self, block):
        if self._last is None:
            raise RuntimeError("sed_crnn_amd: no training forward to look into")
        cfg, ws, x = self._last
        P, _ = self._param_structs()
        T, F = cfg.T, cfg.F
        for l in range(block):
            T, F = T // self.pools[l][1], F // self.pools[l][0]
        pf, pt = self.pools[block]
        route = torch.empty(cfg.B, T // pt, F // pf, self.conv_channels[block], device=x.device, dtype=torch.uint8)
        check(lib().sed_net_routing(C.byref(cfg), C.byref(P), _lib.ptr(x), _lib.ptr(ws), int(block), _lib.ptr(route),
                                    _lib.stream_ptr()), "sed_net_routing")
        return route

    def _run_forward(self, x, training, step_state=None):
        self._check_input(x)
        x = x.detach().contiguous().float()
        B, _, _, T = x.shape
        cfg = self._cfg(B, T, training)
        P, _ = self._param_structs()
        ws = self._workspace(cfg, training)
        if not training:
            self._last_eval = (cfg, ws)
        logits = torch.empty(B, T // self.time_factor, self.dense[-1], device=x.device, dtype=torch.float32)
        if training:
            self._ticket += 1
            self._seed = self._next_seed() if step_state is None else self._graph_seed()
            self._nbt_pending += 1
            self._last = (cfg, ws, x)
            self._last_state = step_state
        seed = self._seed if training else 0
        world = self._sync_world() if training else 1
        if world > 1:
            args = (C.byref(cfg), C.byref(P), _lib.ptr(x), _lib.ptr(logits), _lib.ptr(ws), 1, seed)
            n = len(self.conv_channels)
            for l in range(n):
                check(lib().sed_net_forward_phases(*args, 2 * l, 2 * l + 1, float(world), _lib.stream_ptr()), "sed_net_forward_phases")
                self._allreduce_region(cfg, ws, 0, l)
                check(lib().sed_net_forward_phases(*args, 2 * l + 1, 2 * l + 2, float(world), _lib.stream_ptr()), "sed_net_forward_phases")
            check(lib().sed_net_forward_phases(*args, 2 * n, 2 * n + 1, float(world), _lib.stream_ptr()), "sed_net_forward_phases")
            return logits
        check(lib().sed_net_forward(C.byref(cfg), C.byref(P), _lib.ptr(x), _lib.ptr(logits), _lib.ptr(ws),
                                    int(training), seed, _lib.ptr(step_state) if training else None, _lib.stream_ptr()),
              "sed_net_forward")
        return logits

    def _run_backward(self, x, dlogits, stage_begin=0, stage_end=None):
        if self._last is None:
            raise RuntimeError("sed_crnn_amd: backward without a training forward (or its workspace was evicted)")
        cfg, ws, x = self._last
        P, G = self._param_structs()
        if stage_end is None:
            stage_end = len(self.conv_channels) + 1
        world = self._sync_world()
        if world > 1:
            args = (C.byref(cfg), C.byref(P), C.byref(G), _lib.ptr(x), _lib.ptr(dlogits), _lib.ptr(ws), self._seed)
            n = len(self.conv_channels)
            for s in range(stage_begin, stage_end):
                if s == 0:
                    check(lib().sed_net_backward_phases(*args, 0, 1, float(world), _lib.stream_ptr()), "sed_net_backward_phases")
                    continue
                k = s - 1
                check(lib().sed_net_backward_phases(*args, 2 * k + 1, 2 * k + 2, float(world), _lib.stream_ptr()), "sed_net_backward_phases")
                self._allreduce_region(cfg, ws, 1, n - 1 - k)
                check(lib().sed_net_backward_phases(*args, 2 * k + 2, 2 * k + 3, float(world), _lib.stream_ptr()), "sed_net_backward_phases")
            return
        if getattr(self, "_aux_stream", None) is None or self._aux_stream.device != x.device:
            self._aux_stream = torch.cuda.Stream(device=x.device)
        aux = C.c_void_p(self._aux_stream.cuda_stream) if self.overlap_wgrad else None
        check(lib().sed_net_backward(C.byref(cfg), C.byref(P), C.byref(G), _lib.ptr(x), _lib.ptr(dlogits),
                                     _lib.ptr(ws), self._seed, _lib.ptr(getattr(self, "_last_state", None)), stage_begin,
                                     stage_end, _lib.stream_ptr(), aux), "sed_net_backward")

    def forward(self, x):
        if self.training and torch.is_grad_enabled():
            return _NetFn.apply(self, x, *self._arena_params)
        return self._run_forward(x, training=self.training)

    def _flush_nbt(self):
        if self._nbt_pending:
            for m in self.modules():
                if isinstance(m, BNParams):
                    m.num_batches_tracked += self._nbt_pending
# ... 142 lines not shown
```

### sed_crnn_amd/ops.py

```python
import ctypes as C

import torch

from ._lib import check, lib, ptr, stream_ptr


def _f32c(t):
    assert t.is_cuda and t.dtype == torch.float32 and t.is_contiguous(), "expect contiguous fp32 CUDA tensor"
    return t


def conv3x3_pack(w, mode=0):
    Cout, Cin = w.shape[:2]
    wf = torch.empty(9, Cout, Cin, device=w.device)
    wd = torch.empty(9, Cin, Cout, device=w.device)
    check(lib().sed_conv3x3_pack_weights_ex(ptr(_f32c(w)), ptr(wf), ptr(wd), Cout, Cin, mode, stream_ptr()), "conv3x3_pack")
    return wf, wd


def conv3x3_fwd(x, wp, bias, x_is_nchw, want_stats=True, mode=0):
    if x_is_nchw:
        B, Cin, F, T = x.shape
    else:
        B, T, F, Cin = x.shape
    Cout = wp.shape[1]
    y = torch.empty(B, T, F, Cout, device=x.device)
    stat = None
    if want_stats:
        rows = lib().sed_conv3x3_stat_rows(B, Cin, F, T, Cout, int(x_is_nchw))
        stat = torch.zeros(max(rows, 1), 2, Cout, device=x.device)
    check(lib().sed_conv3x3_fwd_ex(ptr(_f32c(x)), int(x_is_nchw), ptr(_f32c(wp)), ptr(bias), ptr(y), ptr(stat),
                                   B, Cin, F, T, Cout, mode, stream_ptr()), "conv3x3_fwd")
    return y, stat


CONV_PLAN_FIELDS = ("kind", "TT", "FT", "nft", "nct", "tblocks", "rows", "xcd_order")


def conv3x3_plan(B, Cin, F, T, Cout, x_is_nchw=False, which=0):
    out = (C.c_int * 8)()
    check(lib().sed_conv3x3_plan(B, Cin, F, T, Cout, int(x_is_nchw), which, out), "conv3x3_plan")
    return dict(zip(CONV_PLAN_FIELDS, out))


def conv3x3_wino_pack(w):
    Cout, Cin = w.shape[:2]
    n = lib().sed_conv3x3_wino_packed_floats(Cout, Cin)
    uf, ud = torch.empty(n, device=w.device), torch.empty(n, device=w.device)
    check(lib().sed_conv3x3_wino_pack_weights(ptr(_f32c(w)), ptr(uf), ptr(ud), Cout, Cin, stream_ptr()), "conv3x3_wino_pack")
    return uf, ud


def conv3x3_wino_fwd(x, up, bias, Cout, want_stats=True):
    B, T, F, Cin = x.shape
    rows = lib().sed_conv3x3_wino_rows(B, Cin, F, T, Cout)
    if rows <= 0:
        raise ValueError("conv3x3_wino_fwd: shape not supported")
    y = torch.empty(B, T, F, Cout, device=x.device)
    stat = torch.zeros(rows, 2, Cout, device=x.device) if want_stats else None
    check(lib().sed_conv3x3_wino_fwd(ptr(_f32c(x)), ptr(_f32c(up)), ptr(bias), ptr(y), ptr(stat), B, Cin, F, T, Cout, stream_ptr()),
          "conv3x3_wino_fwd")
    return y, stat


def conv3x3_bn_relu_pool_eval(x, w, bias, gamma, beta, running_mean, running_var, eps=1e-5, wino=False):
    B, T, F, Cin = x.shape
    Cout = w.shape[0]
    if wino:
        if lib().sed_conv3x3_wino_rows(B, Cin, F, T, Cout) <= 0:
            raise ValueError("conv3x3_bn_relu_pool_eval: shape not supported by the Winograd kernel")
        uf = torch.empty(lib().sed_conv3x3_wino_packed_floats(Cout, Cin), device=x.device)
        bf = torch.empty(Cout, device=x.device)
        check(lib().sed_conv3x3_wino_pack_weights_bn_folded(ptr(_f32c(w)), ptr(bias), ptr(gamma), ptr(beta), ptr(running_mean), ptr(running_var),
                                                            eps, ptr(uf), ptr(bf), Cout, Cin, stream_ptr()), "conv3x3_wino_pack_weights_bn_folded")
        out = torch.empty(B, T // 2, F, Cout, device=x.device)
        check(lib().sed_conv3x3_wino_bn_relu_pool_eval(ptr(_f32c(x)), ptr(uf), ptr(bf), ptr(out), B, Cin, F, T, Cout, stream_ptr()),
              "conv3x3_wino_bn_relu_pool_eval")
        return out
    if not lib().sed_conv3x3_bn_relu_pool_eval_supported(B, Cin, F, T, Cout):
        raise ValueError("conv3x3_bn_relu_pool_eval: shape not supported")
    wf = torch.empty(9, Cout, Cin, device=x.device)
    bf = torch.empty(Cout, device=x.device)
    check(lib().sed_conv3x3_pack_weights_bn_folded(ptr(_f32c(w)), ptr(bias), ptr(gamma), ptr(beta), ptr(running_mean), ptr(running_var),
                                                   eps, ptr(wf), ptr(bf), Cout, Cin, stream_ptr()), "conv3x3_pack_weights_bn_folded")
    out = torch.empty(B, T // 2, F, Cout, device=x.device)
    check(lib().sed_conv3x3_bn_relu_pool_eval(ptr(_f32c(x)), ptr(wf), ptr(bf), ptr(out), B, Cin, F, T, Cout, stream_ptr()),
          "conv3x3_bn_relu_pool_eval")
    return out


def conv3x3_bf16_pack_folded(w, bias, gamma, beta, running_mean, running_var, eps=1e-5):
    Cout, Cin = w.shape[:2]
    wf = torch.empty(9 * Cout * Cin, device=w.device, dtype=torch.bfloat16)
    bf = torch.empty(Cout, device=w.device)
    check(lib().sed_conv3x3_bf16_pack_weights_bn_folded(ptr(_f32c(w)), ptr(bias), ptr(gamma), ptr(beta), ptr(running_mean),
                                                        ptr(running_var), eps, ptr(wf), ptr(bf), Cout, Cin, stream_ptr()),
          "conv3x3_bf16_pack_weights_bn_folded")
    return wf, bf


def conv3x3_bf16_bn_relu_pool_eval(x, wf, bias_folded, Cout):
    B, T, F, Cin = x.shape
    assert x.is_cuda and x.is_contiguous() and x.dtype in (torch.float32, torch.bfloat16)
    assert wf.dtype == torch.bfloat16 and wf.numel() == 9 * Cout * Cin
    if not lib().sed_conv3x3_bf16_eval_supported(B, Cin, F, T, Cout):
        raise ValueError(f"conv3x3_bf16_bn_relu_pool_eval: shape B={B} Cin={Cin} F={F} T={T} Cout={Cout} not supported")
    out = torch.empty(B, T // 2, F, Cout, device=x.device, dtype=torch.bfloat16)
    check(lib().sed_conv3x3_bf16_bn_relu_pool_eval(ptr(x), int(x.dtype == torch.bfloat16), ptr(wf), ptr(_f32c(bias_folded)), ptr(out),
                                                   B, Cin, F, T, Cout, stream_ptr()), "conv3x3_bf16_bn_relu_pool_eval")
    return out


def gemm_bf16_nt(A, B, bias=None):
    M, K = A.shape
    N = B.shape[0]
    assert A.dtype == torch.bfloat16 and B.dtype == torch.bfloat16 and A.is_contiguous() and B.is_contiguous() and B.shape[1] == K
    out = torch.empty(M, N, device=A.device)
    check(lib().sed_gemm_bf16_nt(ptr(A), ptr(B), ptr(bias), ptr(out), N, M, N, K, stream_ptr()), "gemm_bf16_nt")
    return out


def conv3x3_wgrad(x, dy, x_is_nchw, mode=0):
    if x_is_nchw:
        B, Cin, F, T = x.shape
    else:
        B, T, F, Cin = x.shape
    Cout = dy.shape[-1]
    nbytes = lib().sed_conv3x3_wgrad_workspace_bytes(B, Cin, F, T, Cout)
    ws = torch.empty(nbytes // 4 + 1, device=x.device)
    dw = torch.empty(Cout, Cin, 3, 3, device=x.device)
    check(lib().sed_conv3x3_wgrad_ex(ptr(_f32c(x)), int(x_is_nchw), ptr(_f32c(dy)), ptr(dw), ptr(ws),
                                     B, Cin, F, T, Cout, mode, stream_ptr()), "conv3x3_wgrad")
    return dw


def bn_finalize_train(stat, count, gamma, beta, running_mean, running_var, momentum=0.1, eps=1e-5):
    rows, _, Cc = stat.shape
    mean, rstd, scale, shift = (torch.empty(Cc, device=stat.device) for _ in range(4))
    check(lib().sed_bn_finalize_train(ptr(stat), rows, Cc, float(count), ptr(gamma), ptr(beta), ptr(running_mean),
                                      ptr(running_var), momentum, eps, ptr(mean), ptr(rstd), ptr(scale), ptr(shift),
                                      stream_ptr()), "bn_finalize_train")
    return mean, rstd, scale, shift


def bn_finalize_eval(gamma, beta, rm, rv, eps=1e-5):
    Cc = gamma.numel()
    scale, shift = torch.empty(Cc, device=gamma.device), torch.empty(Cc, device=gamma.device)
    check(lib().sed_bn_finalize_eval(ptr(gamma), ptr(beta), ptr(rm), ptr(rv), eps, Cc, ptr(scale), ptr(shift),
                                     stream_ptr()), "bn_finalize_eval")
    return scale, shift


def bn_relu_pool_drop_fwd(y, scale, shift, pool_f, pool_t, out_tcf=False, drop_p=0.0, seed=0):
    B, T, F, Cc = y.shape
    Tp, Fp = T // pool_t, F // pool_f
    out = torch.empty((B, Tp, Cc, Fp) if out_tcf else (B, Tp, Fp, Cc), device=y.device)
    check(lib().sed_bn_relu_pool_drop_fwd(ptr(_f32c(y)), ptr(scale), ptr(shift), ptr(out), B, T, F, Cc, pool_f, pool_t,
                                          int(out_tcf), drop_p, seed, None, stream_ptr()), "bn_relu_pool_drop_fwd")
    return out


def bn_relu_pool_drop_bwd(y, dout, scale, shift, mean, rstd, pool_f, pool_t, out_tcf=False, drop_p=0.0, seed=0):
    B, T, F, Cc = y.shape
    rows = lib().sed_bn_bwd_rows(B, T, pool_t)
    part = torch.empty(rows, 2, Cc, device=y.device)
    check(lib().sed_bn_relu_pool_drop_bwd_reduce(ptr(_f32c(y)), ptr(_f32c(dout)), ptr(scale), ptr(shift), ptr(mean),
                                                 ptr(rstd), ptr(part), B, T, F, Cc, pool_f, pool_t, int(out_tcf),
                                                 drop_p, seed, None, stream_ptr()), "bn_bwd_reduce")
    sum_g, sum_gx, dgamma, dbeta = (torch.empty(Cc, device=y.device) for _ in range(4))
    check(lib().sed_bn_bwd_finalize(ptr(part), rows, Cc, ptr(sum_g), ptr(sum_gx), ptr(dgamma), ptr(dbeta),
                                    stream_ptr()), "bn_bwd_finalize")
    dy = torch.empty_like(y)
    dbp = torch.empty(rows, Cc, device=y.device)
    check(lib().sed_bn_relu_pool_drop_bwd_apply(ptr(y), ptr(dout), ptr(scale), ptr(shift), ptr(mean), ptr(rstd),
                                                ptr(sum_g), ptr(sum_gx), ptr(dy), ptr(dbp), B, T, F, Cc, pool_f,
                                                pool_t, int(out_tcf), drop_p, seed, None, stream_ptr()), "bn_bwd_apply")
    dbias = torch.empty(Cc, device=y.device)
    check(lib().sed_reduce_rows(ptr(dbp), rows, Cc, Cc, ptr(dbias), stream_ptr()), "reduce_rows")
    return dy, dgamma, dbeta, dbias


def bn_bwd_sums_from_pooled(pooled, dout, gamma, beta, y, mean, rstd, pool_f, pool_t, drop_p=0.0, scale=None, shift=None):
    B, T, F, Cc = y.shape
    if not lib().sed_bn_bwd_reduce_pooled_supported(F, Cc, pool_f, pool_t, 1):
        raise ValueError("bn_bwd_sums_from_pooled: shape not supported")
    rows = lib().sed_bn_bwd_rows(B, T, pool_t)
    part = torch.empty(rows, 2, Cc, device=y.device)
    if scale is None:
        scale = gamma * rstd
        shift = beta - mean * scale
    check(lib().sed_bn_bwd_reduce_pooled(ptr(_f32c(pooled)), ptr(_f32c(dout)), ptr(gamma), ptr(beta), ptr(_f32c(y)), ptr(mean),
                                         ptr(rstd), ptr(scale), ptr(shift), ptr(part), B, T, F, Cc, pool_f, pool_t, 1, drop_p, stream_ptr()),
          "bn_bwd_reduce_pooled")
    sum_g, sum_gx = torch.empty(Cc, device=y.device), torch.empty(Cc, device=y.device)
    check(lib().sed_bn_bwd_finalize(ptr(part), rows, Cc, ptr(sum_g), ptr(sum_gx), None, None, stream_ptr()), "bn_bwd_finalize")
    return sum_g, sum_gx


def conv3x3_dgrad_bnred(dy, wd, pooled, gamma, beta, y_below, mean, rstd, pool_f, pool_t, drop_p=0.0, scale=None, shift=None, wino=False):
    B, T, F, Cc = dy.shape
    Cin = pooled.shape[-1]
    rows = lib().sed_conv3x3_wino_rows(B, Cc, F, T, Cin) if wino else lib().sed_conv3x3_dgrad_bnred_rows(B, Cc, F, T, Cin)
    assert rows > 0, "shape does not take the fused MFMA path"
    dx = torch.empty(B, T, F, Cin, device=dy.device)
    part = torch.empty(rows, 2, Cin, device=dy.device)
    if scale is None:
        scale = gamma * rstd
        shift = beta - mean * scale
    entry = lib().sed_conv3x3_wino_dgrad_bnred if wino else lib().sed_conv3x3_dgrad_bnred
    check(entry(ptr(_f32c(dy)), ptr(_f32c(wd)), ptr(dx), ptr(part), ptr(_f32c(pooled)), ptr(gamma), ptr(beta),
                ptr(_f32c(y_below)), ptr(mean), ptr(rstd), drop_p, pool_f, pool_t, y_below.shape[2],
                y_below.shape[1], B, Cc, F, T, Cin, stream_ptr()), "conv3x3_dgrad_bnred")
    sum_g, sum_gx = torch.empty(Cin, device=dy.device), torch.empty(Cin, device=dy.device)
    check(lib().sed_bn_bwd_finalize_small_gamma(ptr(part), rows, Cin, ptr(sum_g), ptr(sum_gx), None, None, ptr(dx), ptr(pooled),
                                                ptr(y_below), ptr(gamma), ptr(beta), ptr(mean), ptr(rstd), ptr(scale), ptr(shift),
                                                B, y_below.shape[1], y_below.shape[2], pool_f, pool_t, drop_p, stream_ptr()),
          "bn_bwd_finalize_small_gamma")
    return dx, sum_g, sum_gx


def gemm(A, B, bias=None, out=None, beta=0.0):
    M, K = A.shape
    K2, N = B.shape
    assert K == K2
    if out is None:
        out = torch.empty(M, N, device=A.device)
    check(lib().sed_gemm_f32(ptr(A), A.stride(0), A.stride(1), ptr(B), B.stride(0), B.stride(1), ptr(out),
                             out.stride(0), ptr(bias), beta, M, N, K, stream_ptr()), "gemm_f32")
    return out


_GEMM_WS = {}


def gemm_ws(A, B, out=None, bias=None, wgrad=False):
    M, K = A.shape
    _, N = B.shape
    if out is None:
        out = torch.empty(M, N, device=A.device)
    nb = lib().sed_gemm_f32_workspace_bytes(M, N, K)
    key = (A.device, nb)
    ws = _GEMM_WS.get(key) if nb else None
    if nb and ws is None:
        ws = _GEMM_WS[key] = torch.empty(nb // 4 + 1, device=A.device)
    if wgrad:
        assert bias is None
        check(lib().sed_gemm_f32_wgrad(ptr(A), A.stride(0), A.stride(1), ptr(B), B.stride(0), B.stride(1), ptr(out),
                                       out.stride(0), M, N, K, ptr(ws), stream_ptr()), "gemm_f32_wgrad")
        return out
    check(lib().sed_gemm_f32_ws(ptr(A), A.stride(0), A.stride(1), ptr(B), B.stride(0), B.stride(1), ptr(out),
                                out.stride(0), ptr(bias), M, N, K, ptr(ws), stream_ptr()), "gemm_f32_ws")
    return out


def gemm_plan(M, N, K, policy=0):
    bm, bn, splits, k_len = C.c_int(), C.c_int(), C.c_int(), C.c_int()
    check(lib().sed_gemm_f32_plan(M, N, K, policy, C.byref(bm), C.byref(bn), C.byref(splits), C.byref(k_len)), "gemm_f32_plan")
    return bm.value, bn.value, splits.value, k_len.value


def linear_fwd(x, W, b, relu=False):
    M, K = x.shape
    N = W.shape[0]
    y = torch.empty(M, N, device=x.device)
    check(lib().sed_linear_fwd(ptr(_f32c(x)), ptr(_f32c(W)), ptr(b), ptr(y), M, K, N, int(relu), stream_ptr()), "linear_fwd")
    return y


def linear_bwd(x, W, y, dy, relu=False, need_dx=True):
    M, K = x.shape
    N = W.shape[0]
    ws = torch.empty(lib().sed_linear_bwd_workspace_bytes(M, K, N) // 4 + 1, device=x.device)
    dx = torch.empty_like(x) if need_dx else None
    dW, db = torch.empty_like(W), torch.empty(N, device=x.device)
    dy = dy.clone()
    check(lib().sed_linear_bwd(ptr(x), ptr(W), ptr(y), ptr(dy), ptr(dx), ptr(dW), ptr(db), ptr(ws), M, K, N,
                               int(relu), stream_ptr()), "linear_bwd")
    return dx, dW, db


def _pp(tensors):
    arr = (C.c_void_p * len(tensors))(*[t.data_ptr() for t in tensors])
    return arr


def gru_seq_fwd(gi, whh, bhh, save=True):
    B, T, _, H3 = gi.shape
    H = H3 // 3
    out = torch.empty(B, T, 2 * H, device=gi.device)
    saved = torch.empty(B, T, 2, 5, H, device=gi.device) if save else None
    ws = torch.empty(lib().sed_gru_seq_workspace_bytes(H) // 4, device=gi.device)
    check(lib().sed_gru_seq_fwd(ptr(_f32c(gi)), _pp(whh), _pp(bhh), ptr(out), ptr(saved), ptr(ws), B, T, H,
                                stream_ptr()), "gru_seq_fwd")
    return out, saved


def gru_seq_bwd(dout, saved, whh, want_bias=False):
    B, T, H2 = dout.shape
    H = H2 // 2
    dgi = torch.empty(B, T, 2, 3 * H, device=dout.device)
    dgh = torch.empty(B, T, 2, 3 * H, device=dout.device)
    if not want_bias:
        check(lib().sed_gru_seq_bwd(ptr(_f32c(dout)), ptr(saved), _pp(whh), ptr(dgi), ptr(dgh), None, None, None,
                                    B, T, H, stream_ptr()), "gru_seq_bwd")
        return dgi, dgh
    dbih = [torch.empty(3 * H, device=dout.device) for _ in range(2)]
    dbhh = [torch.empty(3 * H, device=dout.device) for _ in range(2)]
    ws = torch.empty(lib().sed_gru_seq_bwd_workspace_bytes(B, H) // 4 + 1, device=dout.device)
    check(lib().sed_gru_seq_bwd(ptr(_f32c(dout)), ptr(saved), _pp(whh), ptr(dgi), ptr(dgh), _pp(dbih), _pp(dbhh),
                                ptr(ws), B, T, H, stream_ptr()), "gru_seq_bwd")
    return dgi, dgh, dbih, dbhh
# ... 85 lines not shown
```

Baseline: 6.028 million mel-frames/s.

## Emit pool-winner candidates from Winograd conv epilogue to shrink BN-pool forward pass

In training, when the layer uses the Winograd forward path with (1,2) pooling, the conv epilogue now also writes a half-size tensor of pool winners. Because BN is a monotone affine map, the winner of each time pair is chosen by the sign of gamma using fmed3 against ±inf. The BN+ReLU+dropout forward then reads only this half-size tensor instead of the full conv output. This roughly halves that kernel's reads, at the cost of extra writes and workspace in the conv epilogue. The full conv output is still written for the backward pass.

```diff
diff --git a/include/sedcrnn.h b/include/sedcrnn.h
--- a/include/sedcrnn.h
+++ b/include/sedcrnn.h
@@ -67,6 +67,8 @@
                                  const float* gamma, const float* beta, const float* conv_out_below, const float* mean,
                                  const float* rstd, float drop_p, int pool_f, int pool_t, int Fy, int Ty,
                                  int B, int C, int F, int T, int Cin, void* stream);
+int sed_conv3x3_wino_fwd_winners(const float* x, const float* uf, const float* bias, float* y, float* stat_partials,
+                                 const float* gamma, float* winners, int B, int Cin, int F, int T, int Cout, void* stream);
 int sed_conv3x3_wino_pack_weights_bn_folded(const float* w_oihw, const float* bias, const float* gamma, const float* beta,
                                             const float* running_mean, const float* running_var, float eps,
                                             float* uf, float* bias_folded, int Cout, int Cin, void* stream);
@@ -98,6 +100,9 @@
 int sed_bn_relu_pool_drop_fwd(const float* y, const float* scale, const float* shift, float* out,
                               int B, int T, int F, int C, int pool_f, int pool_t, int out_tcf,
                               float drop_p, uint64_t seed, const uint64_t* seed_dev, void* stream);
+int sed_bn_relu_drop_fwd_winners(const float* winners, const float* scale, const float* shift, float* out,
+                                 int B, int Tp, int Fp, int C, int out_tcf,
+                                 float drop_p, uint64_t seed, const uint64_t* seed_dev, void* stream);
 
 int sed_bn_relu_pool_route(const float* y, const float* scale, const float* shift, unsigned char* route,
                            int B, int T, int F, int C, int pool_f, int pool_t, void* stream);
@@ -454,6 +459,7 @@
 #define SED_NET_AUX_FIRST 0x1
 #define SED_NET_NO_GATE 0x2
 #define SED_NET_DIRECT_CONV 0x4
+#define SED_NET_NO_POOL_WINNERS 0x8
 
 typedef struct sed_net_params {
     float* conv_w[SED_MAX_CONV];
diff --git a/sed_crnn_amd/_lib.py b/sed_crnn_amd/_lib.py
--- a/sed_crnn_amd/_lib.py
+++ b/sed_crnn_amd/_lib.py
@@ -71,6 +71,7 @@
     "sed_conv3x3_wino_packed_floats": (_sz, [_i, _i]),
     "sed_conv3x3_wino_pack_weights": (_i, [_fp, _fp, _fp, _i, _i, _stream]),
     "sed_conv3x3_wino_fwd": (_i, [_fp, _fp, _fp, _fp, _fp, _i, _i, _i, _i, _i, _stream]),
+    "sed_conv3x3_wino_fwd_winners": (_i, [_fp, _fp, _fp, _fp, _fp, _fp, _fp, _i, _i, _i, _i, _i, _stream]),
     "sed_conv3x3_wino_dgrad_bnred": (_i, [_fp, _fp, _fp, _fp, _fp, _fp, _fp, _fp, _fp, _fp, _f, _i, _i, _i, _i, _i, _i, _i, _i, _i, _stream]),
     "sed_conv3x3_wino_pack_weights_bn_folded": (_i, [_fp, _fp, _fp, _fp, _fp, _fp, _f, _fp, _fp, _i, _i, _stream]),
     "sed_conv3x3_wino_bn_relu_pool_eval": (_i, [_fp, _fp, _fp, _fp, _i, _i, _i, _i, _i, _stream]),
@@ -97,6 +98,7 @@
     "sed_bn_finalize_from_sums": (_i, [_fp, _i, _d, _fp, _fp, _fp, _fp, _f, _f, _fp, _fp, _fp, _fp, _stream]),
     "sed_bn_finalize_eval": (_i, [_fp, _fp, _fp, _fp, _f, _i, _fp, _fp, _stream]),
     "sed_bn_relu_pool_drop_fwd": (_i, [_fp, _fp, _fp, _fp, _i, _i, _i, _i, _i, _i, _i, _f, _u64, _fp, _stream]),
+    "sed_bn_relu_drop_fwd_winners": (_i, [_fp, _fp, _fp, _fp, _i, _i, _i, _i, _i, _f, _u64, _fp, _stream]),
     "sed_bn_relu_pool_route": (_i, [_fp, _fp, _fp, _fp, _i, _i, _i, _i, _i, _i, _stream]),
     "sed_bn_bwd_rows": (_i, [_i, _i, _i]),
     "sed_bn_relu_pool_drop_bwd_reduce": (_i, [_fp, _fp, _fp, _fp, _fp, _fp, _fp, _i, _i, _i, _i, _i, _i, _i, _f, _u64, _fp, _stream]),
diff --git a/sed_crnn_amd/csrc/bnpool.hip b/sed_crnn_amd/csrc/bnpool.hip
--- a/sed_crnn_amd/csrc/bnpool.hip
+++ b/sed_crnn_amd/csrc/bnpool.hip
@@ -264,6 +264,96 @@
     return 0;
 }
 
+__global__ __launch_bounds__(256) void bn_relu_drop_fwd_win_k(
+    const float* __restrict__ win, const float* __restrict__ scale, const float* __restrict__ shift,
+    float* __restrict__ out, size_t n, int C, float drop_p, uint64_t seed, const uint64_t* __restrict__ seed_dev) {
+    if (seed_dev) seed += seed_dev[0] * 0x9E3779B97F4A7C15ull;
+    const int C4 = C >> 2;
+    const float inv_keep = drop_p > 0.f ? 1.f / (1.f - drop_p) : 1.f;
+    const bool small = n <= 0xFFFFFFFFull;
+    for (size_t i = (size_t)blockIdx.x * 256 + threadIdx.x; i < n; i += (size_t)gridDim.x * 256) {
+        const int c4 = small ? (int)((unsigned)i % (unsigned)C4) : (int)(i % C4);
+        f32x4 sc = *(const f32x4*)(scale + c4 * 4), sh = *(const f32x4*)(shift + c4 * 4);
+        f32x4 m = {0, 0, 0, 0};
+        f32x4 v = *(const f32x4*)(win + i * 4);
+        v = v * sc + sh;
+#pragma unroll
+        for (int k = 0; k < 4; ++k) m[k] = fmaxf(m[k], v[k]);
+        if (drop_p > 0.f) {
+#pragma unroll
+            for (int k = 0; k < 4; ++k) m[k] *= sed_drop_mult(seed, i * 4 + k, drop_p, inv_keep);
+        }
+        *(f32x4*)(out + i * 4) = m;
+    }
+}
+
+__global__ __launch_bounds__(256) void bn_relu_drop_fwd_win_tcf_k(
+    const float* __restrict__ win, const float* __restrict__ scale, const float* __restrict__ shift,
+    float* __restrict__ out, int rows, int Fp, int C, float drop_p, uint64_t seed, const uint64_t* __restrict__ seed_dev) {
+    if (seed_dev) seed += seed_dev[0] * 0x9E3779B97F4A7C15ull;
+    extern __shared__ __attribute__((aligned(16))) float tile[];
+    const int C4 = C >> 2, LD = C + 1;
+    const float inv_keep = drop_p > 0.f ? 1.f / (1.f - drop_p) : 1.f;
+    for (int bt = blockIdx.x; bt < rows; bt += gridDim.x) {
+        __syncthreads();
+        for (int i = threadIdx.x; i < Fp * C4; i += 256) {
+            int c4 = i % C4, fp = i / C4;
+            f32x4 sc = *(const f32x4*)(scale + c4 * 4), sh = *(const f32x4*)(shift + c4 * 4);
+            f32x4 m = {0, 0, 0, 0};
+            f32x4 v = *(const f32x4*)(win + ((size_t)bt * Fp * C4 + i) * 4);
+            v = v * sc + sh;
+#pragma unroll
+            for (int k = 0; k < 4; ++k) m[k] = fmaxf(m[k], v[k]);
+            if (drop_p > 0.f) {
+                size_t oi = (((size_t)bt * Fp + fp) * C4 + c4) * 4;
+#pragma unroll
+                for (int k = 0; k < 4; ++k) m[k] *= sed_drop_mult(seed, oi + k, drop_p, inv_keep);
+            }
+#pragma unroll
+            for (int k = 0; k < 4; ++k) tile[fp * LD + c4 * 4 + k] = m[k];
+        }
+        __syncthreads();
+        float* o = out + (size_t)bt * C * Fp;
+        if ((Fp & 3) == 0 && ((size_t)out & 15) == 0) {
+            for (int i = threadIdx.x; i < C * (Fp >> 2); i += 256) {
+                const int c = (i * 4) / Fp, fp = i * 4 - c * Fp;
+                const f32x4 v = {tile[fp * LD + c], tile[(fp + 1) * LD + c], tile[(fp + 2) * LD + c], tile[(fp + 3) * LD + c]};
+                *(f32x4*)(o + i * 4) = v;
+            }
+        } else {
+            for (int i = threadIdx.x; i < C * Fp; i += 256) {
+                int c = i / Fp, fp = i - c * Fp;
+                o[i] = tile[fp * LD + c];
+            }
+        }
+    }
+}
+
+extern "C" int sed_bn_relu_drop_fwd_winners(const float* winners, const float* scale, const float* shift, float* out, int B,
+                                            int Tp, int Fp, int C, int out_tcf, float drop_p, uint64_t seed,
+                                            const uint64_t* seed_dev, void* stream) {
+    SED_REQUIRE(winners && scale && shift && out, "bn_relu_drop_fwd_winners: null pointer");
+    SED_REQUIRE(B > 0 && Tp > 0 && Fp > 0 && C > 0, "bn_relu_drop_fwd_winners: bad shape");
+    SED_REQUIRE(C % 4 == 0, "bn_relu_drop_fwd_winners: C must be a multiple of 4 (got %d)", C);
+    SED_REQUIRE((size_t)B * Tp <= 0x7FFFFFFFull, "bn_relu_drop_fwd_winners: B*Tp=%zu rows do not fit an int", (size_t)B * Tp);
+    SED_REQUIRE(drop_p >= 0.f && drop_p < 1.f, "bn_relu_drop_fwd_winners: drop_p=%f out of [0,1)", drop_p);
+    hipStream_t s = as_stream(stream);
+    SedProfScope prof(SED_K_BN_FWD, s, 8.0 * B * C * (double)Tp * Fp);
+    if (!out_tcf) {
+        size_t n = (size_t)B * Tp * Fp * (C / 4);
+        int grid = (int)((n + 255) / 256 < 8192 ? (n + 255) / 256 : 8192);
+        bn_relu_drop_fwd_win_k<<<grid, 256, 0, s>>>(winners, scale, shift, out, n, C, drop_p, seed, seed_dev);
+    } else {
+        size_t lds = (size_t)Fp * (C + 1) * sizeof(float);
+        SED_REQUIRE(lds <= 150 * 1024, "bn_relu_drop_fwd_winners: F'*C tile too large for LDS");
+        if (lds > 48 * 1024) (void)hipFuncSetAttribute((const void*)bn_relu_drop_fwd_win_tcf_k, hipFuncAttributeMaxDynamicSharedMemorySize, (int)lds);
+        int grid = B * Tp < 4096 ? B * Tp : 4096;
+        bn_relu_drop_fwd_win_tcf_k<<<grid, 256, lds, s>>>(winners, scale, shift, out, B * Tp, Fp, C, drop_p, seed, seed_dev);
+    }
+    SED_LAUNCH_CHECK("bn_relu_drop_fwd_winners");
+    return 0;
+}
+
 __global__ __launch_bounds__(256) void bn_relu_pool_route_k(
     const float* __restrict__ y, const float* __restrict__ scale, const float* __restrict__ shift,
     unsigned char* __restrict__ route, int B, int T, int F, int C, int pf, int pt) {
diff --git a/sed_crnn_amd/csrc/conv_shared.h b/sed_crnn_amd/csrc/conv_shared.h
--- a/sed_crnn_amd/csrc/conv_shared.h
+++ b/sed_crnn_amd/csrc/conv_shared.h
@@ -14,6 +14,7 @@
     const unsigned char* bits;
     float* rgp;
     float invXT;
+    float* cand;
 };
 
 #ifdef __HIPCC__
diff --git a/sed_crnn_amd/csrc/net.hip b/sed_crnn_amd/csrc/net.hip
--- a/sed_crnn_amd/csrc/net.hip
+++ b/sed_crnn_amd/csrc/net.hip
@@ -8,6 +8,7 @@
                int rg_rows;
                int rgrad;
                int wino, wino_d;
+               int cand;
                int ev;
                int bf; };
 
@@ -22,6 +23,7 @@
     size_t wp_f[SED_MAX_CONV], wp_d[SED_MAX_CONV], conv_out[SED_MAX_CONV], stat[SED_MAX_CONV];
     size_t mean[SED_MAX_CONV], rstd[SED_MAX_CONV], scale[SED_MAX_CONV], shift[SED_MAX_CONV];
     size_t pooled[SED_MAX_CONV], bn_sums[SED_MAX_CONV], c1_stat_ws, c1_bits, c1_mom;
+    size_t pool_cand[SED_MAX_CONV];
     size_t bias_f[SED_MAX_CONV];
     size_t wih_perm;
     size_t gi[SED_MAX_GRU], gout[SED_MAX_GRU], saved[SED_MAX_GRU];
@@ -48,7 +50,7 @@
     SED_REQUIRE(c->n_dense >= 1 && c->n_dense <= SED_MAX_DENSE, "net: n_dense=%d out of range", c->n_dense);
     SED_REQUIRE(c->conv_mode >= 0 && c->conv_mode <= 2, "net: conv_mode=%d (0 = exact fp32, 1 = bf16x3 experiment, 2 = bf16 inference)", c->conv_mode);
     SED_REQUIRE(c->conv_mode != 2 || !training, "net: conv_mode 2 (bf16 inference) is an eval-only plan; training runs with conv_mode 0 or 1");
-    SED_REQUIRE((c->flags & ~(SED_NET_AUX_FIRST | SED_NET_NO_GATE | SED_NET_DIRECT_CONV)) == 0, "net: unknown flags 0x%x", c->flags);
+    SED_REQUIRE((c->flags & ~(SED_NET_AUX_FIRST | SED_NET_NO_GATE | SED_NET_DIRECT_CONV | SED_NET_NO_POOL_WINNERS)) == 0, "net: unknown flags 0x%x", c->flags);
     memset(L, 0, sizeof(*L));
     L->n_conv = c->n_conv; L->n_gru = c->n_gru; L->n_dense = c->n_dense;
     const int fm = c->conv_mode == 2 ? 0 : c->conv_mode;
@@ -103,6 +105,8 @@
         L->stat[l] = cv.take((size_t)q.rows * 2 * q.C);
         L->mean[l] = cv.take(q.C); L->rstd[l] = cv.take(q.C); L->scale[l] = cv.take(q.C); L->shift[l] = cv.take(q.C);
         L->pooled[l] = cv.take(q.bf ? (npool + 1) / 2 : npool);
+        q.cand = (training && q.wino && q.pf == 1 && q.pt == 2 && !(c->flags & SED_NET_NO_POOL_WINNERS)) ? 1 : 0;
+        L->pool_cand[l] = q.cand ? cv.take(npool) : 0;
         L->bn_sums[l] = cv.take((size_t)2 * q.C);
         L->bias_f[l] = cv.take(q.C);
         if (npool > max_pool) max_pool = npool;
@@ -332,6 +336,9 @@
                 else if (training)
                     SED_TRY(sed_conv1_stats(in, ws + L.wp_f[l], p->conv_b[l], ws + L.stat[l], ws + L.c1_stat_ws, B, q.Cin, q.F, q.T, q.C,
                                             q.rgrad ? (double*)(ws + L.c1_mom) : nullptr, stream));
+            } else if (q.cand) {
+                SED_TRY(sed_conv3x3_wino_fwd_winners(in, ws + L.wp_f[l], p->conv_b[l], ws + L.conv_out[l], ws + L.stat[l], p->bn_g[l],
+                                                     ws + L.pool_cand[l], B, q.Cin, q.F, q.T, q.C, stream));
             } else if (q.wino) {
                 SED_TRY(sed_conv3x3_wino_fwd(in, ws + L.wp_f[l], p->conv_b[l], ws + L.conv_out[l], training ? ws + L.stat[l] : nullptr,
                                              B, q.Cin, q.F, q.T, q.C, stream));
@@ -361,6 +368,9 @@
                                                     ws + L.pooled[l], B, q.Cin, q.F, q.T, q.C, q.pf, q.pt,
                                                     training ? q.drop : 0.f, layer_seed(seed, l), seed_dev,
                                                     (training && q.rgrad) ? (unsigned char*)(ws + L.c1_bits) : nullptr, stream));
+        else if (q.cand)
+            SED_TRY(sed_bn_relu_drop_fwd_winners(ws + L.pool_cand[l], ws + L.scale[l], ws + L.shift[l], ws + L.pooled[l], B,
+                                                 q.Tp, q.Fp, q.C, last, q.drop, layer_seed(seed, l), seed_dev, stream));
         else
             SED_TRY(sed_bn_relu_pool_drop_fwd(ws + L.conv_out[l], ws + L.scale[l], ws + L.shift[l], ws + L.pooled[l], B,
                                               q.T, q.F, q.C, q.pf, q.pt, last, training ? q.drop : 0.f,
@@ -455,6 +465,7 @@
         else if (is("scale")) { off = L.scale[index]; n = q.C; ok = true; }
         else if (is("shift")) { off = L.shift[index]; n = q.C; ok = true; }
         else if (is("dconv") && training && !q.fused) { off = L.dconv[index]; n = nout; ok = true; }
+        else if (is("pool_cand") && q.cand) { off = L.pool_cand[index]; n = npool; ok = true; }
     }
     if (!ok && gru_idx) {
         const size_t M = (size_t)L.M, H = L.gr[index].H;
diff --git a/sed_crnn_amd/csrc/wino.hip b/sed_crnn_amd/csrc/wino.hip
--- a/sed_crnn_amd/csrc/wino.hip
+++ b/sed_crnn_amd/csrc/wino.hip
@@ -342,6 +342,16 @@
     f32x4 bv = {0, 0, 0, 0};
     if (bias) bv = *(const f32x4*)(bias + cb);
     char* const yb = (char*)(y + (size_t)b * (EV ? T >> 1 : T) * F * Cout + cb);
+    const bool cand = !BNR && !EV && br.cand != nullptr;
+    f32x4 cinf = {0, 0, 0, 0};
+    char* cdb = nullptr;
+    unsigned cov[4] = {0, 0, 0, 0};
+    if (cand) {
+        const f32x4 cgm = *(const f32x4*)(br.gamma + cb);
+#pragma unroll
+        for (int e = 0; e < 4; ++e) cinf[e] = cgm[e] < 0.f ? -INFINITY : INFINITY;
+        cdb = (char*)(br.cand + (size_t)b * (T >> 1) * F * Cout);
+    }
     f32x4 q_kr = {0, 0, 0, 0}, q_nb = {0, 0, 0, 0}, a1 = {0, 0, 0, 0}, a2 = {0, 0, 0, 0};
     if (BNR) {
 #pragma unroll
@@ -357,6 +367,13 @@
 #pragma unroll
     for (int k = 0; k < (RG ? 9 * RGC : 1); ++k) R[k] = (f32x4){0, 0, 0, 0};
     if (!BNR) WN_EPI_ROWS();
+    if (cand) {
+#pragma unroll
+        for (int k = 0; k < 4; ++k) {
+            const int q = q0 + mt * 32 + rq + 8 * k;
+            cov[k] = rov[k] - (unsigned)sed_fdiv(q, geo.invFw) * rstride + (unsigned)cb * 4u;
+        }
+    }
     unsigned xov[4];
 #pragma unroll
     for (int k = 0; k < 4; ++k) xov[k] = RG ? xofftab[mt * 32 + rq + 8 * k] : 0u;
@@ -388,6 +405,12 @@
                 for (int e = 0; e < 4; ++e) pl[e] = fmaxf(fmaxf(o[0][e], o[1][e]), 0.f);
                 *(f32x4*)(yb + ro + jj * cstride) = pl;
                 continue;
+            }
+            if (cand) {
+                f32x4 wn;
+#pragma unroll
+                for (int e = 0; e < 4; ++e) wn[e] = __builtin_amdgcn_fmed3f(o[0][e], o[1][e], cinf[e]);
+                *(f32x4*)(cdb + (cov[k] + jj * cstride)) = wn;
             }
 #pragma unroll
             for (int i = 0; i < 2; ++i) {
@@ -499,7 +522,8 @@
                              int rgc, int B, int Cin, int F, int T, int Cout, hipStream_t s) {
     WinoGeo g;
     SED_REQUIRE(wino_geo(B, Cin, F, T, Cout, &g), "conv3x3_wino: shape B=%d Cin=%d F=%d T=%d Cout=%d is not supported (sed_conv3x3_wino_rows)", B, Cin, F, T, Cout);
-    SED_REQUIRE(rgc >= -1 && rgc <= 2 && (rgc <= 0 || (br && br->x1 && br->bits && br->rgp)) && (rgc >= 0 || (!br && !stat)), "conv3x3_wino: bad epilogue arguments");
+    SED_REQUIRE(rgc >= -2 && rgc <= 2 && (rgc <= 0 || (br && br->x1 && br->bits && br->rgp)) && (rgc != -1 || (!br && !stat)) &&
+                (rgc != -2 || (br && br->gamma && br->cand)), "conv3x3_wino: bad epilogue arguments");
     g.dbg = g_wino_dbg;
     if (rgc > 0) {
         g.lds += ((size_t)64 + (size_t)rgc * (F + 2) * (4 * g.TR + 2) + (size_t)4 * 9 * rgc * 32) * sizeof(float);
@@ -528,6 +552,7 @@
     if (rgc == 1) WN_LAUNCH(WN_NHMAX, true, 1, false);
     else if (rgc == 2) WN_LAUNCH(WN_NHMAX, true, 2, false);
     else if (rgc == -1) WN_LAUNCH(WN_NHMAX, false, 0, true);
+    else if (rgc == -2) WN_LAUNCH(WN_NHMAX, false, 0, false);
     else if (br) WN_LAUNCH(WN_NHMAX, true, 0, false);
     else WN_LAUNCH(WN_NHMAX, false, 0, false);
 #undef WN_LAUNCH
@@ -543,6 +568,17 @@
     hipStream_t s = as_stream(stream);
     SedProfScope prof(SED_K_CONV_MFMA_FWD, s, 2.0 * 9.0 * Cin * Cout * (double)B * T * F);
     return sed_internal_wino_launch(x, uq, bias, y, stat, nullptr, 0, B, Cin, F, T, Cout, s);
+}
+
+extern "C" int sed_conv3x3_wino_fwd_winners(const float* x, const float* uq, const float* bias, float* y, float* stat, const float* gamma,
+                                            float* winners, int B, int Cin, int F, int T, int Cout, void* stream) {
+    SED_REQUIRE(x && uq && y && gamma && winners, "conv3x3_wino_fwd_winners: null pointer");
+    hipStream_t s = as_stream(stream);
+    SedProfScope prof(SED_K_CONV_MFMA_FWD, s, 2.0 * 9.0 * Cin * Cout * (double)B * T * F);
+    ConvBnRed br{};
+    br.gamma = gamma;
+    br.cand = winners;
+    return sed_internal_wino_launch(x, uq, bias, y, stat, &br, -2, B, Cin, F, T, Cout, s);
 }
 
 extern "C" int sed_conv3x3_wino_dgrad_bnred(const float* dy, const float* ud, float* dx, float* partials, const float* pooled,
diff --git a/sed_crnn_amd/model.py b/sed_crnn_amd/model.py
--- a/sed_crnn_amd/model.py
+++ b/sed_crnn_amd/model.py
@@ -347,10 +347,16 @@
             self._structs = (P, G)
         return self._structs
 
+    def _ws_key(self, B, T, training, flags, bf16=False):
+        key = (int(B), int(T), bool(training))
+        if flags:
+            key = key + (("flags", int(flags)),)
+        if bf16:
+            key = key + ("bf16",)
+        return key
+
     def _workspace(self, cfg, training):
-        key = (cfg.B, cfg.T, bool(training))
-        if cfg.conv_mode == 2:
-            key = key + ("bf16",)
+        key = self._ws_key(cfg.B, cfg.T, training, cfg.flags, cfg.conv_mode == 2)
         ws = self._ws.get(key)
         if ws is None:
             nbytes = lib().sed_net_workspace_bytes(C.byref(cfg), int(training))
@@ -368,7 +374,7 @@
         return ws
 
     def pin_workspace(self, B, T, training=True):
-        self._ws_pinned.add((int(B), int(T), bool(training)))
+        self._ws_pinned.add(self._ws_key(B, T, training, getattr(self, "plan_flags", 0)))
 
     def _check_input(self, x):
         if not (isinstance(x, torch.Tensor) and x.is_cuda):
diff --git a/sed_crnn_amd/ops.py b/sed_crnn_amd/ops.py
--- a/sed_crnn_amd/ops.py
+++ b/sed_crnn_amd/ops.py
@@ -61,6 +61,19 @@
     check(lib().sed_conv3x3_wino_fwd(ptr(_f32c(x)), ptr(_f32c(up)), ptr(bias), ptr(y), ptr(stat), B, Cin, F, T, Cout, stream_ptr()),
           "conv3x3_wino_fwd")
     return y, stat
+
+
+def conv3x3_wino_fwd_winners(x, up, bias, gamma, Cout):
+    B, T, F, Cin = x.shape
+    rows = lib().sed_conv3x3_wino_rows(B, Cin, F, T, Cout)
+    if rows <= 0:
+        raise ValueError("conv3x3_wino_fwd_winners: shape not supported")
+    y = torch.empty(B, T, F, Cout, device=x.device)
+    stat = torch.zeros(rows, 2, Cout, device=x.device)
+    win = torch.empty(B, T // 2, F, Cout, device=x.device)
+    check(lib().sed_conv3x3_wino_fwd_winners(ptr(_f32c(x)), ptr(_f32c(up)), ptr(bias), ptr(y), ptr(stat), ptr(_f32c(gamma)), ptr(win),
+                                             B, Cin, F, T, Cout, stream_ptr()), "conv3x3_wino_fwd_winners")
+    return y, stat, win
 
 
 def conv3x3_bn_relu_pool_eval(x, w, bias, gamma, beta, running_mean, running_var, eps=1e-5, wino=False):
@@ -157,6 +170,14 @@
     out = torch.empty((B, Tp, Cc, Fp) if out_tcf else (B, Tp, Fp, Cc), device=y.device)
     check(lib().sed_bn_relu_pool_drop_fwd(ptr(_f32c(y)), ptr(scale), ptr(shift), ptr(out), B, T, F, Cc, pool_f, pool_t,
                                           int(out_tcf), drop_p, seed, None, stream_ptr()), "bn_relu_pool_drop_fwd")
+    return out
+
+
+def bn_relu_drop_fwd_winners(win, scale, shift, out_tcf=False, drop_p=0.0, seed=0, seed_dev=None):
+    B, Tp, Fp, Cc = win.shape
+    out = torch.empty((B, Tp, Cc, Fp) if out_tcf else (B, Tp, Fp, Cc), device=win.device)
+    check(lib().sed_bn_relu_drop_fwd_winners(ptr(_f32c(win)), ptr(scale), ptr(shift), ptr(out), B, Tp, Fp, Cc, int(out_tcf),
+                                             drop_p, seed, ptr(seed_dev), stream_ptr()), "bn_relu_drop_fwd_winners")
     return out
 
 
```

Result: no change. 6.068 million mel-frames/s, median of 6 (+0.7%).
